# ActiveVisionLab/NeFeS

Hardware: AMD Instinct MI355X
Metric: rays/s (fwd+bwd) at 640x480x(64+128) samples, 8x256 MLP (higher is better)
Workload: dtype f32; 1 GPU; BASELINE configs[1]: 7-Scenes-stairs geometry, 64+128 samples, 8x256 MLP + 16-ch feature head; 640x480, random seed-0 weights, fwd + bwd to the 3x4 pose; parallelism=rows/1

## Files before the change

include/nefes_hip.h:

```cpp
#ifndef NEFES_HIP_H
#define NEFES_HIP_H
#include <stddef.h>
#include <stdint.h>

#ifdef __cplusplus
extern "C" {
#endif

#define NEFES_ABI_VERSION 20
#define NEFES_BLOB_FORMAT 17

#define NEFES_E_BADARG (-1)
#define NEFES_E_UNSUPPORTED (-2)
#define NEFES_E_BADBLOB (-3)

typedef struct NefesNetDesc {
    int32_t width;
    int32_t feat_dim;
    int32_t has_transient;
    int32_t xyz_encoding;
    int32_t fold_final;
} NefesNetDesc;
#define NEFES_XYZ_FREQ10 0
#define NEFES_XYZ_EXTERNAL32 1

typedef struct NefesStreamInfo {
    uint64_t slab_off;
    uint32_t n_slabs;
    uint32_t bias_floats;
    uint64_t bias_off;
    uint32_t scale_off;
    uint32_t scale_count;
} NefesStreamInfo;

typedef struct NefesBlobInfo {
    uint64_t total_bytes;
    NefesStreamInfo stream[13];
} NefesBlobInfo;

#define NEFES_COMP_TRANSIENT 1u
#define NEFES_COMP_STATIC_ONLY 2u
#define NEFES_COMP_SIGMA_ONLY 4u
#define NEFES_COMP_WHITE_BKGD 8u
#define NEFES_COMP_FEAT_WEIGHTS_ONLY 16u

#define NEFES_FIELD_SIGMA 0
#define NEFES_FIELD_STATIC 1
#define NEFES_FIELD_FULL 2

int nefes_version(void);

int nefes_blob_info(const NefesNetDesc* desc, NefesBlobInfo* info);
size_t nefes_stream_slab_bytes(const NefesNetDesc* desc, int stream);
int nefes_pack_weights(const NefesNetDesc* desc, const float* const* tensors, int n_tensors, void* blob,
                       size_t blob_bytes);
int nefes_pack_map(const NefesNetDesc* desc, uint32_t* map, size_t n_entries, int64_t* tensor_elems_out);
int nefes_pack_h3_plan(const NefesNetDesc* desc, int32_t* plan, size_t n_ints, size_t* needed);
int nefes_pack_device(const float* flat, int64_t n_params, const uint32_t* map, int64_t n_entries, const int32_t* plan,
                      int n_jobs, int32_t* scratch, void* blob, void* stream);

int nefes_raygen_fwd(int H, int W, float focal, const float* c2w, int row0, int nrows, float* rays_o, float* rays_d,
                     float* viewdirs, void* stream);
size_t nefes_raygen_bwd_workspace(int n_rays);
int nefes_raygen_bwd(int H, int W, float focal, const float* c2w, int row0, int nrows, const float* g_rays_o,
                     const float* g_rays_d, const float* g_viewdirs, void* workspace, float* g_c2w, void* stream);
int nefes_raygen_k_fwd(int H, int W, const float* intr, const float* c2w, int row0, int nrows, float* rays_o, float* rays_d,
                       float* viewdirs, void* stream);
size_t nefes_raygen_k_bwd_workspace(int n_rays);
int nefes_raygen_k_bwd(int H, int W, const float* intr, const float* c2w, int row0, int nrows, const float* g_rays_o,
                       const float* g_rays_d, const float* g_viewdirs, void* workspace, float* g_c2w, float* g_intr, void* stream);
int nefes_raygen_px_fwd(int n, const float* px, const float* intr, const float* c2w, float* rays_o, float* rays_d, float* viewdirs,
                        void* stream);
size_t nefes_raygen_px_bwd_workspace(int n);
int nefes_raygen_px_bwd(int n, const float* px, const float* intr, const float* c2w, const float* g_rays_o, const float* g_rays_d,
                        const float* g_viewdirs, void* workspace, float* g_c2w, float* g_intr, void* stream);
int nefes_sample_px(int C, int H, int W, const float* map, int n, const float* px, float* out, void* stream);
int nefes_ndc_fwd(int H, int W, float focal, float near, int n, const float* rays_o, const float* rays_d, float* out_o,
                  float* out_d, void* stream);
int nefes_ndc_bwd(int H, int W, float focal, float near, int n, const float* rays_o, const float* rays_d,
                  const float* g_out_o, const float* g_out_d, float* g_rays_o, float* g_rays_d, void* stream);
int nefes_coarse_depths(int N, int Nc, float near, float far, int lindisp, const float* t, const float* t_rand,
                        float* z, void* stream);
int nefes_coarse_depths_rays(int N, int Nc, const float* bounds, int stride, int lindisp, const float* t,
                             const float* t_rand, float* z, void* stream);

size_t nefes_field_mask_bytes(const NefesNetDesc* desc, int64_t M);
int nefes_field_fwd(const NefesNetDesc* desc, const void* packed, int mode, int N, int S, const float* rays_o,
                    const float* rays_d, const float* z, const float* pts, const float* xyz_enc, const float* viewdirs,
                    float* raw_t, uint32_t* masks, void* stream);
int nefes_field_bwd(const NefesNetDesc* desc, const void* packed, int N, int S, const float* rays_o,
                    const float* rays_d, const float* z, const float* pts, const float* viewdirs, const float* raw_t,
                    const float* g_raw_t, const uint32_t* masks, float* g_pts, float* g_xyz_enc, float* g_viewdirs_s,
                    void* stream);
int nefes_ray_grad_reduce(int N, int S, const float* z, const float* g_pts, const float* g_viewdirs_s, float* g_rays_o,
                          float* g_rays_d, float* g_viewdirs, void* stream);

int nefes_composite_fwd(int N, int S, int C, uint32_t flags, float beta_min, const float* raw_t, const float* z,
                        float* rgb, float* feat, float* disp, float* acc, float* depth, float* weights, float* beta,
                        void* stream);
int nefes_composite_bwd(int N, int S, int C, uint32_t flags, const float* raw_t, const float* z, const float* g_rgb,
                        const float* g_feat, const float* g_disp, const float* g_acc, const float* g_depth,
                        const float* g_weights, const float* g_beta, float* g_raw_t, void* stream);

int nefes_sample_pdf_merge(int N, int Nc, int Ni, int layout, const float* z_coarse, const float* weights,
                           const float* u, int u_per_ray, const float* cdf_in, float* z_fine, float* z_samples,
                           int32_t* inds, float* cdf_out, void* stream);
int nefes_coarse_sample(int N, int Nc, int Ni, const float* sigma, const float* z, int z_shared_row, const float* u, int u_per_ray,
                        float* z_fine, float* z_samples, float* weights_out, void* stream);

typedef struct NefesHashGridDesc {
    int32_t n_levels;
    int32_t n_features;
    int32_t log2_hashmap_size;
    int32_t base_resolution;
    float per_level_scale;
    float bound;
} NefesHashGridDesc;
size_t nefes_hashgrid_table_entries(const NefesHashGridDesc* desc);
int nefes_hashgrid_fwd(const NefesHashGridDesc* desc, const float* table, int64_t M, const float* x, float* enc,
                       void* stream);
int nefes_hashgrid_bwd_x(const NefesHashGridDesc* desc, const float* table, int64_t M, const float* x, const float* g_enc,
                         float* g_x, void* stream);
size_t nefes_hashgrid_bwd_table_workspace(const NefesHashGridDesc* desc);
int nefes_hashgrid_bwd_table(const NefesHashGridDesc* desc, int64_t M, const float* x, const float* g_enc, float* g_table,
                             void* workspace, void* stream);

int nefes_field_fwd_x6(const NefesNetDesc* desc, const void* packed, int mode, int N, int S, const float* rays_o,
                       const float* rays_d, const float* z, const float* pts, const float* xyz_enc, const float* viewdirs,
                       float* raw_t, uint32_t* masks, void* stream);

int nefes_field_bwd_static(const NefesNetDesc* desc, const void* packed, int N, int S, const float* rays_o,
                           const float* rays_d, const float* z, const float* pts, const float* viewdirs, const float* raw_t,
                           const float* g_raw_t, const uint32_t* masks, float* g_pts, float* g_viewdirs_s, void* stream);

int nefes_field_bwd_x6(const NefesNetDesc* desc, const void* packed, int N, int S, const float* rays_o, const float* rays_d,
                       const float* z, const float* pts, const float* viewdirs, const float* raw_t, const float* g_raw_t,
                       const uint32_t* masks, float* g_pts, float* g_xyz_enc, float* g_viewdirs_s, void* stream);

int nefes_field_fwd_h3(const NefesNetDesc* desc, const void* packed, int mode, int N, int S, const float* rays_o,
                       const float* rays_d, const float* z, const float* pts, const float* xyz_enc, const float* viewdirs,
                       float* raw_t, uint32_t* masks, void* stream);
int nefes_field_fwd_h3_zrow(const NefesNetDesc* desc, const void* packed, int mode, int N, int S, const float* rays_o,
                            const float* rays_d, const float* z_row, const float* viewdirs, float* raw_t, uint32_t* masks,
                            void* stream);
int nefes_field_bwd_h3(const NefesNetDesc* desc, const void* packed, int N, int S, const float* rays_o, const float* rays_d,
                       const float* z, const float* pts, const float* viewdirs, const float* raw_t, const float* g_raw_t,
                       const uint32_t* masks, float* g_pts, float* g_xyz_enc, float* g_viewdirs_s, void* stream);
int nefes_field_fwd_h3_hashgrid(const NefesNetDesc* desc, const void* packed, const NefesHashGridDesc* grid, const float* table,
                                int mode, int N, int S, const float* rays_o, const float* rays_d, const float* z, int z_is_row,
                                const float* viewdirs, float* raw_t, uint32_t* masks, void* stream);
int nefes_field_bwd_h3_hashgrid(const NefesNetDesc* desc, const void* packed, const NefesHashGridDesc* grid, const float* table,
                                int N, int S, const float* rays_o, const float* rays_d, const float* z, const float* viewdirs,
                                const float* raw_t, const float* g_raw_t, const uint32_t* masks, float* g_pts, float* g_viewdirs_s,
                                void* stream);
int nefes_field_fwd_h3_fh(const NefesNetDesc* desc, const void* packed, int mode, int N, int S, const float* rays_o,
                          const float* rays_d, const float* z, const float* viewdirs, float* raw_t, uint32_t* masks, void* stream);
int nefes_field_bwd_h3_fh(const NefesNetDesc* desc, const void* packed, int N, int S, const float* rays_o, const float* rays_d,
                          const float* z, const float* viewdirs, const float* raw_t, const float* g_raw_t, const float* g_gmap,
                          const uint32_t* masks, float* g_pts, float* g_viewdirs_s, void* stream);
int nefes_feat_head_fwd(int N, int C, int F, const float* gmap, const float* w_t, const float* b, float* feat, void* stream);
int nefes_feat_head_bwd(int N, int C, int F, const float* g_feat, const float* w, const float* b, float* g_gmap, void* stream);
int nefes_field_bwd_static_h3(const NefesNetDesc* desc, const void* packed, int N, int S, const float* rays_o, const float* rays_d,
                              const float* z, const float* pts, const float* viewdirs, const float* raw_t, const float* g_raw_t,
                              const uint32_t* masks, float* g_pts, float* g_viewdirs_s, void* stream);
#define NEFES_H3_REQ_TRAIN 1
#define NEFES_H3_REQ_EXT 2
#define NEFES_H3_REQ_HASHGRID 4
#define NEFES_H3_REQ_FH 8
#define NEFES_H3_REQ_ZROW 16
#define NEFES_H3_REQ_STATIC_BWD 32
int nefes_field_h3_instance(const NefesNetDesc* desc, int backward, int mode, unsigned request_flags, char* name, size_t cap);

typedef struct NefesGenericNetDesc {
    int32_t width;
    int32_t depth;
    int32_t skip;
    int32_t feat_dim;
    int32_t has_transient;
    int32_t xyz_encoding;
} NefesGenericNetDesc;
size_t nefes_generic_blob_bytes(const NefesGenericNetDesc* desc);
int nefes_generic_pack(const NefesGenericNetDesc* desc, const float* const* tensors, int n_tensors, void* blob, size_t blob_bytes);
size_t nefes_generic_mask_bytes(const NefesGenericNetDesc* desc, int64_t M);
int nefes_field_fwd_generic(const NefesGenericNetDesc* desc, const void* packed, int mode, int N, int S, const float* rays_o,
                            const float* rays_d, const float* z, const float* pts, const float* viewdirs, float* raw_t,
                            uint32_t* masks, void* stream);
int nefes_field_bwd_generic(const NefesGenericNetDesc* desc, const void* packed, int mode, int N, int S, const float* rays_o,
                            const float* rays_d, const float* z, const float* pts, const float* viewdirs, const float* raw_t,
                            const float* g_raw_t, const uint32_t* masks, float* g_pts, float* g_viewdirs_s, void* stream);
int nefes_field_fwd_generic_ext(const NefesGenericNetDesc* desc, const void* packed, int mode, int N, int S, const float* xyz_enc,
                                const float* viewdirs, float* raw_t, uint32_t* masks, void* stream);
int nefes_field_bwd_generic_ext(const NefesGenericNetDesc* desc, const void* packed, int mode, int N, int S, const float* viewdirs,
                                const float* raw_t, const float* g_raw_t, const uint32_t* masks, float* g_xyz_enc, float* g_viewdirs_s,
                                void* stream);
int nefes_generic_pack_device(const NefesGenericNetDesc* desc, const float* const* tensors, int n_tensors, void* blob,
                              size_t blob_bytes, void* stream);
size_t nefes_generic_train_rows(const NefesGenericNetDesc* desc);
int nefes_generic_train_row_offset(const NefesGenericNetDesc* desc, int block);
int nefes_field_fwd_train_generic(const NefesGenericNetDesc* desc, const void* packed, int mode, int N, int S, const float* rays_o,
                                  const float* rays_d, const float* z, const float* viewdirs, float* raw_t, float* acts, uint32_t* masks,
                                  void* stream);
int nefes_field_bwd_train_generic(const NefesGenericNetDesc* desc, const void* packed, int mode, int N, int S, const float* rays_o,
                                  const float* rays_d, const float* z, const float* viewdirs, const float* raw_t, const float* g_raw_t,
                                  const uint32_t* masks, float* dacts, float* g_pts, float* g_viewdirs_s, void* stream);
size_t nefes_generic_train_rows_ext(const NefesGenericNetDesc* desc);
int nefes_generic_train_row_offset_ext(const NefesGenericNetDesc* desc, int block);
int nefes_field_fwd_train_generic_ext(const NefesGenericNetDesc* desc, const void* packed, int mode, int N, int S, const float* xyz_enc,
                                      const float* viewdirs, float* raw_t, float* acts, uint32_t* masks, void* stream);
int nefes_field_bwd_train_generic_ext(const NefesGenericNetDesc* desc, const void* packed, int mode, int N, int S,
                                      const float* viewdirs, const float* raw_t, const float* g_raw_t, const uint32_t* masks,
                                      float* dacts, float* g_xyz_enc, float* g_viewdirs_s, void* stream);

size_t nefes_train_rows(const NefesNetDesc* desc);
int nefes_train_row_offset(const NefesNetDesc* desc, int block);
int nefes_field_fwd_train(const NefesNetDesc* desc, const void* packed, int mode, int N, int S, const float* rays_o,
                          const float* rays_d, const float* z, const float* pts, const float* viewdirs, float* raw_t,
                          float* acts, uint32_t* masks, void* stream);
int nefes_field_fwd_train_h3(const NefesNetDesc* desc, const void* packed, int mode, int N, int S, const float* rays_o,
                             const float* rays_d, const float* z, const float* pts, const float* viewdirs, float* raw_t,
                             float* acts, uint32_t* masks, void* stream);
int nefes_field_bwd_train(const NefesNetDesc* desc, const void* packed, int mode, int N, int S, const float* rays_o,
                          const float* rays_d, const float* z, const float* viewdirs, const float* raw_t,
                          const float* g_raw_t, const uint32_t* masks, float* dacts, float* g_pts, float* g_viewdirs_s,
                          void* stream);
int nefes_field_bwd_train_h3(const NefesNetDesc* desc, const void* packed, int mode, int N, int S, const float* rays_o,
                             const float* rays_d, const float* z, const float* viewdirs, const float* raw_t,
                             const float* g_raw_t, const uint32_t* masks, float* dacts, float* g_pts, float* g_viewdirs_s,
                             void* stream);
int nefes_field_fwd_train_h3_ext(const NefesNetDesc* desc, const void* packed, int mode, int N, int S, const float* xyz_enc,
                                 const float* viewdirs, float* raw_t, float* acts, uint32_t* masks, void* stream);
int nefes_field_bwd_train_h3_ext(const NefesNetDesc* desc, const void* packed, int mode, int N, int S, const float* viewdirs,
                                 const float* raw_t, const float* g_raw_t, const uint32_t* masks, float* dacts, float* g_xyz_enc,
                                 float* g_viewdirs_s, void* stream);
int nefes_train_head_grad(const NefesNetDesc* desc, int mode, int N, int S, const float* raw_t, const float* g_raw_t,
                          float* dacts, void* stream);
int nefes_train_dx(int64_t n_tiles, int rows, const float* dacts_in, int g_row0, int n_out, const float* wt, int ldw,
                   int n_in, const float* acts, int dst_row0, int accumulate, int mask, float* dacts_out, void* stream);
int nefes_train_dw(int64_t n_tiles, int rows, const float* dacts, int g_row0, int n_out, const float* acts, int x_row0,
                   int n_in, int x_relu, int splits, float* partial, void* stream);
int nefes_train_dw_bias(int64_t n_tiles, int rows, const float* dacts, int g_row0, int n_out, const float* acts, int x_row0,
                        int n_in, int x_relu, int splits, int64_t split_stride, float* partial, void* stream);

int nefes_conv2d_same(int B, int Cin, int Cout, int H, int W, int ksize, const float* x, const float* mask, const float* w_packed,
                      const float* bias, int relu, float* y, void* stream);
size_t nefes_conv2d_wgrad_workspace(int B, int Cin, int Cout, int H, int W, int ksize);
int nefes_conv2d_wgrad(int B, int Cin, int Cout, int H, int W, int ksize, const float* x, const float* g_y, const float* mask, float* g_w,
                       float* g_bias, void* workspace, void* stream);

int nefes_bicubic_up_fwd(int64_t planes, int h, int w, int OH, int OW, int oy0, int ox0, int CH, int CW, const float* in, float* out,
                         void* stream);
int nefes_bicubic_up_bwd(int64_t planes, int h, int w, int OH, int OW, int oy0, int ox0, int CH, int CW, const float* g_out, float* tmp,
                         float* g_in, void* stream);

int nefes_pose_compose_fwd(int n_poses, const float* r, const float* t, const float* init_c2w, float pose_scale, const float* move,
                           float pose_scale2, float* c2w, void* stream);
int nefes_pose_compose_bwd(int n_poses, const float* r, const float* t, const float* init_c2w, float pose_scale, const float* move,
                           float pose_scale2, const float* g_c2w, float* g_r, float* g_t, void* stream);
int nefes_bn_train_fwd(int B, int C, int64_t P, int per_image, const float* x, const float* weight, const float* bias, double eps,
                       double momentum, float* running_mean, float* running_var, int64_t* num_batches_tracked, float* y, double* save,
                       void* stream);
int nefes_bn_train_bwd(int B, int C, int64_t P, int per_image, const float* x, const float* weight, const double* save, const float* g_y,
                       float* g_x, void* stream);
int nefes_bn_train_bwd_affine(int B, int C, int64_t P, const float* x, const float* weight, const double* save, const float* g_y,
                              float* g_x, float* g_weight, float* g_bias, void* stream);
int nefes_svd_reg_fwd(int n_poses, const float* pose, float* out, double* save, void* stream);
int nefes_svd_reg_bwd(int n_poses, const double* save, const float* g_out, float* g_pose, void* stream);
int nefes_regressed_pose_fwd(int n_poses, const float* pose, int do_svd, float t_scale, float mx, float my, float mz, float* out, double* save,
                             void* stream);
int nefes_regressed_pose_bwd(int n_poses, const double* save, int do_svd, float t_scale, const float* g_out, float* g_pose, void* stream);
size_t nefes_psnr_ssim_workspace(int C, int H, int W);
int nefes_psnr_ssim(int C, int H, int W, const float* x, int64_t x_row_stride, int64_t x_plane_stride, const float* y, int64_t y_row_stride,
                    int64_t y_plane_stride, void* workspace, float* out, void* stream);
size_t nefes_cosine_loss_scratch_doubles(int C);
int nefes_cosine_loss_fwd(int C, int64_t P, const float* a, const float* b, double* scratch, float* loss, void* stream);
int nefes_cosine_loss_bwd(int C, int64_t P, const float* a, const float* b, const double* scratch, const float* g_loss, float* g_a,
                          void* stream);

int nefes_upcos_loss_fwd(int C, int h, int w, int OH, int OW, int crop, const float* x, const float* target, double* scratch, float* loss,
                         void* stream);
int nefes_upcos_loss_bwd(int C, int h, int w, int OH, int OW, int crop, const float* x, const float* target, const double* scratch,
                         const float* g_loss, const int* tx_first, const int* tx_count, const float* tx_wt, const int* ty_first,
                         const int* ty_count, const float* ty_wt, int T, float* tmp, float* g_x, void* stream);
size_t nefes_pixcos_scratch_doubles(int G, int64_t P);
int nefes_pixcos_loss_fwd(int G, int C, int64_t P, const float* a, const float* b, double* scratch, float* loss, void* stream);
int nefes_pixcos_loss_bwd(int G, int C, int64_t P, const float* a, const float* b, const double* scratch, const float* g_loss, float* g_a,
                          void* stream);
size_t nefes_uppixcos_scratch_doubles(int G, int OH, int OW, int crop);
int nefes_uppixcos_loss_fwd(int G, int C, int h, int w, int OH, int OW, int crop, const float* x, const float* target, double* scratch,
                            float* loss, void* stream);
int nefes_uppixcos_loss_bwd(int G, int C, int h, int w, int OH, int OW, int crop, const float* x, const float* target, const double* scratch,
                            const float* g_loss, const int* tx_first, const int* tx_count, const float* tx_wt, const int* ty_first,
                            const int* ty_count, const float* ty_wt, int T, float* tmp, float* g_x, void* stream);
int nefes_cosine_loss_masked_fwd(int G, int Cg, int64_t P, const float* a, const float* b, const uint8_t* mask, double* scratch, float* loss,
                                 void* stream);
int nefes_cosine_loss_masked_bwd(int G, int Cg, int64_t P, const float* a, const float* b, const uint8_t* mask, const double* scratch,
                                 const float* g_loss, float* g_a, void* stream);
int nefes_upcos_loss_masked_fwd(int G, int Cg, int h, int w, int OH, int OW, int crop, const float* x, const float* target,
                                const uint8_t* mask, double* scratch, float* loss, void* stream);
int nefes_upcos_loss_masked_bwd(int G, int Cg, int h, int w, int OH, int OW, int crop, const float* x, const float* target,
                                const uint8_t* mask, const double* scratch, const float* g_loss, const int* tx_first, const int* tx_count,
                                const float* tx_wt, const int* ty_first, const int* ty_count, const float* ty_wt, int T, float* tmp,
                                float* g_x, void* stream);
size_t nefes_pixcos_masked_scratch_doubles(int G, int64_t P);
int nefes_pixcos_loss_masked_fwd(int G, int C, int64_t P, const float* a, const float* b, const uint8_t* mask, double* scratch, float* loss,
                                 void* stream);
int nefes_pixcos_loss_masked_bwd(int G, int C, int64_t P, const float* a, const float* b, const uint8_t* mask, const double* scratch,
                                 const float* g_loss, float* g_a, void* stream);
size_t nefes_uppixcos_masked_scratch_doubles(int G, int OH, int OW, int crop);
int nefes_uppixcos_loss_masked_fwd(int G, int C, int h, int w, int OH, int OW, int crop, const float* x, const float* target,
                                   const uint8_t* mask, double* scratch, float* loss, void* stream);
int nefes_uppixcos_loss_masked_bwd(int G, int C, int h, int w, int OH, int OW, int crop, const float* x, const float* target,
                                   const uint8_t* mask, const double* scratch, const float* g_loss, const int* tx_first,
                                   const int* tx_count, const float* tx_wt, const int* ty_first, const int* ty_count, const float* ty_wt,
                                   int T, float* tmp, float* g_x, void* stream);
int nefes_bicubic_gram(int n_in, int n_out, int o0, int n_win, double* G, void* stream);
int nefes_upcos_prepare(int C, int h, int w, int OH, int OW, int crop, const float* target, const int* tx_first, const int* tx_count,
                        const float* tx_wt, const int* ty_first, const int* ty_count, const float* ty_wt, int T, double* tmp, double* tt,
                        double* dbb, void* stream);
int nefes_upcos_gram_fwd(int C, int h, int w, const float* x, const double* tt, const double* dbb, const double* gram_x, const double* gram_y,
                         int band, double* scratch, double* pmat, float* loss, void* stream);
size_t nefes_upcos_gram_lds_bytes(int h, int w, int band);
int nefes_upcos_gram_bwd(int C, int h, int w, const double* tt, const double* pmat, const double* scratch, const float* g_loss, float* g_x,
                         void* stream);
int nefes_bicubic_gather_table(int n_in, int n_out, int o0, int n_win, int T, int* first, int* count, float* wt, void* stream);

int nefes_fusion_input_fwd(int B, int HW, int C, const float* rgb, const float* feat, const float* affine, const float* mean3,
                           const float* std3, float* x, float* y, void* stream);
int nefes_fusion_input_bwd(int B, int HW, int C, const float* g_x, const float* affine, const float* y, const float* std3, float* g_rgb,
                           float* g_feat, void* stream);
int nefes_adam_step(int n, float* p, const float* g, float* m, float* v, float* step, const double* lr, double beta1, double beta2,
                    double eps, void* stream);

#define NEFES_TRAIN_LOSS_ROWS 16
#define NEFES_LOSS_FEAT_MSE 0
#define NEFES_LOSS_FEAT_L1 1
#define NEFES_LOSS_FEAT_COS 2
#define NEFES_LOSS_HAS_RGB_FINE 1u
#define NEFES_LOSS_HAS_RGB_COARSE 2u
#define NEFES_LOSS_HAS_BETA 4u
#define NEFES_LOSS_HAS_FEAT_FINE 8u
#define NEFES_LOSS_HAS_FEAT_COARSE 16u
#define NEFES_LOSS_HAS_FEAT_FUSION 32u
#define NEFES_LOSS_NERFW 64u
#define NEFES_LOSS_PRESENT_ALL 127u
typedef struct NefesTrainLossDesc {
    int32_t N;
    int32_t C;
    int32_t S;
    int32_t feat_kind;
    uint32_t present;
    float coef;
    float lambda_u;
    int64_t sigma_row_stride;
} NefesTrainLossDesc;
size_t nefes_train_loss_scratch_doubles(int N);
int nefes_train_loss_fwd(const NefesTrainLossDesc* desc, const float* rgb_fine, const float* rgb_coarse, const float* rgb_target,
                         const float* beta, const float* transient_sigmas, const float* feat_fine, const float* feat_coarse,
                         const float* feat_fusion, const float* feat_target, double* scratch, float* terms, float* losses, void* stream);
int nefes_train_loss_bwd(const NefesTrainLossDesc* desc, const float* g_color, const float* g_loss_f, const float* g_loss_fusion,
                         const float* rgb_fine, const float* rgb_coarse, const float* rgb_target, const float* beta,
                         const float* transient_sigmas, const float* feat_fine, const float* feat_coarse, const float* feat_fusion,
                         const float* feat_target, float* g_rgb_fine, float* g_rgb_coarse, float* g_beta, float* g_sigma, float* g_feat_fine,
                         float* g_feat_coarse, float* g_feat_fusion, void* stream);

int nefes_probe_mfma_clock(int random_operands, int ms_target, double* clock_ghz, double* fp16_dense_tflops, void* stream);
int nefes_probe_store_hazard(float* out, int64_t n_float4, int nops, void* stream);
int nefes_probe_pk_mul(unsigned* out, int64_t n, int iters, void* stream);
int nefes_probe_hazard(int test, int k, int blocks, int iters, unsigned* count, void* stream);
int nefes_probe_aggressor(int kind, int iters, int blocks, float* sink, void* stream);

#ifdef __cplusplus
}
#endif
#endif
```

nefes_amd/csrc/field_fwd_h3.hip:

```cpp
#include "field_h3_instances.h"
#ifdef NEFES_TU_W128
#define NEFES_SLAB_KIB 16
#else
#define NEFES_SLAB_KIB 32
#endif
#include <stdio.h>
#include <stdlib.h>
#if defined(NEFES_TU_W128) || !defined(H3_NO_ACC_READ_ASM)
#define NEFES_ASM_READS_ACC
#define NEFES_FENCE_TILES
#endif
#if defined(NEFES_TU_W128)
#define NEFES_ACC_VGPR_FORM
#endif

#ifndef NEFES_FWD_CONSUMER_BIAS
#define NEFES_FWD_CONSUMER_BIAS 1
#endif
#include "field_common.h"
#include "../../include/nefes_hip.h"

#include "field_x6.h"
#include "hashgrid.h"
#if !defined(NEFES_TU_W128) && !defined(H3_NO_ACC_READ_ASM)
#define H3_ACC_READ_ASM
#endif
#include "field_h3.h"
#define NEFES_H3_SLOTS 2

struct FieldFwdH3Args {
    const char* stream;
    const float* bias;
    uint32_t n_slabs, bias_floats, scale_off;
    const float* rays_o;
    const float* rays_d;
    const float* z;
    const float* pts;
    const float* xyz_enc;
    const float* viewdirs;
    float* raw_t;
    uint32_t* masks;
    int N, S, R, C;
    long long M;
    int n_tiles;
    uint32_t s_magic, s_shift;
    float* acts;
    int rows;
    int z_row;
    const float2* hg_table;
    HgGeom hg;
    int gout;
};

template <int NT, int T0, int NX>
__device__ __forceinline__ void train_save_h3(float* tile_base, uint32_t voff, int row0, const f32x16 (&X)[NX], float inv) {
    float* p = tile_base + (size_t)(row0 >> 5) * 4096 + voff;
#pragma unroll
    for (int t = 0; t < NT; ++t)
#pragma unroll
        for (int r = 0; r < 16; ++r) {
#ifndef NEFES_TRAIN_NO_STORES
            __builtin_nontemporal_store(X[T0 + t][r] * inv, &p[t * 4096 + nefes_rho(0, r) * 16]);
#endif
        }
}

template <int MODEF, int ENC, int W = 256, int NTR = 1, bool TRAIN = false, bool FH = false>
__global__ __launch_bounds__(256, W == 128 ? 2 : 1) void field_fwd_h3_kernel(FieldFwdH3Args a) {
    constexpr bool FOLD = MODEF == NEFES_FIELD_FULL_FOLD;
    constexpr int MODE = FOLD ? NEFES_FIELD_FULL : MODEF;
    static_assert(NEFES_SLAB_KIB == (W == 128 ? NEFES_H3_FWD_SLAB_KIB_128 : NEFES_H3_FWD_SLAB_KIB), "ring slab size != the packer's for this width");
    static_assert(!FOLD || (MODE != NEFES_FIELD_SIGMA && !TRAIN), "the fold serves the head products of frozen networks");
    constexpr int NTW = W / 32, NTH = W / 64;
    constexpr int ES = ENC != NEFES_XYZ_FREQ10 ? NEFES_X_STEPS : NEFES_E_STEPS;
    constexpr int MW = 8 * (W / 64) + 4 * (W / 128), WT = (NTW + 1) / 2, WH = (NTH + 1) / 2;
    constexpr int NSEG = MODE == NEFES_FIELD_SIGMA ? NEFES_H3F_SIG + 1
                         : (MODE == NEFES_FIELD_STATIC ? NEFES_H3F_N_STATIC : (FOLD ? NEFES_H3FF_N : NEFES_H3F_N));
    extern __shared__ __attribute__((aligned(16))) char smem[];
    char* ring_base = smem;
    float* bias_lds = (float*)(smem + NEFES_H3_SLOTS * NEFES_SLAB_BYTES);
    float* e_lds = bias_lds + ((a.bias_floats + 63) / 64) * 64 + (threadIdx.x >> 6) * (ES * 64) + (threadIdx.x & 63);
    const int lane = threadIdx.x & 63;
    const int wave = __builtin_amdgcn_readfirstlane(threadIdx.x >> 6);
    const int j = lane & 31, h = lane >> 5;
    for (uint32_t i = threadIdx.x; i < a.bias_floats; i += 256) bias_lds[i] = a.bias[i];
    HgGeom* hg_lds = (HgGeom*)(bias_lds + ((a.bias_floats + 63) / 64) * 64 + 4 * ES * 64);
    if constexpr (ENC == NEFES_XYZ_HASHGRID_FUSED) {
        if (threadIdx.x == 0) *hg_lds = a.hg;
    }
    StagedRing ring;
    ring.init(a.stream, a.n_slabs, ring_base, wave, lane);
    const char* ring_lane = ring_base + lane * 16;
    const char* bias_half = (const char*)bias_lds + 16 * h;
    const int* tab_i = (const int*)(bias_lds + a.scale_off);
    const float* tab_f = bias_lds + a.scale_off;
    auto wexp = [&](int seg) { return tab_i[nefes_h3_tab_exp(nefes_h3f_seg(FOLD, seg))]; };
    auto rowb = [&](int seg) { return tab_f[nefes_h3_tab_bound(nefes_h3f_seg(FOLD, seg))]; };
    auto bmax = [&](int blk) { return tab_f[nefes_h3_tab_bias(NSEG, nefes_h3f_bias(FOLD, blk))]; };
    ring.prime(ring_lane);
    constexpr int B_SIG = 8 * W, B_FINAL = B_SIG + 32, B_DIR = B_FINAL + (FOLD ? 0 : W), B_RGB = B_DIR + W / 2,
                  B_T0 = B_RGB + 32 * NTR, B_T1 = B_T0 + W / 2, B_T2 = B_T1 + W / 2, B_TH = B_T2 + W / 2;
#pragma unroll 1
    for (int tile = blockIdx.x; tile < a.n_tiles; tile += gridDim.x) {
        auto locate = [&](uint32_t& m, uint32_t& ray, uint32_t& smp) {
            const uint32_t m_raw = (uint32_t)tile * 128u + (uint32_t)(wave * 32 + j);
            const bool ok = m_raw < (uint32_t)a.M;
            m = ok ? m_raw : (uint32_t)a.M - 1u;
            ray = a.s_magic ? __umulhi(m, a.s_magic) >> a.s_shift : m;
            smp = m - ray * (uint32_t)a.S;
            return ok;
        };
        uint32_t m, ray, smp;
        locate(m, ray, smp);
        float in_o[3] = {0.f, 0.f, 0.f}, in_d[3] = {0.f, 0.f, 0.f}, in_z = 0.f;
        float E[ES];
        if constexpr (ENC == NEFES_XYZ_EXTERNAL32) {
#pragma unroll
            for (int s = 0; s < ES; ++s) E[s] = a.xyz_enc[(size_t)m * 32 + 2 * s + h];
        } else if (ENC != NEFES_XYZ_HASHGRID_FUSED && a.pts) {
#pragma unroll
            for (int c = 0; c < 3; ++c) in_o[c] = a.pts[(size_t)m * 3 + c];
        } else {
            in_z = a.z[a.z_row ? smp : m];
#pragma unroll
            for (int c = 0; c < 3; ++c) { in_o[c] = a.rays_o[ray * 3 + c]; in_d[c] = a.rays_d[ray * 3 + c]; }
        }
        float mE;
        if constexpr (ENC == NEFES_XYZ_EXTERNAL32) {
            mE = pair_max(array_max(E));
        } else if constexpr (ENC == NEFES_XYZ_HASHGRID_FUSED) {
            float x[3];
#pragma unroll
            for (int c = 0; c < 3; ++c) x[c] = add_rn(in_o[c], mul_rn(in_d[c], in_z));
            hg_encode_slots(E, x, h, *hg_lds, a.hg_table);
            mE = pair_max(array_max(E));
        } else {
            float x[3];
#pragma unroll
            for (int c = 0; c < 3; ++c) x[c] = a.pts ? in_o[c] : add_rn(in_o[c], mul_rn(in_d[c], in_z));
            embed_slots<NEFES_N_FREQ_XYZ>(E, x, h);
            mE = fmaxf(fmaxf(1.f, fabsf(x[0])), fmaxf(fabsf(x[1]), fabsf(x[2])));
        }
#pragma unroll
        for (int s = 0; s < ES; ++s) e_lds[s * 64] = E[s];
        float* act_tile = nullptr;
        const uint32_t act_voff = nefes_train_lane_off(wave, j, h);
        const uint32_t emb_off = (uint32_t)(((wave * 32 + j) >> 4) * 512 + h * 16 + (j & 15));
        if constexpr (TRAIN) {
            act_tile = a.acts + (size_t)tile * a.rows * 128;
            float* pe = act_tile + (size_t)(nefes_train_row(W, 0, NEFES_TB_E) >> 5) * 4096 + emb_off;
#pragma unroll
            for (int s = 0; s < ES; ++s) __builtin_nontemporal_store(E[s], &pe[(s >> 4) * 4096 + 2 * (s & 15) * 16]);
        }
        auto save_trunk = [&](int layer, const f32x16 (&X)[NTW], int es) {
            if constexpr (TRAIN) train_save_h3<NTW, 0>(act_tile, act_voff, nefes_train_row(W, 0, NEFES_TB_L1) + (layer - 1) * W, X, pow2i(-es));
        };
        uint32_t* mask_ptr = (MODE != NEFES_FIELD_SIGMA && a.masks) ? a.masks + ((size_t)((long long)tile * 4 + wave) * MW) * 64 + lane : nullptr;
        auto put_masks = [&](const uint32_t* bits, int n) {
            if (MODE != NEFES_FIELD_SIGMA && mask_ptr) {
                for (int w = 0; w < n; ++w) __builtin_nontemporal_store(bits[w], &mask_ptr[w * 64]);
                mask_ptr += n * 64;
            }
        };
        auto raw_col = [&]() -> float* {
            uint32_t mm, rr, ss;
            if (!locate(mm, rr, ss)) return nullptr;
            return a.raw_t + ((size_t)rr * a.R * a.S + ss);
        };
        auto bias_at = [&](int off_floats, int es) { return BiasInitScaled{bias_half + off_floats * 4, pow2i(es)}; };
        constexpr bool CB = !TRAIN && W == 256 && NEFES_FWD_CONSUMER_BIAS;
        float2 nbias;
        f32x16 A[NTW], B[NTW];
        uint32_t bits[WT];
        auto clear_bits = [&]() {
#pragma unroll
            for (int w = 0; w < WT; ++w) bits[w] = 0u;
        };
        constexpr bool CAP = MODE != NEFES_FIELD_SIGMA;
        auto tau_of = [&](float M, int ew) {
            const int t = pick_exp(M);
            return t < 100 - ew ? t : 100 - ew;
        };
        auto sigma_head = [&](const f32x16 (&X)[NTW], int es_x, int tau_x) {
            f32x16 sg[1];
            float mdummy = 0.f;
            const int es = tau_x + wexp(NEFES_H3F_SIG);
            if constexpr (CB) {
                const char* bp8 = bias_half + 7 * W * 4;
                nbias = ReluBiasSplitH<false, NTW, WT>::prime(bp8);
                mma_run_h3<1, W / 16, 0, true>(ring, ring_lane, ReluBiasSplitH<false, NTW, WT>{X, bits, pow2i(tau_x - es_x), mdummy, bp8, pow2i(es_x), nbias},
                                               bias_at(B_SIG, es), sg);
            } else
            mma_run_h3<1, W / 16, 0, true>(ring, ring_lane, ReluSplitH<false, NTW, WT>{X, bits, pow2i(tau_x - es_x), mdummy},
                                           bias_at(B_SIG, es), sg);
            float* col = raw_col();
            if (col && h == 0) {
                const int ch = (MODE == NEFES_FIELD_SIGMA) ? 0 : 3 + a.C;
                __builtin_nontemporal_store(softplus_ref(sg[0][0] * pow2i(-es)), &col[(size_t)ch * a.S]);
            }
        };
        int es_a, es_b = 0;
        float M;
        {
            const int tau = tau_of(mE, wexp(NEFES_H3F_L1));
            es_a = tau + wexp(NEFES_H3F_L1);
            if constexpr (CB) mma_run_h3<NTW, ES / 8, 0, true>(ring, ring_lane, LdsSplitH{e_lds, pow2i(tau)}, ZeroInit{}, A);
            else mma_run_h3<NTW, ES / 8, 0, true>(ring, ring_lane, LdsSplitH{e_lds, pow2i(tau)}, bias_at(0, es_a), A);
            M = rowb(NEFES_H3F_L1) * mE + bmax(NEFES_H3BB_L1);
            save_trunk(1, A, es_a);
        }
#define NEFES_FWD_EVEN_LAYER(L1_, SEG1_)                                                                                       \
        clear_bits();                                                                                                          \
        {                                                                                                                      \
            const int ew = wexp(SEG1_), tau = tau_of(M, ew);                                                                   \
            const float rb_ = rowb(SEG1_), bm_ = bmax((L1_) - 1);           \
            float mx = 0.f;                                                                                                    \
            if constexpr (CB) {                                                                                                \
                const char* bps = bias_half + ((L1_) - 2) * W * 4;                           \
                nbias = ReluBiasSplitH<CAP, NTW, WT>::prime(bps);                                                              \
                mma_run_h3<NTW, W / 16, 0, true>(ring, ring_lane, ReluBiasSplitH<CAP, NTW, WT>{A, bits, pow2i(tau - es_a), mx, bps, pow2i(es_a), nbias}, \
                                                 ZeroInit{}, B);                                                               \
            } else                                                                                                             \
            mma_run_h3<NTW, W / 16, 0, true>(ring, ring_lane, ReluSplitH<CAP, NTW, WT>{A, bits, pow2i(tau - es_a), mx},        \
                                             bias_at(((L1_) - 1) * W, tau + ew), B);                                           \
            M = rb_ * (pair_max(mx) * pow2i(-es_a)) + bm_;                                                                     \
            es_b = tau + ew;                                                                                                   \
            save_trunk(L1_, B, es_b);                                                                                          \
        }                                                                                                                      \
        put_masks(bits, WT);
        constexpr bool END8 = MODE == NEFES_FIELD_SIGMA || FOLD;
        constexpr int NPAIRS = END8 ? 3 : 4;
#pragma unroll 1
        for (int p = 0; p < NPAIRS; ++p) {
            const int l1 = 2 + 2 * p, l2 = l1 + 1;
            const int seg1 = l1 <= 5 ? l1 - 1 : l1;
            const int seg2 = l2 <= 5 ? l2 - 1 : (l2 <= 8 ? l2 : NEFES_H3F_FINAL);
            NEFES_FWD_EVEN_LAYER(l1, seg1)
            clear_bits();
            {
                const int ew = wexp(seg2);
                const int tau = tau_of(p == 1 ? fmaxf(M, mE) : M, ew);
                if (p == 3) sigma_head(B, es_b, tau_of(M, wexp(NEFES_H3F_SIG)));
                const float rb_ = rowb(seg2), bm_ = bmax(l2 <= 8 ? l2 - 1 : NEFES_H3BB_FINAL);
                const float rbe_ = p == 1 ? rowb(NEFES_H3F_L5E) : 0.f;
                float mx = 0.f;
                if constexpr (CB) {
                    const char* bps = bias_half + (l1 - 1) * W * 4;
                    nbias = ReluBiasSplitH<CAP, NTW, WT>::prime(bps);
                    const ReluBiasSplitH<CAP, NTW, WT> src{B, bits, pow2i(tau - es_b), mx, bps, pow2i(es_b), nbias};
                    mma_run_h3<NTW, W / 16, 0, true>(ring, ring_lane, src, ZeroInit{}, A);
                } else
                mma_run_h3<NTW, W / 16, 0, true>(ring, ring_lane, ReluSplitH<CAP, NTW, WT>{B, bits, pow2i(tau - es_b), mx},
                                                 bias_at(l2 <= 8 ? (l2 - 1) * W : B_FINAL, tau + ew), A);
                if (p == 1) mma_run_h3<NTW, ES / 8, 0, false>(ring, ring_lane, LdsSplitH{e_lds, pow2i(tau)}, ZeroInit{}, A);
                M = rb_ * (pair_max(mx) * pow2i(-es_b)) + (p == 1 ? rbe_ * mE : 0.f) + bm_;
                es_a = tau + ew;
                save_trunk(l2, A, es_a);
            }
            put_masks(bits, WT);
        }
        if constexpr (END8) { NEFES_FWD_EVEN_LAYER(8, NEFES_H3F_L8) }
#undef NEFES_FWD_EVEN_LAYER
        if constexpr (MODE == NEFES_FIELD_SIGMA) sigma_head(B, es_b, tau_of(M, wexp(NEFES_H3F_SIG)));
        if constexpr (MODE != NEFES_FIELD_SIGMA) {
            constexpr bool FULL = MODE == NEFES_FIELD_FULL;
            constexpr int NDT = FULL ? 2 * NTH : NTH;
            float v[3];
            {
                uint32_t mm, rr, ss;
                locate(mm, rr, ss);
#pragma unroll
                for (int c = 0; c < 3; ++c) v[c] = a.viewdirs[(size_t)rr * 3 + c];
            }
            float Dv[16];
            {
                float d14[NEFES_D_STEPS];
                embed_slots<NEFES_N_FREQ_DIR>(d14, v, h);
#pragma unroll
                for (int s = 0; s < 16; ++s) Dv[s] = s < NEFES_D_STEPS ? d14[s] : 0.f;
            }
            if constexpr (TRAIN) {
                float* pd = act_tile + (size_t)(nefes_train_row(W, 0, NEFES_TB_DV) >> 5) * 4096 + emb_off;
#pragma unroll
                for (int s = 0; s < NEFES_D_STEPS; ++s) __builtin_nontemporal_store(Dv[s], &pd[2 * s * 16]);
            }
            f32x16 dt[NDT];
            uint32_t bits2[WH];
            auto clear2 = [&]() {
#pragma unroll
                for (int w = 0; w < WH; ++w) bits2[w] = 0u;
            };
            struct Bias2 {
                BiasInitScaled a, b;
                __device__ __forceinline__ f32x16 operator()(int t) const { return t < NTH ? a(t) : b(t - NTH); }
            };
            int es_dt;
            if constexpr (FOLD) {
                sigma_head(B, es_b, tau_of(M, wexp(NEFES_H3F_SIG)));
                const int ew = wexp(NEFES_H3F_DT_H);
                const float mD = pair_max(array_max(Dv));
                const int tau = tau_of(fmaxf(M, mD), ew);
                const float rbh_ = rowb(NEFES_H3F_DT_H), rbd_ = rowb(NEFES_H3F_DT_D);
                const float bm_ = fmaxf(bmax(NEFES_H3BB_DIR), bmax(NEFES_H3BB_T0));
                float mx = 0.f;
                es_dt = tau + ew;
                clear_bits();
                if constexpr (CB) {
                    const char* bp8 = bias_half + 7 * W * 4;
                    nbias = ReluBiasSplitH<CAP, NTW, WT>::prime(bp8);
                    const ReluBiasSplitH<CAP, NTW, WT> src8{B, bits, pow2i(tau - es_b), mx, bp8, pow2i(es_b), nbias};
                    mma_run_h3<NDT, W / 16, 0, true>(ring, ring_lane, src8, Bias2{bias_at(B_DIR, es_dt), bias_at(B_T0, es_dt)}, dt);
                } else {
                    const ReluSplitH<CAP, NTW, WT> src8{B, bits, pow2i(tau - es_b), mx};
                    mma_run_h3<NDT, W / 16, 0, true>(ring, ring_lane, src8, Bias2{bias_at(B_DIR, es_dt), bias_at(B_T0, es_dt)}, dt);
                }
                mma_run_h3<NDT, 2, 0, false>(ring, ring_lane, ArraySplitH<16>{Dv, pow2i(tau)}, ZeroInit{}, dt);
                M = rbh_ * (pair_max(mx) * pow2i(-es_b)) + rbd_ * mD + bm_;
                put_masks(bits, WT);
            } else {
                const int ew = wexp(NEFES_H3F_DT_H);
                const float mD = pair_max(array_max(Dv));
                const int tau = tau_of(fmaxf(M, mD), ew);
                float mx = 0.f;
                es_dt = tau + ew;
                if constexpr (CB) {
                    const char* bpf = bias_half + B_FINAL * 4;
                    nbias = ReluBiasSplitH<false, 1, 1>::prime(bpf);
                    const IdentBiasSplitH<NTW> srcf{A, pow2i(tau - es_a), mx, bpf, pow2i(es_a), nbias};
                    if constexpr (FULL) mma_run_h3<NDT, W / 16, 0, true>(ring, ring_lane, srcf, Bias2{bias_at(B_DIR, es_dt), bias_at(B_T0, es_dt)}, dt);
                    else mma_run_h3<NDT, W / 16, 0, true>(ring, ring_lane, srcf, bias_at(B_DIR, es_dt), dt);
                } else if constexpr (FULL)
                    mma_run_h3<NDT, W / 16, 0, true>(ring, ring_lane, IdentSplitH<NTW, 0>{A, pow2i(tau - es_a), mx},
                                                     Bias2{bias_at(B_DIR, es_dt), bias_at(B_T0, es_dt)}, dt);
                else
                    mma_run_h3<NDT, W / 16, 0, true>(ring, ring_lane, IdentSplitH<NTW, 0>{A, pow2i(tau - es_a), mx}, bias_at(B_DIR, es_dt), dt);
                mma_run_h3<NDT, 2, 0, false>(ring, ring_lane, ArraySplitH<16>{Dv, pow2i(tau)}, ZeroInit{}, dt);
                M = rowb(NEFES_H3F_DT_H) * (pair_max(mx) * pow2i(-es_a)) + rowb(NEFES_H3F_DT_D) * mD
                    + (FULL ? fmaxf(bmax(NEFES_H3BB_DIR), bmax(NEFES_H3BB_T0)) : bmax(NEFES_H3BB_DIR));
                if constexpr (TRAIN) {
                    train_save_h3<NTH, 0>(act_tile, act_voff, nefes_train_row(W, 0, NEFES_TB_DIR), dt, pow2i(-es_dt));
                    if constexpr (FULL) train_save_h3<NTH, NTH>(act_tile, act_voff, nefes_train_row(W, 0, NEFES_TB_T0), dt, pow2i(-es_dt));
                }
            }
            if constexpr (FH) {
                float* col = raw_col();
                if (col) {
                    int S_g = a.S;
                    asm volatile("" : "+s"(S_g));
                    const float inv = pow2i(-es_dt);
                    float* pg = col + (size_t)(3 + 4 * h) * S_g;
#pragma unroll
                    for (int t = 0; t < NTH; ++t)
#pragma unroll
                        for (int r = 0; r < 16; ++r)
                            __builtin_nontemporal_store(fmaxf(dt[t][r] * inv, 0.f), &pg[(size_t)(32 * t + nefes_rho(0, r)) * S_g]);
                    if (h == 0) __builtin_nontemporal_store(1.f, &col[(size_t)(3 + W / 2) * S_g]);
                }
            }
            {
                f32x16 ar[NTR];
                clear2();
                const int ew = wexp(NEFES_H3F_RGB), tau = tau_of(M, ew), es = tau + ew;
                float mdummy = 0.f;
                mma_run_h3<NTR, W / 32, 0, true>(ring, ring_lane, ReluSplitH<true, NDT, WH>{dt, bits2, pow2i(tau - es_dt), mdummy},
                                                 bias_at(B_RGB, es), ar);
                put_masks(bits2, WH);
                float* col = raw_col();
                if (col) {
                    float* ph = col + (size_t)(4 * h) * a.S;
                    const float inv = pow2i(-es);
                    int S_t = a.S, c3 = FH ? 3 : 3 + a.C;
                    asm volatile("" : "+s"(S_t), "+s"(c3));
                    const int full = c3 >> 5;
#pragma unroll
                    for (int t = 0; t < NTR; ++t) {
                        if (t < full) {
#pragma unroll
                            for (int r = 0; r < 16; ++r)
                                __builtin_nontemporal_store(ar[t][r] * inv, &ph[(size_t)(32 * t + nefes_rho(0, r)) * S_t]);
                        } else if (32 * t < c3) {
#pragma unroll
                            for (int r = 0; r < 16; ++r) {
                                const int cu = 32 * t + nefes_rho(0, r);
                                if (cu + 4 * h < c3) __builtin_nontemporal_store(ar[t][r] * inv, &ph[(size_t)cu * S_t]);
                            }
                        }
                    }
                }
            }
            if constexpr (FULL) {
            f32x16 acc3[NTH], acc2[NTH];
            int es3, es2, es_th;
            clear2();
            {
                const int ew = wexp(NEFES_H3F_T1), tau = tau_of(M, ew);
                float mx = 0.f;
                es3 = tau + ew;
                mma_run_h3<NTH, W / 32, 0, true>(ring, ring_lane, ReluSplitH<true, NDT, WH, NTH>{dt, bits2, pow2i(tau - es_dt), mx},
                                                 bias_at(B_T1, es3), acc3);
                M = rowb(NEFES_H3F_T1) * (pair_max(mx) * pow2i(-es_dt)) + bmax(NEFES_H3BB_T1);
                if constexpr (TRAIN) train_save_h3<NTH, 0>(act_tile, act_voff, nefes_train_row(W, 0, NEFES_TB_T1), acc3, pow2i(-es3));
            }
            put_masks(bits2, WH);
            clear2();
            {
                const int ew = wexp(NEFES_H3F_T2), tau = tau_of(M, ew);
                float mx = 0.f;
                es2 = tau + ew;
                mma_run_h3<NTH, W / 32, 0, true>(ring, ring_lane, ReluSplitH<true, NTH, WH>{acc3, bits2, pow2i(tau - es3), mx},
                                                 bias_at(B_T2, es2), acc2);
                M = rowb(NEFES_H3F_T2) * (pair_max(mx) * pow2i(-es3)) + bmax(NEFES_H3BB_T2);
                if constexpr (TRAIN) train_save_h3<NTH, 0>(act_tile, act_voff, nefes_train_row(W, 0, NEFES_TB_T2), acc2, pow2i(-es2));
            }
            put_masks(bits2, WH);
            f32x16 th[1];
            clear2();
            {
                const int ew = wexp(NEFES_H3F_TH), tau = tau_of(M, ew);
                float mdummy = 0.f;
                es_th = tau + ew;
                mma_run_h3<1, W / 32, 0, true>(ring, ring_lane, ReluSplitH<true, NTH, WH>{acc2, bits2, pow2i(tau - es2), mdummy},
                                               bias_at(B_TH, es_th), th);
            }
            put_masks(bits2, WH);
            float* col = raw_col();
            if (col) {
                float* o = col + (size_t)(3 + a.C + 1) * a.S;
                const float inv = pow2i(-es_th);
                if (h == 0) {
                    __builtin_nontemporal_store(sigmoid_ref(th[0][0] * inv), &o[0]);
                    __builtin_nontemporal_store(sigmoid_ref(th[0][1] * inv), &o[(size_t)a.S]);
                    __builtin_nontemporal_store(sigmoid_ref(th[0][2] * inv), &o[(size_t)2 * a.S]);
                    __builtin_nontemporal_store(softplus_ref(th[0][3] * inv), &o[(size_t)3 * a.S]);
                } else {
                    __builtin_nontemporal_store(softplus_ref(th[0][0] * inv), &o[(size_t)4 * a.S]);
                }
            }
            }
        }
    }
}

static void magic_div(uint32_t d, uint32_t& magic, uint32_t& shift) {
    if (d == 1) { magic = 0; shift = 0; return; }
    uint32_t l = 0;
    while ((1ull << l) < d) ++l;
    const uint64_t p = 31 + l;
    magic = (uint32_t)(((1ull << p) + d - 1) / d);
    shift = (uint32_t)(p - 32);
}

template <int MODE, int ENC, int W = 256, int NTR = 1, bool TRAIN = false, bool FH = false>
static int launch_h3(const FieldFwdH3Args& a, hipStream_t st) {
    constexpr int ES_ = ENC != NEFES_XYZ_FREQ10 ? NEFES_X_STEPS : NEFES_E_STEPS;
    const size_t lds = (size_t)NEFES_H3_SLOTS * NEFES_SLAB_BYTES + ((a.bias_floats + 63) / 64) * 256 + (size_t)4 * ES_ * 64 * 4
                       + (ENC == NEFES_XYZ_HASHGRID_FUSED ? 512 : 0);
    static_assert(sizeof(HgGeom) <= 512, "the level geometry's LDS slot");
    auto k = field_fwd_h3_kernel<MODE, ENC, W, NTR, TRAIN, FH>;
    hipError_t e = hipFuncSetAttribute((const void*)k, hipFuncAttributeMaxDynamicSharedMemorySize, (int)lds);
    if (e != hipSuccess) return (int)e;
    int dev = 0, cus = 256;
    (void)hipGetDevice(&dev);
    (void)hipDeviceGetAttribute(&cus, hipDeviceAttributeMultiprocessorCount, dev);
    const int per_cu = W == 128 ? 2 : 1;
    int grid = a.n_tiles < cus * per_cu ? a.n_tiles : cus * per_cu;
    if (const char* cap = getenv("NEFES_DEBUG_MAX_GRID")) {
        const int c = atoi(cap);
        if (c > 0 && c < grid) grid = c;
    }
    hipLaunchKernelGGL(k, dim3(grid), dim3(256), lds, st, a);
    return (int)hipGetLastError();
}

#ifdef NEFES_TU_W128
constexpr bool kTuW128 = true;
#else
constexpr bool kTuW128 = false;
#endif
#define X(part, MODE, ENC, W, NTR, TRAIN, FH) \
    static_assert(part != NEFES_TU_PART || (W == 128) == kTuW128, "a Wd = 128 row belongs to an object built for Wd = 128, and no other row does");
NEFES_H3_FWD_INSTANCES(X)
#undef X

template <int PART>
static int h3_fwd_launch_rows(const NefesH3FwdKey& k, const FieldFwdH3Args& a, hipStream_t st) {
#define X(part, MODE, ENC, W, NTR, TRAIN, FH)                                                                          \
    if constexpr (part == PART) {                                                                                      \
        if (k == NEFES_H3_FWD_KEY(MODE, ENC, W, NTR, TRAIN, FH))                                                       \
            return launch_h3<NEFES_FIELD_##MODE, NEFES_XYZ_##ENC, W, NTR, TRAIN != 0, FH != 0>(a, st);                 \
    }
    NEFES_H3_FWD_INSTANCES(X)
#undef X
    return NEFES_E_UNSUPPORTED;
}
#define X(part, MODE, ENC, W, NTR, TRAIN, FH) int NEFES_H3_FWD_PART_FN(part)(const NefesH3FwdKey&, const FieldFwdH3Args&, hipStream_t);
NEFES_H3_FWD_INSTANCES(X)
#undef X
int NEFES_H3_FWD_PART_FN(NEFES_TU_PART)(const NefesH3FwdKey& k, const FieldFwdH3Args& a, hipStream_t st) {
    return h3_fwd_launch_rows<NEFES_TU_PART>(k, a, st);
}

#if NEFES_TU_PART == 0
struct H3FwdRow {
    NefesH3FwdKey key;
    const char* name;
    int (*launch)(const NefesH3FwdKey&, const FieldFwdH3Args&, hipStream_t);
};
static const H3FwdRow h3_fwd_rows[] = {
#define X(part, MODE, ENC, W, NTR, TRAIN, FH) \
    {NEFES_H3_FWD_KEY(MODE, ENC, W, NTR, TRAIN, FH), "fwd p" #part " <" #MODE "," #ENC "," #W "," #NTR "," #TRAIN "," #FH ">", NEFES_H3_FWD_PART_FN(part)},
    NEFES_H3_FWD_INSTANCES(X)
#undef X
};

struct H3FwdSel {
    int rc;
    const H3FwdRow* row;
};
static H3FwdSel h3_fwd_select(const NefesNetDesc* desc, int mode, unsigned req) {
    const bool train = req & NEFES_H3_REQ_TRAIN, fh = req & NEFES_H3_REQ_FH, fused_grid = req & NEFES_H3_REQ_HASHGRID;
    const bool ext = desc->xyz_encoding == NEFES_XYZ_EXTERNAL32, fold = desc->fold_final != 0;
    const int cls = nefes_head_class(desc->feat_dim), w = desc->width;
    if (fused_grid ? !ext : (fh && ext)) return {NEFES_E_BADARG, nullptr};
    if ((req & NEFES_H3_REQ_ZROW) && desc->xyz_encoding != NEFES_XYZ_FREQ10) return {NEFES_E_UNSUPPORTED, nullptr};
    if (mode != NEFES_FIELD_FULL && mode != NEFES_FIELD_STATIC && (train || mode != NEFES_FIELD_SIGMA)) return {NEFES_E_UNSUPPORTED, nullptr};
    if (mode == NEFES_FIELD_FULL && !desc->has_transient) return {NEFES_E_BADARG, nullptr};
    bool ok;
    if (train) {
        ok = (req & NEFES_H3_REQ_EXT) ? (w == 256 && ext) : ((w == 256 || w == 128) && desc->xyz_encoding == NEFES_XYZ_FREQ10);
        ok = ok && cls >= 0 && !fold;
    } else {
        ok = (w == 256 || (w == 128 && !ext)) && cls >= 0 && (ext || desc->xyz_encoding == NEFES_XYZ_FREQ10);
        ok = ok && !(mode == NEFES_FIELD_STATIC && ext);
        ok = ok && !(fold && mode != NEFES_FIELD_SIGMA && !(mode == NEFES_FIELD_FULL && w == 256 && !ext && !fh));
        ok = ok && !(fh && (desc->feat_dim != 0 || w != 128 || ext || mode != NEFES_FIELD_FULL));
    }
    if (!ok) return {NEFES_E_UNSUPPORTED, nullptr};
    const NefesH3FwdKey key = {fold && mode == NEFES_FIELD_FULL ? NEFES_FIELD_FULL_FOLD : mode,
                               fused_grid ? NEFES_XYZ_HASHGRID_FUSED : desc->xyz_encoding, w,
                               mode == NEFES_FIELD_SIGMA ? (w == 128 ? 5 : 1) : (cls == 0 ? 1 : 5), train, fh};
    for (const H3FwdRow& r : h3_fwd_rows)
        if (r.key == key) return {0, &r};
    return {NEFES_E_UNSUPPORTED, nullptr};
}

static int h3_fwd_stream(const NefesNetDesc* desc, const NefesH3FwdKey& k, NefesStreamInfo* si) {
    NefesBlobInfo info;
    int rc = nefes_blob_info(desc, &info);
    if (rc) return rc;
    *si = info.stream[k.mode == NEFES_FIELD_SIGMA ? NEFES_STREAM_FWD_SIGMA_H3
                      : (k.mode == NEFES_FIELD_STATIC ? NEFES_STREAM_FWD_STATIC_H3 : NEFES_STREAM_FWD_FULL_H3)];
    return si->n_slabs == 0 ? NEFES_E_UNSUPPORTED : 0;
}

static int h3_fwd_args(const NefesNetDesc* desc, const void* packed, const NefesH3FwdKey& k, int N, int S,
                       const NefesHashGridDesc* grid, FieldFwdH3Args& a) {
    NefesStreamInfo si;
    int rc = h3_fwd_stream(desc, k, &si);
    if (rc) return rc;
    a.stream = (const char*)packed + si.slab_off;
    a.bias = (const float*)((const char*)packed + si.bias_off);
    a.n_slabs = si.n_slabs; a.bias_floats = si.bias_floats; a.scale_off = si.scale_off;
    if (k.enc == NEFES_XYZ_HASHGRID_FUSED) {
        rc = hg_geometry(grid, &a.hg, nullptr);
        if (rc) return rc;
        if (a.hg.n_levels != 16) return NEFES_E_UNSUPPORTED;
    }
    a.gout = k.fh ? k.w / 2 : 0;
    a.N = N; a.S = S; a.C = k.fh ? a.gout + 1 : desc->feat_dim;
    a.R = k.mode == NEFES_FIELD_SIGMA ? 1 : 3 + a.C + (k.mode == NEFES_FIELD_STATIC ? 1 : 6);
    a.M = (long long)N * S;
    if (a.M >= (1ll << 31) - 256) return NEFES_E_UNSUPPORTED;
    a.n_tiles = (int)((a.M + 127) / 128);
    a.rows = k.train ? nefes_train_row(desc->width, desc->feat_dim, NEFES_TB_END) : 0;
    magic_div((uint32_t)S, a.s_magic, a.s_shift);
    return 0;
}

static int h3_fwd_run(const NefesNetDesc* desc, const void* packed, int mode, unsigned req, int N, int S,
                      const NefesHashGridDesc* grid, FieldFwdH3Args& a, void* stream) {
    const H3FwdSel s = h3_fwd_select(desc, mode, req);
    if (s.rc) return s.rc;
    const int rc = h3_fwd_args(desc, packed, s.row->key, N, S, grid, a);
    return rc ? rc : s.row->launch(s.row->key, a, (hipStream_t)stream);
}

int nefes_h3_bwd_instance(const NefesNetDesc* desc, int mode, unsigned req, const char** name);

extern "C" int nefes_field_h3_instance(const NefesNetDesc* desc, int backward, int mode, unsigned request_flags, char* name, size_t cap) {
    if (!desc || !name || cap == 0) return NEFES_E_BADARG;
    name[0] = 0;
    const unsigned kind = request_flags & ~(unsigned)NEFES_H3_REQ_EXT;
    if ((kind & (kind - 1)) || (request_flags >> 6) || ((request_flags & NEFES_H3_REQ_EXT) && kind != NEFES_H3_REQ_TRAIN) ||
        (request_flags & (backward ? NEFES_H3_REQ_ZROW : NEFES_H3_REQ_STATIC_BWD)))
        return NEFES_E_BADARG;
    const char* text = nullptr;
    int rc;
    if (backward) {
        rc = nefes_h3_bwd_instance(desc, mode, request_flags, &text);
    } else {
        const H3FwdSel s = h3_fwd_select(desc, mode, request_flags);
        NefesStreamInfo si;
        rc = s.rc ? s.rc : h3_fwd_stream(desc, s.row->key, &si);
        if (!rc) text = s.row->name;
    }
    if (text) snprintf(name, cap, "%s", text);
    return rc;
}

extern "C" int nefes_field_fwd_train_h3(const NefesNetDesc* desc, const void* packed, int mode, int N, int S, const float* rays_o,
                                        const float* rays_d, const float* z, const float* pts, const float* viewdirs,
                                        float* raw_t, float* acts, uint32_t* masks, void* stream) {
    if (!desc || !packed || !raw_t || !acts || !viewdirs || N <= 0 || S <= 0) return NEFES_E_BADARG;
    if (!pts && !(rays_o && rays_d && z)) return NEFES_E_BADARG;
    FieldFwdH3Args a = {};
    a.rays_o = rays_o; a.rays_d = rays_d; a.z = z; a.pts = pts; a.viewdirs = viewdirs; a.raw_t = raw_t; a.masks = masks; a.acts = acts;
    return h3_fwd_run(desc, packed, mode, NEFES_H3_REQ_TRAIN, N, S, nullptr, a, stream);
}

extern "C" int nefes_field_fwd_train_h3_ext(const NefesNetDesc* desc, const void* packed, int mode, int N, int S, const float* xyz_enc,
                                            const float* viewdirs, float* raw_t, float* acts, uint32_t* masks, void* stream) {
    if (!desc || !packed || !xyz_enc || !raw_t || !acts || !viewdirs || N <= 0 || S <= 0) return NEFES_E_BADARG;
    FieldFwdH3Args a = {};
    a.xyz_enc = xyz_enc; a.viewdirs = viewdirs; a.raw_t = raw_t; a.masks = masks; a.acts = acts;
    return h3_fwd_run(desc, packed, mode, NEFES_H3_REQ_TRAIN | NEFES_H3_REQ_EXT, N, S, nullptr, a, stream);
}

static int field_fwd_h3_impl(const NefesNetDesc* desc, const void* packed, int mode, unsigned req, int N, int S,
                             const NefesHashGridDesc* grid, FieldFwdH3Args& a, void* stream) {
    if (!desc || !packed || !a.raw_t || N <= 0 || S <= 0) return NEFES_E_BADARG;
    const bool ext = desc->xyz_encoding == NEFES_XYZ_EXTERNAL32;
    const bool fused_grid = ext && a.hg_table != nullptr;
    if (fused_grid ? !(a.rays_o && a.rays_d && a.z && grid) : (ext ? !a.xyz_enc : (!a.pts && !(a.rays_o && a.rays_d && a.z)))) return NEFES_E_BADARG;
    if (!a.viewdirs && (mode == NEFES_FIELD_FULL || (mode == NEFES_FIELD_STATIC && !ext))) return NEFES_E_BADARG;
    return h3_fwd_run(desc, packed, mode, req, N, S, grid, a, stream);
}

extern "C" int nefes_field_fwd_h3(const NefesNetDesc* desc, const void* packed, int mode, int N, int S, const float* rays_o,
                                  const float* rays_d, const float* z, const float* pts, const float* xyz_enc,
                                  const float* viewdirs, float* raw_t, uint32_t* masks, void* stream) {
    FieldFwdH3Args a = {};
    a.rays_o = rays_o; a.rays_d = rays_d; a.z = z; a.pts = pts; a.xyz_enc = xyz_enc; a.viewdirs = viewdirs; a.raw_t = raw_t; a.masks = masks;
    return field_fwd_h3_impl(desc, packed, mode, 0, N, S, nullptr, a, stream);
}

extern "C" int nefes_field_fwd_h3_hashgrid(const NefesNetDesc* desc, const void* packed, const NefesHashGridDesc* grid,
                                           const float* table, int mode, int N, int S, const float* rays_o, const float* rays_d,
                                           const float* z, int z_is_row, const float* viewdirs, float* raw_t, uint32_t* masks,
                                           void* stream) {
    if (!desc || desc->xyz_encoding != NEFES_XYZ_EXTERNAL32 || !grid || !table) return NEFES_E_BADARG;
    FieldFwdH3Args a = {};
    a.rays_o = rays_o; a.rays_d = rays_d; a.z = z; a.z_row = z_is_row ? 1 : 0; a.viewdirs = viewdirs; a.raw_t = raw_t; a.masks = masks;
    a.hg_table = (const float2*)table;
    return field_fwd_h3_impl(desc, packed, mode, NEFES_H3_REQ_HASHGRID, N, S, grid, a, stream);
}

extern "C" int nefes_field_fwd_h3_fh(const NefesNetDesc* desc, const void* packed, int mode, int N, int S, const float* rays_o,
                                     const float* rays_d, const float* z, const float* viewdirs, float* raw_t, uint32_t* masks,
                                     void* stream) {
    if (!rays_o || !rays_d || !z) return NEFES_E_BADARG;
    FieldFwdH3Args a = {};
    a.rays_o = rays_o; a.rays_d = rays_d; a.z = z; a.viewdirs = viewdirs; a.raw_t = raw_t; a.masks = masks;
    return field_fwd_h3_impl(desc, packed, mode, NEFES_H3_REQ_FH, N, S, nullptr, a, stream);
}

extern "C" int nefes_field_fwd_h3_zrow(const NefesNetDesc* desc, const void* packed, int mode, int N, int S, const float* rays_o,
                                       const float* rays_d, const float* z_row, const float* viewdirs, float* raw_t, uint32_t* masks,
                                       void* stream) {
    if (!rays_o || !rays_d || !z_row) return NEFES_E_BADARG;
    if (desc && desc->xyz_encoding != NEFES_XYZ_FREQ10) return NEFES_E_UNSUPPORTED;
    FieldFwdH3Args a = {};
    a.rays_o = rays_o; a.rays_d = rays_d; a.z = z_row; a.z_row = 1; a.viewdirs = viewdirs; a.raw_t = raw_t; a.masks = masks;
    return field_fwd_h3_impl(desc, packed, mode, NEFES_H3_REQ_ZROW, N, S, nullptr, a, stream);
}
#endif
```

nefes_amd/csrc/field_h3.h:

```cpp
#pragma once
#ifndef NEFES_H3_WIDE_MIN
#define NEFES_H3_WIDE_MIN 8
#endif
#ifndef NEFES_H3_WIDE_MAX
#define NEFES_H3_WIDE_MAX 64
#endif

typedef _Float16 f16x8 __attribute__((ext_vector_type(8)));

struct Split2 {
    u32x4 h, l;
};
__device__ __forceinline__ f16x8 as_f16x8(u32x4 v) {
    f16x8 r;
    __builtin_memcpy(&r, &v, 16);
    return r;
}
__device__ __forceinline__ f16x8 as_f16x8(f32x4 v) {
    f16x8 r;
    __builtin_memcpy(&r, &v, 16);
    return r;
}

__device__ __forceinline__ float pow2i(int e) {
    e = e < -126 ? -126 : (e > 127 ? 127 : e);
    return __uint_as_float((uint32_t)(e + 127) << 23);
}
__device__ __forceinline__ int pick_exp(float m) {
    const int be = (int)(__float_as_uint(m) >> 23);
    const int ex = NEFES_H3_TARGET_EXP + 127 - be;
    return (be < 20 || be > 250) ? 0 : ex;
}
__device__ __forceinline__ float pair_max(float m) {
    const uint32_t u = __float_as_uint(m);
    const auto r = __builtin_amdgcn_permlane32_swap(u, u, false, false);
    const uint32_t a = r[0], b = r[1];
    return __uint_as_float(a > b ? a : b);
}
__device__ __forceinline__ void max3_acc(float& m, float x0, float x1) {
    asm volatile("v_max3_f32 %0, %0, %1, %2" : "+v"(m) : "v"(x0), "v"(x1));
}
__device__ __forceinline__ void absmax3_acc(float& m, float x0, float x1) {
    asm volatile("v_max3_f32 %0, %0, |%1|, |%2|" : "+v"(m) : "v"(x0), "v"(x1));
}
template <int N>
__device__ __forceinline__ float array_max(const float (&v)[N]) {
    float m = 0.f;
#pragma unroll
    for (int i = 0; i < N; ++i) m = fmaxf(m, fabsf(v[i]));
    return m;
}
__device__ __forceinline__ int cap_exp(int ex, int es_in, int ew) {
    const int room = 100 - es_in - ew;
    return ex < room ? ex : room;
}

__device__ __forceinline__ void split_pair_hi(Split2& o, int p, float x0, float x1, float r) {
    uint32_t h;
    asm volatile(
        "v_fma_mixlo_f16 %0, %1, %3, 0 op_sel_hi:[0,0,0]\n\t"
        "v_fma_mixhi_f16 %0, %2, %3, 0 op_sel_hi:[0,0,0]"
        : "=&v"(h)
        : "v"(x0), "v"(x1), "v"(r));
    o.h[p] = h;
}
template <bool NOP>
__device__ __forceinline__ void split_pair_lo(Split2& o, int p, float x0, float x1, float r) {
    uint32_t l;
    const uint32_t h = o.h[p];
    if (NOP)
        asm volatile(
            "v_fma_mixlo_f16 %0, %1, %3, -%4 op_sel:[0,0,0] op_sel_hi:[0,0,1]\n\t"
            "v_fma_mixhi_f16 %0, %2, %3, -%4 op_sel:[0,0,1] op_sel_hi:[0,0,1]\n\t"
            "s_nop 1"
            : "=&v"(l)
            : "v"(x0), "v"(x1), "v"(r), "v"(h));
    else
        asm volatile(
            "v_fma_mixlo_f16 %0, %1, %3, -%4 op_sel:[0,0,0] op_sel_hi:[0,0,1]\n\t"
            "v_fma_mixhi_f16 %0, %2, %3, -%4 op_sel:[0,0,1] op_sel_hi:[0,0,1]"
            : "=&v"(l)
            : "v"(x0), "v"(x1), "v"(r), "v"(h));
    o.l[p] = l;
}
template <bool NOP>
__device__ __forceinline__ void split_pair_h(Split2& o, int p, float x0, float x1, float r) {
    uint32_t h, l;
    if (NOP)
        asm volatile(
            "v_fma_mixlo_f16 %0, %2, %4, 0 op_sel_hi:[0,0,0]\n\t"
            "v_fma_mixhi_f16 %0, %3, %4, 0 op_sel_hi:[0,0,0]\n\t"
            "v_fma_mixlo_f16 %1, %2, %4, -%0 op_sel:[0,0,0] op_sel_hi:[0,0,1]\n\t"
            "v_fma_mixhi_f16 %1, %3, %4, -%0 op_sel:[0,0,1] op_sel_hi:[0,0,1]\n\t"
            "s_nop 1"
            : "=&v"(h), "=&v"(l)
            : "v"(x0), "v"(x1), "v"(r));
    else
        asm volatile(
            "v_fma_mixlo_f16 %0, %2, %4, 0 op_sel_hi:[0,0,0]\n\t"
            "v_fma_mixhi_f16 %0, %3, %4, 0 op_sel_hi:[0,0,0]\n\t"
            "v_fma_mixlo_f16 %1, %2, %4, -%0 op_sel:[0,0,0] op_sel_hi:[0,0,1]\n\t"
            "v_fma_mixhi_f16 %1, %3, %4, -%0 op_sel:[0,0,1] op_sel_hi:[0,0,1]"
            : "=&v"(h), "=&v"(l)
            : "v"(x0), "v"(x1), "v"(r));
    o.h[p] = h;
    o.l[p] = l;
}

struct PairRegs {
    float x0, x1;
};
__device__ __forceinline__ float acc_read(const float& x) {
#if defined(H3_ACC_READ_ASM)
    float v;
    asm volatile("v_accvgpr_read_b32 %0, %1" : "=v"(v) : "a"(x));
    return v;
#else
    return x;
#endif
}
template <bool CAPTURE, int NX, int NWORDS, int T0 = 0>
struct ReluSplitH {
    const f32x16 (&X)[NX];
    uint32_t (&bits)[NWORDS];
    float r;
    float& m;
    __device__ __forceinline__ void stage_a(PairRegs& s, int q, int p) const {
        s.x0 = acc_read(X[T0 + (q >> 1)][(q & 1) * 8 + 2 * p]);
        s.x1 = acc_read(X[T0 + (q >> 1)][(q & 1) * 8 + 2 * p + 1]);
        if (CAPTURE) {
            mask_shift_in(bits[(8 * q + 2 * p) >> 5], s.x0);
            mask_shift_in(bits[(8 * q + 2 * p + 1) >> 5], s.x1);
        }
    }
    __device__ __forceinline__ void stage_b(PairRegs& s) const {
        s.x0 = relu1<false>(s.x0);
        s.x1 = relu1<false>(s.x1);
        max3_acc(m, s.x0, s.x1);
    }
    template <bool NOP>
    __device__ __forceinline__ void stage_c(Split2& o, int p, const PairRegs& s) const { split_pair_h<NOP>(o, p, s.x0, s.x1, r); }
    __device__ __forceinline__ void stage_c1(Split2& o, int p, const PairRegs& s) const { split_pair_hi(o, p, s.x0, s.x1, r); }
    template <bool NOP>
    __device__ __forceinline__ void stage_c2(Split2& o, int p, const PairRegs& s) const { split_pair_lo<NOP>(o, p, s.x0, s.x1, r); }
};
template <bool CAPTURE, int NX, int NWORDS>
struct ReluBiasSplitH {
    const f32x16 (&X)[NX];
    uint32_t (&bits)[NWORDS];
    float r;
    float& m;
    const char* bp;
    float bs;
    float2& nb;
    static __device__ __forceinline__ int pair_off(int q, int p) {
        const int r0 = (q & 1) * 8 + 2 * p;
        return ((q >> 1) * 32 + 8 * (r0 >> 2) + (r0 & 3)) * 4;
    }
    static __device__ __forceinline__ float2 prime(const char* bp_) { return *(const float2*)(bp_ + pair_off(0, 0)); }
    __device__ __forceinline__ void stage_a(PairRegs& s, int q, int p) const {
        const float2 b = nb;
        const int qn = p == 3 ? q + 1 : q, pn = p == 3 ? 0 : p + 1;
        nb = *(const float2*)(bp + pair_off(qn, pn));
        s.x0 = __builtin_fmaf(b.x, bs, acc_read(X[q >> 1][(q & 1) * 8 + 2 * p]));
        s.x1 = __builtin_fmaf(b.y, bs, acc_read(X[q >> 1][(q & 1) * 8 + 2 * p + 1]));
        if (CAPTURE) {
            mask_shift_in(bits[(8 * q + 2 * p) >> 5], s.x0);
            mask_shift_in(bits[(8 * q + 2 * p + 1) >> 5], s.x1);
        }
    }
    __device__ __forceinline__ void stage_b(PairRegs& s) const {
        s.x0 = relu1<false>(s.x0);
        s.x1 = relu1<false>(s.x1);
        max3_acc(m, s.x0, s.x1);
    }
    template <bool NOP>
    __device__ __forceinline__ void stage_c(Split2& o, int p, const PairRegs& s) const { split_pair_h<NOP>(o, p, s.x0, s.x1, r); }
    __device__ __forceinline__ void stage_c1(Split2& o, int p, const PairRegs& s) const { split_pair_hi(o, p, s.x0, s.x1, r); }
    template <bool NOP>
    __device__ __forceinline__ void stage_c2(Split2& o, int p, const PairRegs& s) const { split_pair_lo<NOP>(o, p, s.x0, s.x1, r); }
};
template <int NX>
struct IdentBiasSplitH {
    const f32x16 (&X)[NX];
    float r;
    float& m;
    const char* bp;
    float bs;
    float2& nb;
    __device__ __forceinline__ void stage_a(PairRegs& s, int q, int p) const {
        const float2 b = nb;
        const int qn = p == 3 ? q + 1 : q, pn = p == 3 ? 0 : p + 1;
        nb = *(const float2*)(bp + ReluBiasSplitH<false, 1, 1>::pair_off(qn, pn));
        s.x0 = __builtin_fmaf(b.x, bs, acc_read(X[q >> 1][(q & 1) * 8 + 2 * p]));
        s.x1 = __builtin_fmaf(b.y, bs, acc_read(X[q >> 1][(q & 1) * 8 + 2 * p + 1]));
    }
    __device__ __forceinline__ void stage_b(PairRegs& s) const { absmax3_acc(m, s.x0, s.x1); }
    template <bool NOP>
    __device__ __forceinline__ void stage_c(Split2& o, int p, const PairRegs& s) const { split_pair_h<NOP>(o, p, s.x0, s.x1, r); }
    __device__ __forceinline__ void stage_c1(Split2& o, int p, const PairRegs& s) const { split_pair_hi(o, p, s.x0, s.x1, r); }
    template <bool NOP>
    __device__ __forceinline__ void stage_c2(Split2& o, int p, const PairRegs& s) const { split_pair_lo<NOP>(o, p, s.x0, s.x1, r); }
};
template <int NX, int NWORDS, int T0>
struct MaskedSplitH {
    const f32x16 (&X)[NX];
    uint32_t (&bits)[NWORDS];
    float r;
    float& m;
    __device__ __forceinline__ void stage_a(PairRegs& s, int q, int p) const {
        s.x0 = mask_pick<false>(bits[(8 * q + 2 * p) >> 5], 8 * q + 2 * p, acc_read(X[T0 + (q >> 1)][(q & 1) * 8 + 2 * p]));
        s.x1 = mask_pick<false>(bits[(8 * q + 2 * p + 1) >> 5], 8 * q + 2 * p + 1, acc_read(X[T0 + (q >> 1)][(q & 1) * 8 + 2 * p + 1]));
    }
    __device__ __forceinline__ void stage_b(PairRegs& s) const {
        absmax3_acc(m, s.x0, s.x1);
    }
    template <bool NOP>
    __device__ __forceinline__ void stage_c(Split2& o, int p, const PairRegs& s) const { split_pair_h<NOP>(o, p, s.x0, s.x1, r); }
    __device__ __forceinline__ void stage_c1(Split2& o, int p, const PairRegs& s) const { split_pair_hi(o, p, s.x0, s.x1, r); }
    template <bool NOP>
    __device__ __forceinline__ void stage_c2(Split2& o, int p, const PairRegs& s) const { split_pair_lo<NOP>(o, p, s.x0, s.x1, r); }
};
template <int NX, int NWORDS, int T0, int NADD>
struct MaskedAddSplitH {
    const f32x16 (&X)[NX];
    uint32_t (&bits)[NWORDS];
    float r;
    float& m;
    const float (&add)[NADD];
    float sa;
    __device__ __forceinline__ void stage_a(PairRegs& s, int q, int p) const {
        const float x0 = __builtin_fmaf(add[8 * q + 2 * p], sa, acc_read(X[T0 + (q >> 1)][(q & 1) * 8 + 2 * p]));
        const float x1 = __builtin_fmaf(add[8 * q + 2 * p + 1], sa, acc_read(X[T0 + (q >> 1)][(q & 1) * 8 + 2 * p + 1]));
        s.x0 = mask_pick<false>(bits[(8 * q + 2 * p) >> 5], 8 * q + 2 * p, x0);
        s.x1 = mask_pick<false>(bits[(8 * q + 2 * p + 1) >> 5], 8 * q + 2 * p + 1, x1);
    }
    __device__ __forceinline__ void stage_b(PairRegs& s) const { absmax3_acc(m, s.x0, s.x1); }
    template <bool NOP>
    __device__ __forceinline__ void stage_c(Split2& o, int p, const PairRegs& s) const { split_pair_h<NOP>(o, p, s.x0, s.x1, r); }
    __device__ __forceinline__ void stage_c1(Split2& o, int p, const PairRegs& s) const { split_pair_hi(o, p, s.x0, s.x1, r); }
    template <bool NOP>
    __device__ __forceinline__ void stage_c2(Split2& o, int p, const PairRegs& s) const { split_pair_lo<NOP>(o, p, s.x0, s.x1, r); }
};
template <int NX, int T0>
struct IdentSplitH {
    const f32x16 (&X)[NX];
    float r;
    float& m;
    __device__ __forceinline__ void stage_a(PairRegs& s, int q, int p) const {
        s.x0 = acc_read(X[T0 + (q >> 1)][(q & 1) * 8 + 2 * p]);
        s.x1 = acc_read(X[T0 + (q >> 1)][(q & 1) * 8 + 2 * p + 1]);
    }
    __device__ __forceinline__ void stage_b(PairRegs& s) const { absmax3_acc(m, s.x0, s.x1); }
    template <bool NOP>
    __device__ __forceinline__ void stage_c(Split2& o, int p, const PairRegs& s) const { split_pair_h<NOP>(o, p, s.x0, s.x1, r); }
    __device__ __forceinline__ void stage_c1(Split2& o, int p, const PairRegs& s) const { split_pair_hi(o, p, s.x0, s.x1, r); }
    template <bool NOP>
    __device__ __forceinline__ void stage_c2(Split2& o, int p, const PairRegs& s) const { split_pair_lo<NOP>(o, p, s.x0, s.x1, r); }
};
template <int N>
struct ArraySplitH {
    const float (&v)[N];
    float r;
    __device__ __forceinline__ void stage_a(PairRegs& s, int q, int p) const { s.x0 = v[8 * q + 2 * p]; s.x1 = v[8 * q + 2 * p + 1]; }
    __device__ __forceinline__ void stage_b(PairRegs&) const {}
    template <bool NOP>
    __device__ __forceinline__ void stage_c(Split2& o, int p, const PairRegs& s) const { split_pair_h<NOP>(o, p, s.x0, s.x1, r); }
    __device__ __forceinline__ void stage_c1(Split2& o, int p, const PairRegs& s) const { split_pair_hi(o, p, s.x0, s.x1, r); }
    template <bool NOP>
    __device__ __forceinline__ void stage_c2(Split2& o, int p, const PairRegs& s) const { split_pair_lo<NOP>(o, p, s.x0, s.x1, r); }
};
struct LdsSplitH {
    const float* base;
    float r;
    __device__ __forceinline__ void stage_a(PairRegs& s, int q, int p) const {
        s.x0 = base[(8 * q + 2 * p) * 64];
        s.x1 = base[(8 * q + 2 * p + 1) * 64];
    }
    __device__ __forceinline__ void stage_b(PairRegs&) const {}
    template <bool NOP>
    __device__ __forceinline__ void stage_c(Split2& o, int p, const PairRegs& s) const { split_pair_h<NOP>(o, p, s.x0, s.x1, r); }
    __device__ __forceinline__ void stage_c1(Split2& o, int p, const PairRegs& s) const { split_pair_hi(o, p, s.x0, s.x1, r); }
    template <bool NOP>
    __device__ __forceinline__ void stage_c2(Split2& o, int p, const PairRegs& s) const { split_pair_lo<NOP>(o, p, s.x0, s.x1, r); }
};

struct BiasInitScaled {
    const char* p;
    float s;
    __device__ __forceinline__ f32x16 operator()(int t) const {
        f32x16 c;
#pragma unroll
        for (int q = 0; q < 4; ++q) {
            const f32x4 b = *(const f32x4*)(p + (t * 32 + 8 * q) * 4);
            c[4 * q + 0] = b[0] * s; c[4 * q + 1] = b[1] * s; c[4 * q + 2] = b[2] * s; c[4 * q + 3] = b[3] * s;
        }
        return c;
    }
};

struct StagedRing {
    const char* src;
    uint32_t n_slabs;
    uint32_t g_next;
    uint32_t c_slot;
    uint32_t cur_off;
    uint32_t my_off;
    char* my_lds;
    f32x4 pf;
    f32x4 stage[NEFES_SLAB_PIECES];

    __device__ __forceinline__ void load_piece(int q) {
        stage[q] = *(const f32x4*)(src + (size_t)g_next * NEFES_SLAB_BYTES + my_off + q * 1024);
    }
    __device__ __forceinline__ void init(const char* stream, uint32_t nslabs, char* ring_base, int wave, int lane) {
        src = stream; n_slabs = nslabs;
        my_off = (uint32_t)(wave * NEFES_SLAB_PIECES * 1024 + lane * 16);
        my_lds = ring_base + my_off;
        g_next = 0; c_slot = 0; cur_off = 0;
#pragma unroll
        for (int q = 0; q < NEFES_SLAB_PIECES; ++q) load_piece(q);
#pragma unroll
        for (int q = 0; q < NEFES_SLAB_PIECES; ++q) *(f32x4*)(my_lds + q * 1024) = stage[q];
        g_next = n_slabs > 1 ? 1 : 0;
#pragma unroll
        for (int q = 0; q < NEFES_SLAB_PIECES; ++q) load_piece(q);
        g_next = (g_next + 1 == n_slabs) ? 0 : g_next + 1;
    }
    __device__ __forceinline__ void store_piece(int q) {
        *(f32x4*)(my_lds + (c_slot ^ 1u) * NEFES_SLAB_BYTES + q * 1024) = stage[q];
    }
    __device__ __forceinline__ void fetch_piece(int q) {
        load_piece(q);
        if (q == NEFES_SLAB_PIECES - 1) g_next = (g_next + 1 == n_slabs) ? 0 : g_next + 1;
    }
    __device__ __forceinline__ void issue_piece(int q) {
        *(f32x4*)(my_lds + (c_slot ^ 1u) * NEFES_SLAB_BYTES + q * 1024) = stage[q];
        load_piece(q);
        if (q == NEFES_SLAB_PIECES - 1) g_next = (g_next + 1 == n_slabs) ? 0 : g_next + 1;
    }
    __device__ __forceinline__ uint32_t acquire() {
        asm volatile("s_waitcnt lgkmcnt(0)" ::: "memory");
        __builtin_amdgcn_s_barrier();
        c_slot ^= 1u;
        return c_slot * NEFES_SLAB_BYTES;
    }
    __device__ __forceinline__ void prime(const char* ring_lane) {
        asm volatile("s_waitcnt lgkmcnt(0)" ::: "memory");
        __builtin_amdgcn_s_barrier();
        cur_off = 0;
        pf = *(const f32x4*)(ring_lane);
    }
    __device__ __forceinline__ void drain() {}
};

__device__ __forceinline__ void mfma_h3_asm(f32x16& c, const f32x4& a, const u32x4& b) {
    asm volatile("v_mfma_f32_32x32x16_f16 %0, %1, %2, %0" : "+a"(c) : "v"(a), "v"(b));
}
__device__ __forceinline__ void mfma_h3_asm_v(f32x16& c, const f32x4& a, const u32x4& b) {
    asm volatile("v_mfma_f32_32x32x16_f16 %0, %1, %2, %0" : "+v"(c) : "v"(a), "v"(b));
}
__device__ __forceinline__ void mfma_h3_asm_c0(f32x16& c, const f32x4& a, const u32x4& b) {
    asm volatile("v_mfma_f32_32x32x16_f16 %0, %1, %2, 0" : "=a"(c) : "v"(a), "v"(b));
}
__device__ __forceinline__ void mfma_h3_asm_v_c0(f32x16& c, const f32x4& a, const u32x4& b) {
    asm volatile("v_mfma_f32_32x32x16_f16 %0, %1, %2, 0" : "=v"(c) : "v"(a), "v"(b));
}
template <class T> struct h3_is_zero_init { static constexpr bool value = false; };
template <> struct h3_is_zero_init<ZeroInit> { static constexpr bool value = true; };
template <int NT, int KS16, int T0, bool FIRST = true, int VT = 0, class SrcFn, class InitFn, int NACC, class Ring>
__device__ __forceinline__ void mma_run_h3_wide(Ring& ring, const char* ring_lane, const SrcFn& src, const InitFn& init,
                                                f32x16 (&acc)[NACC]) {
    static_assert(T0 + NT <= NACC, "accumulator array too small");
    static_assert(T0 + NT - 2 >= VT, "the run's last two tiles must be AGPR tiles (end-of-run wait states)");
    static_assert(NT >= 8 && NT % 2 == 0, "the gap schedule below pairs tiles: an even tile hosts a pair, the odd one a ring piece");
    constexpr int UPS = (NEFES_SLAB_FRAGS / 4) / 2;
    constexpr int NU = KS16 * NT;
    constexpr int NSLAB = (NU + UPS - 1) / UPS;
    Split2 B0, B1;
    auto BQ = [&](int k) -> Split2& { return (k & 1) ? B1 : B0; };
    asm volatile("s_nop 13" ::: "memory");
#ifdef H3_WIDE_ENTRY_FENCE
    __builtin_amdgcn_sched_barrier(0);
    asm volatile("s_nop 7\n\ts_nop 7\n\ts_nop 1" ::: "memory");
    __builtin_amdgcn_sched_barrier(0);
#endif
    {
        PairRegs s0;
#pragma unroll
        for (int pp = 0; pp < 4; ++pp) {
            src.stage_a(s0, 0, pp);
            src.stage_b(s0);
            if (pp == 3) src.template stage_c<true>(B0, pp, s0);
            else src.template stage_c<false>(B0, pp, s0);
        }
    }
    constexpr bool C0 = FIRST && h3_is_zero_init<InitFn>::value
        ;
    if (FIRST && !C0) acc[T0] = init(0);
    const char* p = ring_lane + ring.cur_off;
    f32x4 ha0 = ring.pf, la0 = *(const f32x4*)(p + 1024);
    f32x4 ha1 = *(const f32x4*)(p + 2048), la1 = *(const f32x4*)(p + 3072);
    f32x4 ha2, la2;
    auto HA = [&](int k) -> f32x4& { return k % 3 == 0 ? ha0 : (k % 3 == 1 ? ha1 : ha2); };
    auto LA = [&](int k) -> f32x4& { return k % 3 == 0 ? la0 : (k % 3 == 1 ? la1 : la2); };
    PairRegs ps[4];
#pragma unroll
    for (int sl = 0; sl < NSLAB; ++sl) {
        const int nu = (NU - sl * UPS) < UPS ? (NU - sl * UPS) : UPS;
        const int acq_u = nu >= 2 ? nu - 2 : 0;
        auto piece_unit = [&](int qq) { const int m_ = ((2 * qq + 1) * nu) / UPS; return m_ < acq_u ? m_ : acq_u; };
#pragma unroll
        for (int uu = 0; uu < UPS; ++uu) {
            if (uu < nu) {
                const int u = sl * UPS + uu, q = u / NT, t = u % NT;
                const bool make = q + 1 < KS16;
                const int pp = t / 2;
                const bool host = make && (t % 2 == 0) && pp < 4;
                const bool tail = make && (t % 2 == 1) && pp < 4;
                const char* pn = p + (2 * uu + 4) * 1024;
                Split2& B = BQ(q);
                Split2& Bn = BQ(q + 1);
                f32x4 &h0 = HA(u), &l0 = LA(u), &h2 = HA(u + 2), &l2 = LA(u + 2);
                __builtin_amdgcn_sched_barrier(0);
                const bool vt = T0 + t < VT;
                if (C0 && q == 0) {
                    if (vt) mfma_h3_asm_v_c0(acc[T0 + t], l0, B.h);
                    else mfma_h3_asm_c0(acc[T0 + t], l0, B.h);
                } else {
                    if (FIRST && q == 0) {
                        if (vt) asm volatile("s_nop 1" : "+v"(acc[T0 + t]));
                        else asm volatile("s_nop 1" : "+a"(acc[T0 + t]));
                    }
                    if (vt) mfma_h3_asm_v(acc[T0 + t], l0, B.h);
                    else mfma_h3_asm(acc[T0 + t], l0, B.h);
                }
                __builtin_amdgcn_sched_barrier(0);
                if (host) src.stage_a(ps[pp], q + 1, pp);
                if (tail) src.template stage_c2<false>(Bn, pp, ps[pp]);
                if (!host && uu != acq_u) h2 = *(const f32x4*)(pn);
                __builtin_amdgcn_sched_barrier(0);
                asm volatile("" ::"v"(l0), "v"(B.h));
                if (vt) mfma_h3_asm_v(acc[T0 + t], h0, B.l);
                else mfma_h3_asm(acc[T0 + t], h0, B.l);
                __builtin_amdgcn_sched_barrier(0);
                if (host) src.stage_b(ps[pp]);
                if (host && uu != acq_u) h2 = *(const f32x4*)(pn);
                if (!host) {
#pragma unroll
                    for (int qq = 0; qq < NEFES_SLAB_PIECES; ++qq)
                        if (piece_unit(qq) == uu) ring.store_piece(qq);
                }
                if (FIRST && !C0 && q == 0 && t + 1 < NT) {
                    acc[T0 + t + 1] = init(t + 1);
                }
                __builtin_amdgcn_sched_barrier(0);
                asm volatile("" ::"v"(B.l));
                if (vt) mfma_h3_asm_v(acc[T0 + t], h0, B.h);
                else mfma_h3_asm(acc[T0 + t], h0, B.h);
                __builtin_amdgcn_sched_barrier(0);
                if (host) src.stage_c1(Bn, pp, ps[pp]);
                if (!host) {
#pragma unroll
                    for (int qq = 0; qq < NEFES_SLAB_PIECES; ++qq)
                        if (piece_unit(qq) == uu) ring.fetch_piece(qq);
                }
                if (uu == acq_u) {
#pragma unroll
                    for (int qq = 0; qq < NEFES_SLAB_PIECES; ++qq)
                        if (piece_unit(qq) == uu && host) { ring.store_piece(qq); ring.fetch_piece(qq); }
                    ring.cur_off = ring.acquire();
                    p = ring_lane + ring.cur_off - (size_t)nu * 2048;
                    pn = p + (2 * uu + 4) * 1024;
                    h2 = *(const f32x4*)(pn);
                }
                l2 = *(const f32x4*)(pn + 1024);
                if (uu + 1 == nu) p = ring_lane + ring.cur_off;
                asm volatile("" ::"v"(h0), "v"(B.h));
                __builtin_amdgcn_sched_barrier(0);
            }
        }
    }
    ring.pf = HA(NU);
    asm volatile("s_nop 12\n\ts_nop 4"
                 : "+a"(acc[T0 + NT - 1]), "+a"(acc[T0 + NT - 2])
                 : "v"(HA(NU - 1)), "v"(BQ(KS16 - 1).h), "v"(BQ(KS16 - 1).l));
#pragma unroll
    for (int t = 0; t < VT; ++t)
        if (t >= T0 && t < T0 + NT) asm volatile("" : "+v"(acc[t]));
}

template <int NT, int KS16, int T0, bool FIRST = true, class SrcFn, class InitFn, int NACC, class Ring>
__device__ __forceinline__ void mma_run_h3_small(Ring& ring, const char* ring_lane, const SrcFn& src, const InitFn& init,
                                           f32x16 (&acc)[NACC]) {
    static_assert(T0 + NT <= NACC, "accumulator array too small");
    constexpr int UPS = (NEFES_SLAB_FRAGS / 4) / 2;
    constexpr int NU = KS16 * NT;
    constexpr int NSLAB = (NU + UPS - 1) / UPS;
    Split2 B, Bn;
    {
        PairRegs s0;
#pragma unroll
        for (int pp = 0; pp < 4; ++pp) {
            src.stage_a(s0, 0, pp);
            src.stage_b(s0);
            if (pp == 3) src.template stage_c<true>(B, pp, s0);
            else src.template stage_c<false>(B, pp, s0);
        }
    }
    Bn = B;
    if (FIRST) acc[T0] = init(0);
    const char* p = ring_lane + ring.cur_off;
    f32x4 ah = ring.pf, al = *(const f32x4*)(p + 1024);
#pragma unroll
    for (int sl = 0; sl < NSLAB; ++sl) {
        const int nu = (NU - sl * UPS) < UPS ? (NU - sl * UPS) : UPS;
#pragma unroll
        for (int uu = 0; uu < UPS; ++uu) {
            if (uu < nu) {
                const int u = sl * UPS + uu, q = u / NT, t = u % NT;
                f32x4 nh;
                const bool last = !(uu + 1 < nu);
                if (!last) {
                    nh = *(const f32x4*)(p + (2 * uu + 2) * 1024);
                } else {
#pragma unroll
                    for (int qq = 0; qq < NEFES_SLAB_PIECES; ++qq)
                        if ((qq * nu) / NEFES_SLAB_PIECES >= uu) ring.issue_piece(qq);
                    ring.cur_off = ring.acquire();
                    p = ring_lane + ring.cur_off;
                    nh = *(const f32x4*)(p);
                }
                if (t == 0 && q > 0) B = Bn;
                __builtin_amdgcn_sched_barrier(0);
                const f16x8 Ah = as_f16x8(ah), Al = as_f16x8(al);
                const f16x8 Bh = as_f16x8(B.h), Bl = as_f16x8(B.l);
                f32x16 c = acc[T0 + t];
                c = __builtin_amdgcn_mfma_f32_32x32x16_f16(Al, Bh, c, 0, 0, 0);
                al = *(const f32x4*)(p + (last ? 1 : 2 * uu + 3) * 1024);
                if (FIRST && q == 0 && t + 1 < NT) acc[T0 + t + 1] = init(t + 1);
                if (uu + 1 < nu) {
#pragma unroll
                    for (int qq = 0; qq < NEFES_SLAB_PIECES; ++qq)
                        if ((qq * nu) / NEFES_SLAB_PIECES == uu) {
                            __builtin_amdgcn_sched_barrier(0);
                            ring.issue_piece(qq);
                            __builtin_amdgcn_sched_barrier(0);
                        }
                }
                c = __builtin_amdgcn_mfma_f32_32x32x16_f16(Ah, Bl, c, 0, 0, 0);
                c = __builtin_amdgcn_mfma_f32_32x32x16_f16(Ah, Bh, c, 0, 0, 0);
                acc[T0 + t] = c;
                if (q + 1 < KS16) {
                    constexpr int STRIDE = NT >= 8 ? 2 : 1;
#pragma unroll
                    for (int pp = 0; pp < 4; ++pp)
                        if (NT >= 4 ? (t == pp * STRIDE + STRIDE - 1) : (t == (pp * NT) / 4)) {
                            PairRegs s1;
                            src.stage_a(s1, q + 1, pp);
                            src.stage_b(s1);
                            if (pp == 3) src.template stage_c<true>(Bn, pp, s1);
                            else src.template stage_c<false>(Bn, pp, s1);
#pragma unroll
                            for (int i = 0; i < 2; ++i) {
                                __builtin_amdgcn_sched_group_barrier(0x008, 1, 0);
                                __builtin_amdgcn_sched_group_barrier(0x002, 4, 0);
                            }
                        }
                }
                ah = nh;
            }
        }
    }
    ring.pf = ah;
    mfma_results_fence_tiles<12, NT, T0>(acc);
}

template <int NT, int KS16, int T0, bool FIRST = true, int VT = 0, bool ALLOW_WIDE = true, class SrcFn, class InitFn, int NACC, class Ring>
__device__ __forceinline__ void mma_run_h3(Ring& ring, const char* ring_lane, const SrcFn& src, const InitFn& init,
                                           f32x16 (&acc)[NACC]) {
    if constexpr (ALLOW_WIDE && NT >= NEFES_H3_WIDE_MIN && NT % 2 == 0 && NT <= NEFES_H3_WIDE_MAX) mma_run_h3_wide<NT, KS16, T0, FIRST, VT>(ring, ring_lane, src, init, acc);
    else mma_run_h3_small<NT, KS16, T0, FIRST>(ring, ring_lane, src, init, acc);
}
```

nefes_amd/csrc/field_h3_instances.h:

```cpp
#pragma once

#ifndef NEFES_TU_PART
#define NEFES_TU_PART 0
#endif
#if NEFES_TU_PART >= 2 && NEFES_TU_PART % 2 == 0
#define NEFES_TU_W128
#elif NEFES_TU_PART == 0 || NEFES_TU_PART == 1 || NEFES_TU_PART == 5 || NEFES_TU_PART == 9 || \
    NEFES_TU_PART == 11 || NEFES_TU_PART == 13
#define NEFES_TU_BWD_WIDE
#endif

#define NEFES_XYZ_HASHGRID_FUSED 2
#define NEFES_FIELD_FULL_FOLD 3
#define NEFES_H3B_FOLD 16

struct NefesH3FwdKey { int mode, enc, w, ntr, train, fh; };
struct NefesH3BwdKey { int w, kr16, enc, has_t, train, fh; };
inline bool operator==(const NefesH3FwdKey& a, const NefesH3FwdKey& b) {
    return a.mode == b.mode && a.enc == b.enc && a.w == b.w && a.ntr == b.ntr && a.train == b.train && a.fh == b.fh;
}
inline bool operator==(const NefesH3BwdKey& a, const NefesH3BwdKey& b) {
    return a.w == b.w && a.kr16 == b.kr16 && a.enc == b.enc && a.has_t == b.has_t && a.train == b.train && a.fh == b.fh;
}

#define NEFES_H3_FWD_INSTANCES(X)                                                                                                  \
    X(0, SIGMA, FREQ10, 256, 1, 0, 0)                                                                                              \
    X(0, FULL, FREQ10, 256, 1, 0, 0)                                                                                               \
    X(1, SIGMA, EXTERNAL32, 256, 1, 0, 0)                                                                                          \
    X(1, FULL, EXTERNAL32, 256, 1, 0, 0)                                                                                           \
                                                                                                            \
    X(1, STATIC, FREQ10, 256, 1, 0, 0)                                                                                             \
                                                                                       \
    X(1, SIGMA, HASHGRID_FUSED, 256, 1, 0, 0)                                                                                      \
    X(1, FULL, HASHGRID_FUSED, 256, 1, 0, 0)                                                                                       \
                                                     \
    X(2, SIGMA, FREQ10, 128, 5, 0, 0)                                                                                              \
    X(2, FULL, FREQ10, 128, 5, 0, 0)                                                                                               \
    X(2, STATIC, FREQ10, 128, 5, 0, 0)                                                                                             \
    X(3, STATIC, FREQ10, 256, 1, 1, 0)                                                                                             \
    X(3, FULL, FREQ10, 256, 1, 1, 0)                                                                                               \
                                                                                        \
    X(3, STATIC, EXTERNAL32, 256, 1, 1, 0)                                                                                         \
    X(3, FULL, EXTERNAL32, 256, 1, 1, 0)                                                                                           \
    X(4, STATIC, FREQ10, 128, 5, 1, 0)                                                                                             \
    X(4, FULL, FREQ10, 128, 5, 1, 0)                                                                                               \
                                                                            \
    X(5, FULL, FREQ10, 256, 5, 0, 0)                                                                                               \
    X(5, STATIC, FREQ10, 256, 5, 0, 0)                                                                                             \
    X(6, FULL, FREQ10, 128, 1, 0, 0)                                                                                               \
    X(6, STATIC, FREQ10, 128, 1, 0, 0)                                                                                             \
    X(6, FULL, FREQ10, 128, 1, 0, 1)                                                \
    X(7, STATIC, FREQ10, 256, 5, 1, 0)                                                                                             \
    X(7, FULL, FREQ10, 256, 5, 1, 0)                                                                                               \
    X(8, STATIC, FREQ10, 128, 1, 1, 0)                                                                                             \
    X(8, FULL, FREQ10, 128, 1, 1, 0)                                                                                               \
    X(9, FULL_FOLD, FREQ10, 256, 1, 0, 0)                                                                                          \
    X(11, FULL_FOLD, FREQ10, 256, 5, 0, 0)                                                                                         \
                                                            \
    X(13, FULL, EXTERNAL32, 256, 5, 0, 0)                                                                                          \
    NEFES_H3_FWD_HG_CLASS1(X)                                                                                                      \
    X(15, STATIC, EXTERNAL32, 256, 5, 1, 0)                                                                                        \
    X(15, FULL, EXTERNAL32, 256, 5, 1, 0)

#define NEFES_H3_BWD_INSTANCES(X)                                                                                                  \
    X(0, 256, 2, FREQ10, 1, 0, 0)                                                                                                  \
    X(1, 256, 2, EXTERNAL32, 1, 0, 0)                                                                                              \
    X(1, 256, 2, FREQ10, 0, 0, 0)                                                                                                  \
                                                                                                                         \
    X(1, 256, 2, HASHGRID_FUSED, 1, 0, 0)                                                                                          \
    X(2, 128, 9, FREQ10, 1, 0, 0)                                                                                                  \
    X(2, 128, 9, FREQ10, 0, 0, 0)                                                                                                  \
    X(3, 256, 2, FREQ10, 0, 1, 0)                                                                                                  \
    X(3, 256, 2, FREQ10, 1, 1, 0)                                                                                                  \
    X(3, 256, 2, EXTERNAL32, 0, 1, 0)                                                                     \
    X(3, 256, 2, EXTERNAL32, 1, 1, 0)                                                                                              \
    X(4, 128, 9, FREQ10, 0, 1, 0)                                                                                                  \
    X(4, 128, 9, FREQ10, 1, 1, 0)                                                                                                  \
    X(5, 256, 9, FREQ10, 1, 0, 0)                                                                                                  \
    X(5, 256, 9, FREQ10, 0, 0, 0)                                                                                                  \
    X(6, 128, 2, FREQ10, 1, 0, 0)                                                                                                  \
    X(6, 128, 2, FREQ10, 0, 0, 0)                                                                                                  \
    X(6, 128, 2, FREQ10, 1, 0, 1)                                                                               \
    X(7, 256, 9, FREQ10, 0, 1, 0)                                                                                                  \
    X(7, 256, 9, FREQ10, 1, 1, 0)                                                                                                  \
    X(8, 128, 2, FREQ10, 0, 1, 0)                                                                                                  \
    X(8, 128, 2, FREQ10, 1, 1, 0)                                                                                                  \
    X(9, 256, 2 | NEFES_H3B_FOLD, FREQ10, 1, 0, 0)                                                                                 \
    X(11, 256, 9 | NEFES_H3B_FOLD, FREQ10, 1, 0, 0)                                                                                \
                                                                          \
    X(13, 256, 9, EXTERNAL32, 1, 0, 0)                                                                                             \
    NEFES_H3_BWD_HG_CLASS1(X)                                                                                                      \
    X(15, 256, 9, EXTERNAL32, 0, 1, 0)                                                                                             \
    X(15, 256, 9, EXTERNAL32, 1, 1, 0)

#ifdef NEFES_H3_HG_CLASS1
#define NEFES_H3_FWD_HG_CLASS1(X) X(13, FULL, HASHGRID_FUSED, 256, 5, 0, 0)
#define NEFES_H3_BWD_HG_CLASS1(X) X(13, 256, 9, HASHGRID_FUSED, 1, 0, 0)
#else
#define NEFES_H3_FWD_HG_CLASS1(X)
#define NEFES_H3_BWD_HG_CLASS1(X)
#endif

#define NEFES_H3_PASTE_(a, b) a##b
#define NEFES_H3_PASTE(a, b) NEFES_H3_PASTE_(a, b)
#define NEFES_H3_FWD_PART_FN(part) NEFES_H3_PASTE(nefes_fwd_h3_launch_part, part)
#define NEFES_H3_BWD_PART_FN(part) NEFES_H3_PASTE(nefes_bwd_h3_launch_part, part)

#define NEFES_H3_FWD_KEY(MODE, ENC, W, NTR, TRAIN, FH) NefesH3FwdKey{NEFES_FIELD_##MODE, NEFES_XYZ_##ENC, W, NTR, TRAIN, FH}
#define NEFES_H3_BWD_KEY(W, KR16, ENC, HAS_T, TRAIN, FH) NefesH3BwdKey{W, KR16, NEFES_XYZ_##ENC, HAS_T, TRAIN, FH}
```

nefes_amd/csrc/layout.h:

```cpp
#pragma once
#include <stdint.h>

#if defined(__HIP__)
#define NEFES_HD __host__ __device__ inline __attribute__((always_inline))
#else
#define NEFES_HD inline
#endif

#ifndef NEFES_FWD_SLAB_KIB
#define NEFES_FWD_SLAB_KIB 32
#endif
#ifndef NEFES_BWD_SLAB_KIB
#define NEFES_BWD_SLAB_KIB 32
#endif
#define NEFES_FRAGS_OF_KIB(kib) ((kib) * 4)
#define NEFES_SLAB_BYTES (NEFES_SLAB_KIB * 1024)
#define NEFES_SLAB_FRAGS NEFES_FRAGS_OF_KIB(NEFES_SLAB_KIB)
#define NEFES_SLAB_PIECES (NEFES_SLAB_BYTES / 4096)
#define NEFES_RING_SLOTS (128 / NEFES_FWD_SLAB_KIB)
#define NEFES_BWD_SLOTS (96 / NEFES_BWD_SLAB_KIB)
#define NEFES_N_FREQ_XYZ 10
#define NEFES_N_FREQ_DIR 4
#define NEFES_E_STEPS 32
#define NEFES_D_STEPS 14
#define NEFES_X_STEPS 16

NEFES_HD int nefes_rho(int h, int r) { return (r & 3) + 8 * (r >> 2) + 4 * h; }
NEFES_HD int nefes_row_reg(int i) { return (i & 3) + 4 * (i >> 3); }
NEFES_HD int nefes_row_half(int i) { return (i >> 2) & 1; }
NEFES_HD int nefes_nat_slot(int s, int h) { return 32 * (s >> 4) + nefes_rho(h, s & 15); }
NEFES_HD int nefes_emb_slot(int L, int s, int h) {
    if (s < 3 * L) return 3 + 6 * (s / 3) + 3 * h + (s % 3);
    if (s == 3 * L) return h;
    if (s == 3 * L + 1) return h == 0 ? 2 : -1;
    return -1;
}
NEFES_HD int nefes_head_class(int C) { return C < 0 ? -1 : (3 + C <= 32 ? 0 : (3 + C <= 144 ? 1 : -1)); }
NEFES_HD int nefes_head_ntr(int C) { return 3 + C <= 32 ? 1 : 5; }
NEFES_HD int nefes_head_kr16(int C) { return 3 + C <= 32 ? 2 : 9; }
#define NEFES_HEAD_MAX_C 141
NEFES_HD int nefes_steps_per_slab(int nt, int slab_frags) { return slab_frags / nt; }
NEFES_HD int nefes_segment_slabs(int nt, int ks, int slab_frags) {
    const int sps = slab_frags / nt;
    return (ks + sps - 1) / sps;
}

enum { NEFES_STREAM_FWD_SIGMA = 0, NEFES_STREAM_FWD_STATIC = 1, NEFES_STREAM_FWD_FULL = 2, NEFES_STREAM_BWD_FULL = 3,
       NEFES_STREAM_FWD_SIGMA_X6 = 4, NEFES_STREAM_FWD_FULL_X6 = 5, NEFES_STREAM_BWD_FULL_X6 = 6, NEFES_STREAM_BWD_STATIC = 7,
       NEFES_STREAM_FWD_SIGMA_H3 = 8, NEFES_STREAM_FWD_FULL_H3 = 9, NEFES_STREAM_BWD_FULL_H3 = 10,
       NEFES_STREAM_FWD_STATIC_H3 = 11, NEFES_STREAM_BWD_STATIC_H3 = 12,
       NEFES_N_STREAMS = 13 };
#define NEFES_X6_SLAB_KIB 48
#define NEFES_H3_FWD_SLAB_KIB 32
#define NEFES_H3_FWD_SLAB_KIB_128 16
#define NEFES_H3_BWD_SLAB_KIB 32
#define NEFES_H3_BWD_SLAB_KIB_128 16
#define NEFES_H3_TARGET_EXP 14
NEFES_HD int nefes_stream_slab_kib(int stream, int width) {
    if (stream == NEFES_STREAM_BWD_FULL || stream == NEFES_STREAM_BWD_FULL_X6 || stream == NEFES_STREAM_BWD_STATIC) return NEFES_BWD_SLAB_KIB;
    if (stream == NEFES_STREAM_BWD_FULL_H3 || stream == NEFES_STREAM_BWD_STATIC_H3) return width == 128 ? NEFES_H3_BWD_SLAB_KIB_128 : NEFES_H3_BWD_SLAB_KIB;
    if (stream == NEFES_STREAM_FWD_SIGMA_H3 || stream == NEFES_STREAM_FWD_FULL_H3 || stream == NEFES_STREAM_FWD_STATIC_H3)
        return width == 128 ? NEFES_H3_FWD_SLAB_KIB_128 : NEFES_H3_FWD_SLAB_KIB;
    return stream >= NEFES_STREAM_FWD_SIGMA_X6 ? NEFES_X6_SLAB_KIB : NEFES_FWD_SLAB_KIB;
}
#define NEFES_PACK_KEEP 0xffffffffu
#define NEFES_BLOB_HEADER_BYTES 512

enum { NEFES_H3F_L1 = 0, NEFES_H3F_L2, NEFES_H3F_L3, NEFES_H3F_L4, NEFES_H3F_L5H, NEFES_H3F_L5E, NEFES_H3F_L6, NEFES_H3F_L7,
       NEFES_H3F_L8, NEFES_H3F_SIG, NEFES_H3F_FINAL, NEFES_H3F_DT_H, NEFES_H3F_DT_D, NEFES_H3F_RGB, NEFES_H3F_T1, NEFES_H3F_T2,
       NEFES_H3F_TH, NEFES_H3F_N };
NEFES_HD int nefes_h3_tab_exp(int seg) { return 2 * seg; }
NEFES_HD int nefes_h3_tab_bound(int seg) { return 2 * seg + 1; }
NEFES_HD int nefes_h3_tab_bias(int n_segs, int block) { return 2 * n_segs + block; }
enum { NEFES_H3BB_L1 = 0, NEFES_H3BB_SIG = 8, NEFES_H3BB_FINAL, NEFES_H3BB_DIR, NEFES_H3BB_RGB, NEFES_H3BB_T0, NEFES_H3BB_T1,
       NEFES_H3BB_T2, NEFES_H3BB_TH };
enum { NEFES_H3B_RGB = 0, NEFES_H3B_TH, NEFES_H3B_T2, NEFES_H3B_T1, NEFES_H3B_T0, NEFES_H3B_DIR, NEFES_H3B_FINAL, NEFES_H3B_SIG,
       NEFES_H3B_L8, NEFES_H3B_L7, NEFES_H3B_L6, NEFES_H3B_L5, NEFES_H3B_L4, NEFES_H3B_L3, NEFES_H3B_L2, NEFES_H3B_L1,
       NEFES_H3B_N };
#define NEFES_H3F_N_STATIC (NEFES_H3F_RGB + 1)
#define NEFES_H3B_N_STATIC (NEFES_H3B_N - 4)
NEFES_HD int nefes_h3b_seg(int has_transient, int seg) { return (has_transient || seg == NEFES_H3B_RGB) ? seg : seg - 4; }
enum { NEFES_H3FF_SIG = NEFES_H3F_SIG, NEFES_H3FF_DT_H, NEFES_H3FF_DT_D, NEFES_H3FF_RGB, NEFES_H3FF_T1, NEFES_H3FF_T2, NEFES_H3FF_TH,
       NEFES_H3FF_N };
enum { NEFES_H3FBB_SIG = NEFES_H3BB_SIG, NEFES_H3FBB_DIR, NEFES_H3FBB_RGB, NEFES_H3FBB_T0, NEFES_H3FBB_T1, NEFES_H3FBB_T2, NEFES_H3FBB_TH };
enum { NEFES_H3BF_RGB = 0, NEFES_H3BF_TH, NEFES_H3BF_T2, NEFES_H3BF_T1, NEFES_H3BF_T0, NEFES_H3BF_DIR, NEFES_H3BF_SIG, NEFES_H3BF_L8,
       NEFES_H3BF_L7, NEFES_H3BF_L6, NEFES_H3BF_L5, NEFES_H3BF_L4, NEFES_H3BF_L3, NEFES_H3BF_L2, NEFES_H3BF_L1, NEFES_H3BF_N };
#define NEFES_H3FF_N_STATIC (NEFES_H3FF_RGB + 1)
#define NEFES_H3BF_N_STATIC (NEFES_H3BF_N - 4)
NEFES_HD int nefes_h3f_seg(int fold, int seg) { return (fold && seg > NEFES_H3F_FINAL) ? seg - 1 : seg; }
NEFES_HD int nefes_h3f_bias(int fold, int block) { return (fold && block > NEFES_H3BB_FINAL) ? block - 1 : block; }
NEFES_HD int nefes_h3b_fold_seg(int fold, int seg) { return (fold && seg > NEFES_H3B_FINAL) ? seg - 1 : seg; }
static_assert(NEFES_H3FF_DT_H == NEFES_H3F_DT_H - 1 && NEFES_H3FF_TH == NEFES_H3F_TH - 1 && NEFES_H3FBB_DIR == NEFES_H3BB_DIR - 1 &&
              NEFES_H3FBB_TH == NEFES_H3BB_TH - 1 && NEFES_H3BF_SIG == NEFES_H3B_SIG - 1 && NEFES_H3BF_L1 == NEFES_H3B_L1 - 1,
              "folded ordinals = the unfolded ones with FINAL taken out");

NEFES_HD int nefes_mask_words(int W) { return 8 * (W / 64) + 4 * (W / 128); }

enum { NEFES_TB_E = 0, NEFES_TB_DV = 1, NEFES_TB_L1 = 2 , NEFES_TB_FINAL = 10, NEFES_TB_DIR = 11,
       NEFES_TB_T0 = 12, NEFES_TB_T1 = 13, NEFES_TB_T2 = 14, NEFES_TB_RGB = 15, NEFES_TB_SIG = 16, NEFES_TB_TH = 17,
       NEFES_TB_END = 18 };
NEFES_HD size_t nefes_train_off(int row, int sample) {
    return ((size_t)(row >> 5) * 8 + (size_t)(sample >> 4)) * 512 + (size_t)(row & 31) * 16 + (size_t)(sample & 15);
}
NEFES_HD uint32_t nefes_train_lane_off(int wave, int j, int h) { return (uint32_t)(((wave * 32 + j) >> 4) * 512 + 4 * h * 16 + (j & 15)); }
NEFES_HD int nefes_train_row(int W, int C, int block) {
    const int ntr = nefes_head_ntr(C);
    int r = 0;
    if (block == NEFES_TB_E) return r;
    r += 2 * NEFES_E_STEPS;
    if (block == NEFES_TB_DV) return r;
    r += 32;
    if (block >= NEFES_TB_L1 && block <= NEFES_TB_FINAL) return r + (block - NEFES_TB_L1) * W;
    r += 9 * W;
    if (block >= NEFES_TB_DIR && block <= NEFES_TB_T2) return r + (block - NEFES_TB_DIR) * (W / 2);
    r += 4 * (W / 2);
    if (block == NEFES_TB_RGB) return r;
    r += 32 * ntr;
    if (block == NEFES_TB_SIG) return r;
    r += 32;
    if (block == NEFES_TB_TH) return r;
    return r + 32;
}
```

nefes_amd/lib.py:

```python
import ctypes as C
import os

import torch

_HERE = os.path.dirname(os.path.abspath(__file__))
LIB_PATH = os.environ.get("NEFES_HIP_LIB") or os.path.join(_HERE, "libnefes_hip.so")


class NefesNetDesc(C.Structure):
    _fields_ = [("width", C.c_int32), ("feat_dim", C.c_int32), ("has_transient", C.c_int32), ("xyz_encoding", C.c_int32),
                ("fold_final", C.c_int32)]


class NefesGenericNetDesc(C.Structure):
    _fields_ = [("width", C.c_int32), ("depth", C.c_int32), ("skip", C.c_int32), ("feat_dim", C.c_int32), ("has_transient", C.c_int32),
                ("xyz_encoding", C.c_int32)]


class NefesStreamInfo(C.Structure):
    _fields_ = [("slab_off", C.c_uint64), ("n_slabs", C.c_uint32), ("bias_floats", C.c_uint32), ("bias_off", C.c_uint64),
                ("scale_off", C.c_uint32), ("scale_count", C.c_uint32)]


class NefesBlobInfo(C.Structure):
    _fields_ = [("total_bytes", C.c_uint64), ("stream", NefesStreamInfo * 13)]


class NefesTrainLossDesc(C.Structure):
    _fields_ = [("N", C.c_int32), ("C", C.c_int32), ("S", C.c_int32), ("feat_kind", C.c_int32), ("present", C.c_uint32),
                ("coef", C.c_float), ("lambda_u", C.c_float), ("sigma_row_stride", C.c_int64)]


class NefesHashGridDesc(C.Structure):
    _fields_ = [("n_levels", C.c_int32), ("n_features", C.c_int32), ("log2_hashmap_size", C.c_int32),
                ("base_resolution", C.c_int32), ("per_level_scale", C.c_float), ("bound", C.c_float)]


ABI_VERSION = 20
STREAM_FWD_SIGMA, STREAM_FWD_STATIC, STREAM_FWD_FULL, STREAM_BWD_FULL, STREAM_FWD_SIGMA_X6, STREAM_FWD_FULL_X6, STREAM_BWD_FULL_X6, STREAM_BWD_STATIC = 0, 1, 2, 3, 4, 5, 6, 7
STREAM_FWD_SIGMA_H3, STREAM_FWD_FULL_H3, STREAM_BWD_FULL_H3, STREAM_FWD_STATIC_H3, STREAM_BWD_STATIC_H3 = 8, 9, 10, 11, 12
FIELD_SIGMA, FIELD_STATIC, FIELD_FULL = 0, 1, 2
XYZ_FREQ10, XYZ_EXTERNAL32 = 0, 1
H3_REQ_TRAIN, H3_REQ_EXT, H3_REQ_HASHGRID, H3_REQ_FH, H3_REQ_ZROW, H3_REQ_STATIC_BWD = 1, 2, 4, 8, 16, 32
(TB_E, TB_DV, TB_L1, TB_FINAL, TB_DIR, TB_T0, TB_T1, TB_T2, TB_RGB, TB_SIG, TB_TH, TB_END) = (0, 1, 2, 10, 11, 12, 13, 14, 15, 16,
                                                                                              17, 18)
COMP_TRANSIENT, COMP_STATIC_ONLY, COMP_SIGMA_ONLY, COMP_WHITE_BKGD, COMP_FEAT_WEIGHTS_ONLY = 1, 2, 4, 8, 16

TRAIN_LOSS_ROWS = 16
LOSS_FEAT_MSE, LOSS_FEAT_L1, LOSS_FEAT_COS = 0, 1, 2
(LOSS_HAS_RGB_FINE, LOSS_HAS_RGB_COARSE, LOSS_HAS_BETA, LOSS_HAS_FEAT_FINE, LOSS_HAS_FEAT_COARSE, LOSS_HAS_FEAT_FUSION,
 LOSS_NERFW) = 1, 2, 4, 8, 16, 32, 64

_p, _i, _f, _u32, _sz = C.c_void_p, C.c_int, C.c_float, C.c_uint32, C.c_size_t
_desc = C.POINTER(NefesNetDesc)
_gdesc = C.POINTER(NefesGenericNetDesc)

SIGNATURES = {
    "nefes_version": (_i, []),
    "nefes_blob_info": (_i, [_desc, C.POINTER(NefesBlobInfo)]),
    "nefes_stream_slab_bytes": (_sz, [_desc, _i]),
    "nefes_fusion_input_fwd": (_i, [_i, _i, _i, _p, _p, _p, C.POINTER(_f), C.POINTER(_f), _p, _p, _p]),
    "nefes_fusion_input_bwd": (_i, [_i, _i, _i, _p, _p, _p, C.POINTER(_f), _p, _p, _p]),
    "nefes_upcos_loss_fwd": (_i, [_i, _i, _i, _i, _i, _i, _p, _p, _p, _p, _p]),
    "nefes_upcos_loss_bwd": (_i, [_i, _i, _i, _i, _i, _i, _p, _p, _p, _p, _p, _p, _p, _p, _p, _p, _i, _p, _p, _p]),
    "nefes_bicubic_gather_table": (_i, [_i, _i, _i, _i, _i, _p, _p, _p, _p]),
    "nefes_bicubic_gram": (_i, [_i, _i, _i, _i, _p, _p]),
    "nefes_bn_train_fwd": (_i, [_i, _i, C.c_int64, _i, _p, _p, _p, C.c_double, C.c_double, _p, _p, _p, _p, _p, _p]),
    "nefes_bn_train_bwd": (_i, [_i, _i, C.c_int64, _i, _p, _p, _p, _p, _p, _p]),
    "nefes_bn_train_bwd_affine": (_i, [_i, _i, C.c_int64, _p, _p, _p, _p, _p, _p, _p, _p]),
    "nefes_svd_reg_fwd": (_i, [_i, _p, _p, _p, _p]),
    "nefes_svd_reg_bwd": (_i, [_i, _p, _p, _p, _p]),
    "nefes_regressed_pose_fwd": (_i, [_i, _p, _i, _f, _f, _f, _f, _p, _p, _p]),
    "nefes_regressed_pose_bwd": (_i, [_i, _p, _i, _f, _p, _p, _p]),
    "nefes_upcos_prepare": (_i, [_i, _i, _i, _i, _i, _i, _p, _p, _p, _p, _p, _p, _p, _i, _p, _p, _p, _p]),
    "nefes_upcos_gram_fwd": (_i, [_i, _i, _i, _p, _p, _p, _p, _p, _i, _p, _p, _p, _p]),
    "nefes_upcos_gram_bwd": (_i, [_i, _i, _i, _p, _p, _p, _p, _p, _p]),
    "nefes_upcos_gram_lds_bytes": (_sz, [_i, _i, _i]),
    "nefes_adam_step": (_i, [_i, _p, _p, _p, _p, _p, _p, C.c_double, C.c_double, C.c_double, _p]),
    "nefes_pack_weights": (_i, [_desc, C.POINTER(_p), _i, _p, _sz]),
    "nefes_pack_map": (_i, [_desc, _p, _sz, _p]),
    "nefes_pack_h3_plan": (_i, [_desc, _p, _sz, C.POINTER(_sz)]),
    "nefes_pack_device": (_i, [_p, C.c_int64, _p, C.c_int64, _p, _i, _p, _p, _p]),
    "nefes_raygen_fwd": (_i, [_i, _i, _f, _p, _i, _i, _p, _p, _p, _p]),
    "nefes_raygen_bwd_workspace": (_sz, [_i]),
    "nefes_raygen_bwd": (_i, [_i, _i, _f, _p, _i, _i, _p, _p, _p, _p, _p, _p]),
    "nefes_raygen_k_fwd": (_i, [_i, _i, _p, _p, _i, _i, _p, _p, _p, _p]),
    "nefes_raygen_k_bwd_workspace": (_sz, [_i]),
    "nefes_raygen_k_bwd": (_i, [_i, _i, _p, _p, _i, _i, _p, _p, _p, _p, _p, _p, _p]),
    "nefes_raygen_px_fwd": (_i, [_i, _p, _p, _p, _p, _p, _p, _p]),
    "nefes_raygen_px_bwd_workspace": (_sz, [_i]),
    "nefes_raygen_px_bwd": (_i, [_i, _p, _p, _p, _p, _p, _p, _p, _p, _p, _p]),
    "nefes_sample_px": (_i, [_i, _i, _i, _p, _i, _p, _p, _p]),
    "nefes_ndc_fwd": (_i, [_i, _i, _f, _f, _i, _p, _p, _p, _p, _p]),
    "nefes_ndc_bwd": (_i, [_i, _i, _f, _f, _i, _p, _p, _p, _p, _p, _p, _p]),
    "nefes_coarse_depths": (_i, [_i, _i, _f, _f, _i, _p, _p, _p, _p]),
    "nefes_coarse_depths_rays": (_i, [_i, _i, _p, _i, _i, _p, _p, _p, _p]),
    "nefes_field_mask_bytes": (_sz, [_desc, C.c_int64]),
    "nefes_field_fwd": (_i, [_desc, _p, _i, _i, _i, _p, _p, _p, _p, _p, _p, _p, _p, _p]),
    "nefes_field_bwd": (_i, [_desc, _p, _i, _i, _p, _p, _p, _p, _p, _p, _p, _p, _p, _p, _p, _p]),
    "nefes_ray_grad_reduce": (_i, [_i, _i, _p, _p, _p, _p, _p, _p, _p]),
    "nefes_composite_fwd": (_i, [_i, _i, _i, _u32, _f, _p, _p, _p, _p, _p, _p, _p, _p, _p, _p]),
    "nefes_composite_bwd": (_i, [_i, _i, _i, _u32, _p, _p, _p, _p, _p, _p, _p, _p, _p, _p, _p]),
    "nefes_hashgrid_table_entries": (_sz, [C.POINTER(NefesHashGridDesc)]),
    "nefes_hashgrid_fwd": (_i, [C.POINTER(NefesHashGridDesc), _p, C.c_int64, _p, _p, _p]),
    "nefes_hashgrid_bwd_x": (_i, [C.POINTER(NefesHashGridDesc), _p, C.c_int64, _p, _p, _p, _p]),
    "nefes_hashgrid_bwd_table_workspace": (_sz, [C.POINTER(NefesHashGridDesc)]),
    "nefes_hashgrid_bwd_table": (_i, [C.POINTER(NefesHashGridDesc), C.c_int64, _p, _p, _p, _p, _p]),
    "nefes_field_bwd_static": (_i, [_desc, _p, _i, _i, _p, _p, _p, _p, _p, _p, _p, _p, _p, _p, _p]),
    "nefes_field_bwd_x6": (_i, [_desc, _p, _i, _i, _p, _p, _p, _p, _p, _p, _p, _p, _p, _p, _p, _p]),
    "nefes_field_fwd_x6": (_i, [_desc, _p, _i, _i, _i, _p, _p, _p, _p, _p, _p, _p, _p, _p]),
    "nefes_field_bwd_h3": (_i, [_desc, _p, _i, _i, _p, _p, _p, _p, _p, _p, _p, _p, _p, _p, _p, _p]),
    "nefes_field_bwd_static_h3": (_i, [_desc, _p, _i, _i, _p, _p, _p, _p, _p, _p, _p, _p, _p, _p, _p]),
    "nefes_field_h3_instance": (_i, [_desc, _i, _i, C.c_uint, C.c_char_p, _sz]),
    "nefes_feat_head_fwd": (_i, [_i, _i, _i, _p, _p, _p, _p, _p]),
    "nefes_feat_head_bwd": (_i, [_i, _i, _i, _p, _p, _p, _p, _p]),
    "nefes_field_fwd_h3_fh": (_i, [_desc, _p, _i, _i, _i, _p, _p, _p, _p, _p, _p, _p]),
    "nefes_field_bwd_h3_fh": (_i, [_desc, _p, _i, _i, _p, _p, _p, _p, _p, _p, _p, _p, _p, _p, _p]),
    "nefes_field_fwd_h3_hashgrid": (_i, [_desc, _p, C.POINTER(NefesHashGridDesc), _p, _i, _i, _i, _p, _p, _p, _i, _p, _p, _p, _p]),
    "nefes_field_bwd_h3_hashgrid": (_i, [_desc, _p, C.POINTER(NefesHashGridDesc), _p, _i, _i, _p, _p, _p, _p, _p, _p, _p, _p, _p, _p]),
    "nefes_field_fwd_h3": (_i, [_desc, _p, _i, _i, _i, _p, _p, _p, _p, _p, _p, _p, _p, _p]),
    "nefes_field_fwd_h3_zrow": (_i, [_desc, _p, _i, _i, _i, _p, _p, _p, _p, _p, _p, _p]),
    "nefes_coarse_sample": (_i, [_i, _i, _i, _p, _p, _i, _p, _i, _p, _p, _p, _p]),
    "nefes_conv2d_same": (_i, [_i, _i, _i, _i, _i, _i, _p, _p, _p, _p, _i, _p, _p]),
    "nefes_conv2d_wgrad_workspace": (_sz, [_i, _i, _i, _i, _i, _i]),
    "nefes_conv2d_wgrad": (_i, [_i, _i, _i, _i, _i, _i, _p, _p, _p, _p, _p, _p, _p]),
    "nefes_probe_mfma_clock": (_i, [_i, _i, C.POINTER(C.c_double), C.POINTER(C.c_double), _p]),
    "nefes_probe_store_hazard": (_i, [_p, C.c_int64, _i, _p]),
    "nefes_probe_pk_mul": (_i, [_p, C.c_int64, _i, _p]),
    "nefes_probe_hazard": (_i, [_i, _i, _i, _i, _p, _p]),
    "nefes_probe_aggressor": (_i, [_i, _i, _i, _p, _p]),
    "nefes_generic_blob_bytes": (_sz, [_gdesc]),
    "nefes_generic_pack": (_i, [_gdesc, C.POINTER(_p), _i, _p, _sz]),
    "nefes_generic_mask_bytes": (_sz, [_gdesc, C.c_int64]),
    "nefes_field_fwd_generic": (_i, [_gdesc, _p, _i, _i, _i, _p, _p, _p, _p, _p, _p, _p, _p]),
    "nefes_field_bwd_generic": (_i, [_gdesc, _p, _i, _i, _i, _p, _p, _p, _p, _p, _p, _p, _p, _p, _p, _p]),
    "nefes_field_fwd_generic_ext": (_i, [_gdesc, _p, _i, _i, _i, _p, _p, _p, _p, _p]),
    "nefes_field_bwd_generic_ext": (_i, [_gdesc, _p, _i, _i, _i, _p, _p, _p, _p, _p, _p, _p]),
    "nefes_generic_pack_device": (_i, [_gdesc, C.POINTER(_p), _i, _p, _sz, _p]),
    "nefes_generic_train_rows": (_sz, [_gdesc]),
    "nefes_generic_train_row_offset": (_i, [_gdesc, _i]),
    "nefes_field_fwd_train_generic": (_i, [_gdesc, _p, _i, _i, _i, _p, _p, _p, _p, _p, _p, _p, _p]),
    "nefes_field_bwd_train_generic": (_i, [_gdesc, _p, _i, _i, _i, _p, _p, _p, _p, _p, _p, _p, _p, _p, _p, _p]),
    "nefes_generic_train_rows_ext": (_sz, [_gdesc]),
    "nefes_generic_train_row_offset_ext": (_i, [_gdesc, _i]),
    "nefes_field_fwd_train_generic_ext": (_i, [_gdesc, _p, _i, _i, _i, _p, _p, _p, _p, _p, _p]),
    "nefes_field_bwd_train_generic_ext": (_i, [_gdesc, _p, _i, _i, _i, _p, _p, _p, _p, _p, _p, _p, _p]),
    "nefes_train_rows": (_sz, [_desc]),
    "nefes_train_row_offset": (_i, [_desc, _i]),
    "nefes_field_fwd_train": (_i, [_desc, _p, _i, _i, _i, _p, _p, _p, _p, _p, _p, _p, _p, _p]),
    "nefes_field_fwd_train_h3": (_i, [_desc, _p, _i, _i, _i, _p, _p, _p, _p, _p, _p, _p, _p, _p]),
    "nefes_field_bwd_train": (_i, [_desc, _p, _i, _i, _i, _p, _p, _p, _p, _p, _p, _p, _p, _p, _p, _p]),
    "nefes_field_bwd_train_h3": (_i, [_desc, _p, _i, _i, _i, _p, _p, _p, _p, _p, _p, _p, _p, _p, _p, _p]),
    "nefes_field_fwd_train_h3_ext": (_i, [_desc, _p, _i, _i, _i, _p, _p, _p, _p, _p, _p]),
    "nefes_field_bwd_train_h3_ext": (_i, [_desc, _p, _i, _i, _i, _p, _p, _p, _p, _p, _p, _p, _p]),
    "nefes_train_head_grad": (_i, [_desc, _i, _i, _i, _p, _p, _p, _p]),
    "nefes_train_dx": (_i, [C.c_int64, _i, _p, _i, _i, _p, _i, _i, _p, _i, _i, _i, _p, _p]),
    "nefes_train_dw": (_i, [C.c_int64, _i, _p, _i, _i, _p, _i, _i, _i, _i, _p, _p]),
    "nefes_train_dw_bias": (_i, [C.c_int64, _i, _p, _i, _i, _p, _i, _i, _i, _i, C.c_int64, _p, _p]),
    "nefes_bicubic_up_fwd": (_i, [C.c_int64, _i, _i, _i, _i, _i, _i, _i, _i, _p, _p, _p]),
    "nefes_bicubic_up_bwd": (_i, [C.c_int64, _i, _i, _i, _i, _i, _i, _i, _i, _p, _p, _p, _p]),
    "nefes_pose_compose_fwd": (_i, [_i, _p, _p, _p, C.c_float, C.POINTER(C.c_float), C.c_float, _p, _p]),
    "nefes_pose_compose_bwd": (_i, [_i, _p, _p, _p, C.c_float, C.POINTER(C.c_float), C.c_float, _p, _p, _p, _p]),
    "nefes_psnr_ssim_workspace": (_sz, [_i, _i, _i]),
    "nefes_psnr_ssim": (_i, [_i, _i, _i, _p, C.c_int64, C.c_int64, _p, C.c_int64, C.c_int64, _p, _p, _p]),
    "nefes_cosine_loss_scratch_doubles": (_sz, [_i]),
    "nefes_cosine_loss_fwd": (_i, [_i, C.c_int64, _p, _p, _p, _p, _p]),
    "nefes_cosine_loss_bwd": (_i, [_i, C.c_int64, _p, _p, _p, _p, _p, _p]),
    "nefes_pixcos_scratch_doubles": (_sz, [_i, C.c_int64]),
    "nefes_pixcos_loss_fwd": (_i, [_i, _i, C.c_int64, _p, _p, _p, _p, _p]),
    "nefes_pixcos_loss_bwd": (_i, [_i, _i, C.c_int64, _p, _p, _p, _p, _p, _p]),
    "nefes_uppixcos_scratch_doubles": (_sz, [_i, _i, _i, _i]),
    "nefes_uppixcos_loss_fwd": (_i, [_i, _i, _i, _i, _i, _i, _i, _p, _p, _p, _p, _p]),
    "nefes_uppixcos_loss_bwd": (_i, [_i, _i, _i, _i, _i, _i, _i, _p, _p, _p, _p, _p, _p, _p, _p, _p, _p, _i, _p, _p, _p]),
    "nefes_cosine_loss_masked_fwd": (_i, [_i, _i, C.c_int64, _p, _p, _p, _p, _p, _p]),
    "nefes_cosine_loss_masked_bwd": (_i, [_i, _i, C.c_int64, _p, _p, _p, _p, _p, _p, _p]),
    "nefes_upcos_loss_masked_fwd": (_i, [_i, _i, _i, _i, _i, _i, _i, _p, _p, _p, _p, _p, _p]),
    "nefes_upcos_loss_masked_bwd": (_i, [_i, _i, _i, _i, _i, _i, _i, _p, _p, _p, _p, _p, _p, _p, _p, _p, _p, _p, _i, _p, _p, _p]),
    "nefes_pixcos_masked_scratch_doubles": (_sz, [_i, C.c_int64]),
    "nefes_pixcos_loss_masked_fwd": (_i, [_i, _i, C.c_int64, _p, _p, _p, _p, _p, _p]),
    "nefes_pixcos_loss_masked_bwd": (_i, [_i, _i, C.c_int64, _p, _p, _p, _p, _p, _p, _p]),
    "nefes_uppixcos_masked_scratch_doubles": (_sz, [_i, _i, _i, _i]),
    "nefes_uppixcos_loss_masked_fwd": (_i, [_i, _i, _i, _i, _i, _i, _i, _p, _p, _p, _p, _p, _p]),
    "nefes_uppixcos_loss_masked_bwd": (_i, [_i, _i, _i, _i, _i, _i, _i, _p, _p, _p, _p, _p, _p, _p, _p, _p, _p, _p, _i, _p, _p, _p]),
    "nefes_train_loss_scratch_doubles": (_sz, [_i]),
    "nefes_train_loss_fwd": (_i, [C.POINTER(NefesTrainLossDesc)] + [_p] * 13),
    "nefes_train_loss_bwd": (_i, [C.POINTER(NefesTrainLossDesc)] + [_p] * 20),
    "nefes_sample_pdf_merge": (_i, [_i, _i, _i, _i, _p, _p, _p, _i, _p, _p, _p, _p, _p, _p]),
}

_lib = None


def load():
    global _lib
    if _lib is not None:
        return _lib
    if not os.path.exists(LIB_PATH):
        raise RuntimeError(
            f"{LIB_PATH} not found: build it with `python -c 'import __graft_entry__ as g; g.build()'` "
            "or `make -C nefes_amd/csrc`. nefes_amd has no CPU or PyTorch fallback for the hot path.")
    lib = C.CDLL(LIB_PATH)
    for name, (res, args) in SIGNATURES.items():
        fn = getattr(lib, name)
        fn.restype = res
        fn.argtypes = args
    if lib.nefes_version() != ABI_VERSION:
        raise RuntimeError("libnefes_hip.so ABI version mismatch")
    _lib = lib
    return lib


COMPILED_SET = ("fp16 two-part instances (default): widths 128 / 256 x feature heads of 0..29 or 30..141 channels with the frequency "
                "embedding, width 256 x 0..29 or 30..141 channels with an external 32-feature embedding (hash grid); bf16x6 and fp32-MFMA instances "
                "(NEFES_SPLIT=x6 / f32): width 256 x 16 channels and width 128 x 128 channels only")
GENERIC_SET = ("generic fp32-MFMA kernels (frequency embedding: frozen weights, or train mode with NEFES_GENERIC_TRAIN=1; an external "
               "32-feature embedding (hash grid): frozen weights only, the table may train -- or train mode with "
               "NEFES_GENERIC_TRAIN_EXT=1): any width that is "
               "a multiple of 32 from 32 to 512, depth 1..8 with skips=[4] (or none when depth <= 4), feature heads of 1..141 channels")
COMPILED_SET += ".  Other shapes (NeRFH_NFF.packed_generic): " + GENERIC_SET


def check(rc, what):
    if rc != 0:
        kind = {-1: "bad argument", -2: "unsupported configuration", -3: "bad weight blob"}.get(rc, f"hipError {rc}")
        raise RuntimeError(f"{what} failed: {kind}" + (f".  Compiled: {COMPILED_SET}" if rc == -2 else ""))
```

nefes_amd/ops.py:

```python
import collections
import ctypes as C
from typing import Optional

import os

import torch

from . import lib as L


def _stream():
    return C.c_void_p(torch.cuda.current_stream().cuda_stream)


TIMERS = None


class _timed:

    def __init__(self, name):
        self.name = name

    def __enter__(self):
        if TIMERS is not None and self.name is not None:
# ... 141 lines not shown
    return g, gk


class RayGenK(torch.autograd.Function):

    @staticmethod
    def forward(ctx, c2w, intr, H, W, row0, nrows):
        o, d, v = raygen_k_fwd(H, W, intr, c2w, row0, nrows)
        ctx.save_for_backward(c2w, intr)
        ctx.geom = (H, W, row0, nrows)
        return o, d, v

    @staticmethod
    def backward(ctx, g_o, g_d, g_v):
        c2w, intr = ctx.saved_tensors
        H, W, row0, nrows = ctx.geom
        g, gk = raygen_k_bwd(H, W, intr, c2w, row0, nrows, g_o, g_d, g_v, want_intr=ctx.needs_input_grad[1])
        if not (tuple(c2w.shape) == (3, 4) and c2w.dtype == torch.float32):
            out = torch.zeros_like(c2w)
            out[:3, :4] = g
            g = out
        return g, gk, None, None, None, None


def as_pixels(x, device):
    dev = torch.device(device)
    if torch.is_tensor(x):
        ok_shape = x.dim() == 2 and x.shape[1] == 2 and x.shape[0] > 0
        here = x.device.type == dev.type and (dev.index is None or x.device.index == dev.index)
        if here and x.dtype == torch.float32 and ok_shape and x.is_contiguous():
            return x
        integer = not (x.dtype.is_floating_point or x.dtype.is_complex or x.dtype == torch.bool)
        if ok_shape and integer:
            return x.detach().to(dev, torch.float32).contiguous()
        if x.device.type != "cpu":
            raise ValueError(f"nefes_amd: pixels on a device must be a contiguous float32 (or an integer) [K, 2] tensor of (x, y) on {dev}; got "
                             f"{x.dtype} {tuple(x.shape)} on {x.device}")
    import numpy as np
    a = np.asarray(x.detach().numpy() if torch.is_tensor(x) else x, dtype=np.float64)
    if a.ndim != 2 or a.shape[1] != 2 or a.shape[0] == 0:
        raise ValueError(f"nefes_amd: pixels must be [K, 2] rows of (x, y) = (column, row); got shape {a.shape}")
    if not np.isfinite(a).all():
        k = int(np.argwhere(~np.isfinite(a))[0][0])
        raise ValueError(f"nefes_amd: pixel {k} = ({float(a[k, 0])!r}, {float(a[k, 1])!r}) is not finite")
    return torch.tensor(np.ascontiguousarray(a), dtype=torch.float32, device=dev)


def _px(px):
    if px.dim() != 2 or px.shape[1] != 2 or px.shape[0] == 0:
        raise RuntimeError(f"nefes_amd: `px` must be [K, 2] rows of (x, y); got {tuple(px.shape)}")
    return _chk(px.detach(), "px")


def raygen_px_fwd(px, intr, c2w):
    c2w = _f32(c2w[:3, :4])
    n = px.shape[0]
    o = torch.empty(n, 3, device=c2w.device)
    d = torch.empty_like(o)
    v = torch.empty_like(o)
    L.check(L.load().nefes_raygen_px_fwd(n, _px(px), _intr(intr), _chk(c2w, "c2w"), _chk(o, "o"), _chk(d, "d"), _chk(v, "v"), _stream()),
            "nefes_raygen_px_fwd")
    return o, d, v


def raygen_px_bwd(px, intr, c2w, g_o, g_d, g_v, want_intr=True):
    lib = L.load()
    c2w = _f32(c2w[:3, :4])
    n = px.shape[0]
    ws = torch.empty(lib.nefes_raygen_px_bwd_workspace(n), dtype=torch.uint8, device=c2w.device)
    g = torch.empty(3, 4, device=c2w.device)
    gk = torch.empty(4, device=c2w.device) if want_intr else None
    fix = lambda t: None if t is None else _f32(t)
    g_o, g_d, g_v = fix(g_o), fix(g_d), fix(g_v)
    L.check(lib.nefes_raygen_px_bwd(n, _px(px), _intr(intr), _chk(c2w, "c2w"), _chk(g_o, "g_o"), _chk(g_d, "g_d"), _chk(g_v, "g_v"),
                                    _chk(ws, "ws", torch.uint8), _chk(g, "g_c2w"), _chk(gk, "g_intr"), _stream()), "nefes_raygen_px_bwd")
    return g, gk


class RayGenPx(torch.autograd.Function):

    @staticmethod
    def forward(ctx, c2w, intr, px):
        o, d, v = raygen_px_fwd(px, intr, c2w)
        ctx.save_for_backward(c2w, intr, px)
        return o, d, v

    @staticmethod
    def backward(ctx, g_o, g_d, g_v):
        c2w, intr, px = ctx.saved_tensors
        g, gk = raygen_px_bwd(px, intr, c2w, g_o, g_d, g_v, want_intr=ctx.needs_input_grad[1])
        if not (tuple(c2w.shape) == (3, 4) and c2w.dtype == torch.float32):
            out = torch.zeros_like(c2w)
            out[:3, :4] = g
            g = out
        return g, gk, None


def sample_pixels(map, px, out=None):
    if map.dim() != 3:
        raise RuntimeError(f"nefes_amd: sample_pixels: `map` must be [C, H, W]; got {tuple(map.shape)}")
    Cc, H, W = (int(v) for v in map.shape)
    n = px.shape[0]
    if out is None:
        out = torch.empty(Cc, n, device=map.device)
    elif tuple(out.shape) != (Cc, n):
        raise RuntimeError(f"nefes_amd: sample_pixels: `out` must be [{Cc}, {n}]; got {tuple(out.shape)}")
    L.check(L.load().nefes_sample_px(Cc, H, W, _chk(map.detach(), "map"), n, _px(px), _chk(out, "out"), _stream()), "nefes_sample_px")
    return out


class NdcRays(torch.autograd.Function):

    @staticmethod
    def forward(ctx, rays_o, rays_d, H, W, focal, near):
        o, d = _f32(rays_o).reshape(-1, 3), _f32(rays_d).reshape(-1, 3)
        oo, od = torch.empty_like(o), torch.empty_like(d)
        L.check(L.load().nefes_ndc_fwd(H, W, float(focal), float(near), o.shape[0], _chk(o, "o"), _chk(d, "d"),
                                       _chk(oo, "oo"), _chk(od, "od"), _stream()), "nefes_ndc_fwd")
        ctx.save_for_backward(o, d)
        ctx.geom = (H, W, focal, near, rays_o.shape)
        return oo.reshape(rays_o.shape), od.reshape(rays_d.shape)

    @staticmethod
    def backward(ctx, g_oo, g_od):
        o, d = ctx.saved_tensors
        H, W, focal, near, shape = ctx.geom
        go, gd = torch.empty_like(o), torch.empty_like(d)
        g_oo = None if g_oo is None else _f32(g_oo).reshape(-1, 3)
        g_od = None if g_od is None else _f32(g_od).reshape(-1, 3)
        L.check(L.load().nefes_ndc_bwd(H, W, float(focal), float(near), o.shape[0], _chk(o, "o"), _chk(d, "d"),
                                       _chk(g_oo, "g_oo"), _chk(g_od, "g_od"), _chk(go, "go"), _chk(gd, "gd"), _stream()),
                "nefes_ndc_bwd")
        return go.reshape(shape), gd.reshape(shape), None, None, None, None


_LINSPACE = {}


def _linspace01(n, device):
    key = (int(n), str(device))
    t = _LINSPACE.get(key)
    if t is None:
        t = _LINSPACE[key] = torch.linspace(0., 1., steps=int(n), device=device)
    return t


def coarse_depths(N, Nc, near, far, lindisp=False, t_rand=None, device="cuda", bounds=None):
    t = _linspace01(Nc, device)
    z = torch.empty(N, Nc, device=device)
    t_rand = None if t_rand is None else _f32(t_rand)
    if bounds is not None:
        if not (bounds.is_cuda and bounds.dtype == torch.float32 and bounds.dim() == 2 and bounds.shape[0] == N
                and bounds.shape[1] >= 2 and bounds.stride(1) == 1):
            raise RuntimeError("nefes_amd: `bounds` must be a float32 CUDA tensor [N, >=2] with unit column stride")
        L.check(L.load().nefes_coarse_depths_rays(N, Nc, C.c_void_p(bounds.data_ptr()), int(bounds.stride(0)),
                                                  int(bool(lindisp)), _chk(t, "t"), _chk(t_rand, "t_rand"), _chk(z, "z"),
                                                  _stream()), "nefes_coarse_depths_rays")
        return z
    L.check(L.load().nefes_coarse_depths(N, Nc, float(near), float(far), int(bool(lindisp)), _chk(t, "t"),
                                         _chk(t_rand, "t_rand"), _chk(z, "z"), _stream()), "nefes_coarse_depths")
    return z


_ZROW = {}
_ZROW_MAX = 64


def coarse_depth_row(Nc, near, far, lindisp=False, device="cuda"):
    key = (int(Nc), float(near), float(far), bool(lindisp), str(device))
    z = _ZROW.get(key)
    if z is not None:
        _ZROW[key] = _ZROW.pop(key)
        return z
    z = coarse_depths(1, Nc, near, far, lindisp, None, device=device).reshape(-1)
    if not torch.cuda.is_current_stream_capturing():
        _ZROW[key] = z
        while len(_ZROW) > _ZROW_MAX:
            _ZROW.pop(next(iter(_ZROW)))
    return z


def fused_coarse_pass_ok(pk, Nc, Ni, N=0, grid=None):
    enc_ok = pk.xyz_encoding == L.XYZ_FREQ10 if grid is None else hashgrid_fused_ok(pk, grid)
    return (FUSED_COARSE and h3_serves(pk) and enc_ok and Nc in (64, 128, 256)
            and Ni > 0 and Nc + Ni <= 512 and N * Nc < H3_MAX_SAMPLES)


def field_sigma_row(pk, rays_o, rays_d, z_row, grid=None):
    rays_o, rays_d = _f32(rays_o), _f32(rays_d)
    return _field_fwd(pk, L.FIELD_SIGMA, rays_o.shape[0], z_row.numel(), rays_o=rays_o, rays_d=rays_d, z=z_row, grid=grid)[0]


def coarse_sample(sigma, z, Ni, u=None, want_samples=True, want_weights=False):
    sigma, z = _f32(sigma), _f32(z)
    N, Nc = sigma.shape[0], sigma.shape[-1]
    dev = sigma.device
    if u is None:
        u = _linspace01(Ni, dev)
    u = _f32(u)
    z_fine = torch.empty(N, Nc + Ni, device=dev)
    z_samples = torch.empty(N, Ni, device=dev) if want_samples else None
    weights = torch.empty(N, Nc, device=dev) if want_weights else None
    with _timed("coarse_sample"):
        L.check(L.load().nefes_coarse_sample(N, Nc, Ni, _chk(sigma, "sigma"), _chk(z, "z"), 1 if z.dim() == 1 else 0, _chk(u, "u"),
                                             1 if u.dim() == 2 else 0, _chk(z_fine, "z_fine"), _chk(z_samples, "z_samples"),
                                             _chk(weights, "weights"), _stream()), "nefes_coarse_sample")
    _tap("z_fine", z_fine)
    _tap("z_samples", z_samples)
    return (z_fine, z_samples, weights) if want_weights else (z_fine, z_samples)


class PackedField:

    LAYERS_COARSE = [f"xyz_encoding_{i}.0" for i in range(1, 9)] + ["xyz_encoding_final", "dir_encoding.0",
                                                                    "static_sigma.0", "static_rgb.0"]
    LAYERS_FINE = LAYERS_COARSE + ["transient_encoding.0", "transient_encoding.2", "transient_encoding.4",
                                   "transient_sigma.0", "transient_rgb.0", "transient_beta.0"]

    def __init__(self, state_dict, width, feat_dim, has_transient, device, xyz_encoding=0, fold_final=False):
        lib = L.load()
        self.desc = L.NefesNetDesc(int(width), int(feat_dim), 1 if has_transient else 0, int(xyz_encoding), 1 if fold_final else 0)
        self.fold = bool(fold_final)
        self.xyz_encoding = int(xyz_encoding)
        self.width, self.feat_dim, self.has_transient = int(width), int(feat_dim), bool(has_transient)
        info = L.NefesBlobInfo()
        L.check(lib.nefes_blob_info(self.desc, info), "nefes_blob_info")
        names = self.LAYERS_FINE if has_transient else self.LAYERS_COARSE
        host = []
        for n in names:
            host.append(state_dict[n + ".weight"].detach().to("cpu", torch.float32).contiguous())
            host.append(state_dict[n + ".bias"].detach().to("cpu", torch.float32).contiguous())
        ptrs = (C.c_void_p * len(host))(*[t.data_ptr() for t in host])
        blob = torch.zeros(info.total_bytes, dtype=torch.uint8)
        L.check(lib.nefes_pack_weights(self.desc, ptrs, len(host), C.c_void_p(blob.data_ptr()), blob.numel()),
                "nefes_pack_weights")
        self.blob = blob.to(device)
        self.info = info
        self.generation = 0
        self.h3_valid = True
        self._map = None

    def repack(self, params):
        lib = L.load()
        if self.fold:
            raise RuntimeError("nefes_amd: a folded pack (fold_final) holds products of parameters and is not re-packed on the device; "
                               "trainable networks take NeRFH_NFF.packed()")
        if self._map is None:
            n = self.info.total_bytes // 2
            host_map = torch.zeros(n, dtype=torch.int32)
            elems = (C.c_int64 * 36)()
            L.check(lib.nefes_pack_map(self.desc, C.c_void_p(host_map.data_ptr()), n, C.cast(elems, C.c_void_p)), "nefes_pack_map")
            self._map = host_map.to(self.blob.device)
            self._elems = list(elems)[:36 if self.has_transient else 24]
            need = C.c_size_t(0)
            L.check(lib.nefes_pack_h3_plan(self.desc, None, 0, C.byref(need)), "nefes_pack_h3_plan")
            plan = torch.zeros(int(need.value), dtype=torch.int32)
            L.check(lib.nefes_pack_h3_plan(self.desc, C.c_void_p(plan.data_ptr()), plan.numel(), None), "nefes_pack_h3_plan")
            self._plan_jobs = int(plan[0])
            self._plan = plan.to(self.blob.device)
            self._plan_scratch = torch.zeros(32, dtype=torch.int32, device=self.blob.device)
        if [int(p.numel()) for p in params] != self._elems:
            raise RuntimeError("nefes_amd: parameter shapes do not match the packed network description")
        flat = torch.cat([p.detach().reshape(-1) for p in params]).to(torch.float32)
        h3 = REPACK_H3 and self._plan_jobs > 0
        L.check(lib.nefes_pack_device(flat.data_ptr(), flat.numel(), self._map.data_ptr(), self._map.numel(),
                                      self._plan.data_ptr() if h3 else None, self._plan_jobs if h3 else 0,
                                      self._plan_scratch.data_ptr() if h3 else None, self.blob.data_ptr(), _stream()),
                "nefes_pack_device")
        self.generation += 1
        if not h3:
            self.h3_valid = False

    def h3_byte_ranges(self):
        out = []
        for k in (L.STREAM_FWD_SIGMA_H3, L.STREAM_FWD_FULL_H3, L.STREAM_BWD_FULL_H3, L.STREAM_FWD_STATIC_H3, L.STREAM_BWD_STATIC_H3):
            si = self.info.stream[k]
            if si.n_slabs:
                slab = int(L.load().nefes_stream_slab_bytes(self.desc, k))
                out.append((int(si.slab_off), int(si.slab_off + si.n_slabs * slab)))
                out.append((int(si.bias_off + 4 * si.scale_off), int(si.bias_off + 4 * si.bias_floats)))
        return out

    def check_generation(self, gen):
        if gen != self.generation:
            raise RuntimeError("nefes_amd: the network weights were modified (re-packed) between this forward pass and its "
                               "backward pass")

    def mask_bytes(self, M):
        return L.load().nefes_field_mask_bytes(self.desc, M)

    def train_rows(self):
        lib = L.load()
        return int(lib.nefes_train_rows(self.desc)), [int(lib.nefes_train_row_offset(self.desc, b)) for b in range(L.TB_END + 1)]

    def n_raw(self, mode):
        return 1 if mode == L.FIELD_SIGMA else (3 + self.feat_dim + (1 if mode == L.FIELD_STATIC else 6))


SPLIT = os.environ.get("NEFES_SPLIT", "h3")
REPACK_H3 = os.environ.get("NEFES_REPACK_H3", "1") != "0"
USE_X6 = os.environ.get("NEFES_X6", "1") != "0"
FUSED_COARSE = os.environ.get("NEFES_FUSED_COARSE", "1") != "0"
FOLD_FINAL = os.environ.get("NEFES_FOLD_FINAL", "1") != "0"
FACTORED_HEAD = os.environ.get("NEFES_FACTORED_HEAD", "1") != "0"
FIELD_GENERIC = os.environ.get("NEFES_FIELD_GENERIC", "0") == "1"
FUSED_HASHGRID = os.environ.get("NEFES_FUSED_HASHGRID", "1") != "0"

FUSION_TRAIN = os.environ.get("NEFES_HIP_FUSION_TRAIN", "0") == "1"


HEAD_MAX_C = 141
COMPILED_SET = L.COMPILED_SET
H3_MAX_SAMPLES = (1 << 31) - 256
MODE_NAMES = ("sigma", "static", "full")


def head_class(C):
    return -1 if C < 0 else (0 if 3 + C <= 32 else (1 if 3 + C <= 144 else -1))


def canonical_shape(pk):
    return (pk.width == 256 and pk.feat_dim == 16) or (pk.width == 128 and pk.feat_dim == 128 and pk.xyz_encoding == L.XYZ_FREQ10)


def h3_shape(pk):
    cls = head_class(pk.feat_dim)
    if pk.width not in (128, 256) or cls < 0:
        return False
    return True if pk.xyz_encoding == L.XYZ_FREQ10 else pk.width == 256


def _h3(pk):
    if SPLIT not in ("h3", "x6", "f32"):
        raise ValueError("nefes_amd.ops.SPLIT must be 'h3', 'x6' or 'f32'")
    return SPLIT == "h3" and pk.h3_valid


def h3_serves(pk):
    return _h3(pk) and h3_shape(pk)


def static_h3(pk):
    return h3_serves(pk) and pk.xyz_encoding == L.XYZ_FREQ10


def _has_instance(pk):
    return canonical_shape(pk) or h3_serves(pk)


def x6_supported(pk, mode):
    if mode == L.FIELD_STATIC:
        return static_h3(pk)
    return _has_instance(pk) and (mode == L.FIELD_SIGMA or (mode == L.FIELD_FULL and pk.has_transient))


def require_instance(pk, what):
    if _has_instance(pk):
        return
    raise RuntimeError(f"nefes_amd: no kernel instance serves {what} for W={pk.width}, f_dim={pk.feat_dim}, "
                       f"xyz_encoding={pk.xyz_encoding} with NEFES_SPLIT={SPLIT}"
                       f"{'' if pk.h3_valid else ' (fp16 streams stale: NEFES_REPACK_H3=0)'}.  Compiled: {COMPILED_SET}")


def fold_shape(width, feat_dim, xyz_encoding=L.XYZ_FREQ10):
    return width == 256 and head_class(feat_dim) >= 0 and xyz_encoding == L.XYZ_FREQ10


def fold_serves(width, feat_dim, xyz_encoding):
    return FOLD_FINAL and SPLIT == "h3" and USE_X6 and not FIELD_GENERIC and fold_shape(width, feat_dim, xyz_encoding)


def factored_head_serves(width, feat_dim):
    return FACTORED_HEAD and SPLIT == "h3" and not FIELD_GENERIC and width == 128 and 3 + feat_dim > 3 + width // 2 + 1


def is_generic(pk):
    return bool(getattr(pk, "generic", False))


def hashgrid_fused_ok(pk, grid):
    return (FUSED_HASHGRID and isinstance(grid, HashGrid) and h3_serves(pk) and pk.xyz_encoding == L.XYZ_EXTERNAL32
            and head_class(pk.feat_dim) == 0 and grid.desc.n_levels == 16 and grid.desc.n_features == 2)


Route = collections.namedtuple("Route", "entry key label g_enc")


def field_route(pk, mode, backward=False, kind="rays", M=0, override=None):
    name = MODE_NAMES[mode]
    d = "bwd" if backward else "fwd"
    switched = USE_X6 and SPLIT != "f32"
    route = lambda entry, key, g_enc=False: Route(entry, key, entry, g_enc)
    gen_ext = is_generic(pk) and pk.xyz_encoding == L.XYZ_EXTERNAL32
    if is_generic(pk) and (kind == "enc") != gen_ext:
        raise RuntimeError(f"nefes_amd: the generic field kernels of W={pk.width}, D={pk.depth}, f_dim={pk.feat_dim} were packed for "
                           f"{'a supplied 32-feature encoding' if gen_ext else 'the frequency embedding'} (xyz_encoding={pk.xyz_encoding}) "
                           f"and cannot take input of kind '{kind}'")
    if kind in ("hashgrid", "zrow"):
        if M >= H3_MAX_SAMPLES:
            raise RuntimeError("nefes_amd: too many samples for one launch of the fp16 two-part kernels (32-bit sample index)")
        if kind == "zrow":
            return route("nefes_field_fwd_h3_zrow", "field_fwd[sigma,h3]")
        if backward:
            return route("nefes_field_bwd_h3_hashgrid", "field_bwd[h3,hashgrid]")
        if mode == L.FIELD_STATIC:
            raise NotImplementedError("nefes_amd: the hash-grid field kernels evaluate the sigma-only or the full head")
        return route("nefes_field_fwd_h3_hashgrid", f"field_fwd[{name},h3,hashgrid]")
    if is_generic(pk):
        if gen_ext:
            return route(f"nefes_field_{d}_generic_ext", f"field_{d}[{name},generic,ext]", backward)
        return route(f"nefes_field_{d}_generic", f"field_{d}[{name},generic]")
    fold = getattr(pk, "fold", False)
    if not backward:
        if override is None:
            split = switched and x6_supported(pk, mode) and (kind != "points" or pk.xyz_encoding == L.XYZ_FREQ10)
        else:
            split = override == "split"
        if split:
            h3 = h3_serves(pk) and M < H3_MAX_SAMPLES
            if h3 or mode != L.FIELD_STATIC:
                if not h3 and not canonical_shape(pk):
                    raise RuntimeError(f"nefes_amd: {M} samples in one launch exceed the fp16 two-part kernels' 32-bit sample index and "
                                       f"W={pk.width}, f_dim={pk.feat_dim} has no other instance; render fewer rays per launch")
                if fold and not (h3 and mode == L.FIELD_FULL):
                    raise RuntimeError("nefes_amd: a folded pack serves the full pass on the fp16 two-part kernels only")
                return route("nefes_field_fwd_h3" if h3 else "nefes_field_fwd_x6",
                             f"field_fwd[{name},{'h3' if h3 else 'x6'}{',fold' if fold else ''}]")
        if not canonical_shape(pk):
            raise RuntimeError(f"nefes_amd: the {name} forward of W={pk.width}, f_dim={pk.feat_dim} was routed to "
                               f"the fp32-MFMA instances (NEFES_SPLIT={SPLIT}; or a frozen network's static head with test_time=False), "
                               f"which exist for the canonical shapes only.  Compiled: {COMPILED_SET}")
        return route("nefes_field_fwd", f"field_fwd[{name}]")
    if mode == L.FIELD_STATIC:
        if switched and static_h3(pk) and M < H3_MAX_SAMPLES:
            return route("nefes_field_bwd_static_h3", "field_bwd[static,h3]")
        if not canonical_shape(pk):
            raise RuntimeError(f"nefes_amd: the static-head backward of W={pk.width}, f_dim={pk.feat_dim} was routed to the fp32-MFMA "
                               f"instances (NEFES_SPLIT={SPLIT}), which exist for the canonical shapes only.  Compiled: {COMPILED_SET}")
        return route("nefes_field_bwd_static", "field_bwd[static]")
    ext = pk.xyz_encoding == L.XYZ_EXTERNAL32
    if switched and x6_supported(pk, L.FIELD_FULL):
        h3 = _h3(pk)
        if fold and not h3:
            raise RuntimeError("nefes_amd: a folded pack serves the fp16 two-part kernels only")
        return route("nefes_field_bwd_h3" if h3 else "nefes_field_bwd_x6",
                     ("field_bwd[h3,fold]" if fold else "field_bwd[h3]") if h3 else "field_bwd[x6]", ext)
    return route("nefes_field_bwd", "field_bwd", ext)


def _blob(pk):
    return _chk(pk.blob, "blob", torch.uint8)


def _alloc_masks(pk, M, dev, want):
    return torch.empty(pk.mask_bytes(M) // 4, dtype=torch.int32, device=dev) if want else None


def _tap_masks(pk, masks, N, S, mode):
    if masks is not None and is_generic(pk):
        _tap("masks_generic", (masks, N, S, pk, mode))
    elif masks is not None:
        _tap("masks", (masks, N, S, pk.width, mode))


def _input_kind(z, pts, xyz_enc, grid):
    if grid is not None:
        return "hashgrid"
    if z is not None and z.dim() == 1:
        return "zrow"
    return "points" if pts is not None else ("enc" if xyz_enc is not None else "rays")


def _field_fwd(pk, mode, N, S, rays_o=None, rays_d=None, z=None, pts=None, xyz_enc=None, viewdirs=None, want_masks=False, grid=None,
               override=None):
    rt = field_route(pk, mode, False, _input_kind(z, pts, xyz_enc, grid), N * S, override)
    dev = pk.blob.device
    raw_t = torch.empty(N, pk.n_raw(mode), S, device=dev)
    masks = _alloc_masks(pk, N * S, dev, want_masks)
    o, d, zz, v = _chk(rays_o, "rays_o"), _chk(rays_d, "rays_d"), _chk(z, "z"), _chk(viewdirs, "viewdirs")
    if rt.entry == "nefes_field_fwd_generic":
        args = (mode, N, S, o, d, zz, _chk(pts, "pts"), v)
    elif rt.entry == "nefes_field_fwd_generic_ext":
        args = (mode, N, S, _chk(xyz_enc, "xyz_enc"), v)
    elif rt.entry == "nefes_field_fwd_h3_hashgrid":
        args = (grid.desc, _chk(grid.table, "table"), mode, N, S, o, d, zz, 1 if z.dim() == 1 else 0, v)
    elif rt.entry == "nefes_field_fwd_h3_zrow":
        args = (mode, N, S, o, d, zz, v)
    else:
        args = (mode, N, S, o, d, zz, _chk(pts, "pts"), _chk(xyz_enc, "xyz_enc"), v)
    with _timed(rt.key):
        L.check(getattr(L.load(), rt.entry)(pk.desc, _blob(pk), *args, _chk(raw_t, "raw_t"), _chk(masks, "masks", torch.int32), _stream()),
                rt.label)
    _tap_masks(pk, masks, N, S, mode)
    return raw_t, masks


def _field_bwd(pk, mode, N, S, raw_t, g_raw_t, masks, rays_o=None, rays_d=None, z=None, pts=None, viewdirs=None, grid=None, enc=False):
    rt = field_route(pk, mode, True, _input_kind(z, pts, True if enc else None, grid), N * S)
    dev = pk.blob.device
    g_in, g_vs = torch.empty(N * S, 32 if rt.g_enc else 3, device=dev), torch.empty(N * S, 3, device=dev)
    o, d, zz, v = _chk(rays_o, "rays_o"), _chk(rays_d, "rays_d"), _chk(z, "z"), _chk(viewdirs, "viewdirs")
    out = (_chk(raw_t, "raw_t"), _chk(g_raw_t, "g_raw_t"), _chk(masks, "masks", torch.int32))
    if rt.entry == "nefes_field_bwd_generic":
        args = (mode, N, S, o, d, zz, _chk(pts, "pts"), v, *out, _chk(g_in, "g_pts"))
    elif rt.entry == "nefes_field_bwd_generic_ext":
        args = (mode, N, S, v, *out, _chk(g_in, "g_enc"))
    elif rt.entry == "nefes_field_bwd_h3_hashgrid":
        args = (grid.desc, _chk(grid.table, "table"), N, S, o, d, zz, v, *out, _chk(g_in, "g_pts"))
    elif rt.entry.startswith("nefes_field_bwd_static"):
        args = (N, S, o, d, zz, _chk(pts, "pts"), v, *out, _chk(g_in, "g_pts"))
    else:
        args = (N, S, o, d, zz, _chk(pts, "pts"), v, *out, None if rt.g_enc else _chk(g_in, "g_pts"), _chk(g_in, "g_enc") if rt.g_enc else None)
    with _timed(rt.key):
        L.check(getattr(L.load(), rt.entry)(pk.desc, _blob(pk), *args, _chk(g_vs, "g_vs"), _stream()), rt.label)
    return g_in, g_vs


def field_fwd(pk, mode, N, S, rays_o=None, rays_d=None, z=None, pts=None, viewdirs=None, want_masks=False, xyz_enc=None):
    return _field_fwd(pk, mode, N, S, rays_o, rays_d, z, pts, xyz_enc, viewdirs, want_masks, override="f32")


def field_fwd_x6(pk, mode, N, S, rays_o=None, rays_d=None, z=None, viewdirs=None, want_masks=False, xyz_enc=None, pts=None):
    return _field_fwd(pk, mode, N, S, rays_o, rays_d, z, pts, xyz_enc, viewdirs, want_masks, override="split")


def field_bwd(pk, N, S, raw_t, g_raw_t, masks, rays_o=None, rays_d=None, z=None, pts=None, viewdirs=None, mode=L.FIELD_FULL):
    return _field_bwd(pk, mode, N, S, raw_t, g_raw_t, masks, rays_o, rays_d, z, pts, viewdirs)


def field_fwd_generic(pk, mode, N, S, rays_o=None, rays_d=None, z=None, pts=None, viewdirs=None, want_masks=False):
    return _field_fwd(pk, mode, N, S, rays_o, rays_d, z, pts, None, viewdirs, want_masks)


def field_bwd_generic(pk, mode, N, S, raw_t, g_raw_t, masks, rays_o=None, rays_d=None, z=None, pts=None, viewdirs=None):
    return _field_bwd(pk, mode, N, S, raw_t, g_raw_t, masks, rays_o, rays_d, z, pts, viewdirs)


def ray_grad_reduce(N, S, z, g_pts, g_vs):
    dev = g_pts.device
    g_o, g_d, g_v = (torch.empty(N, 3, device=dev) for _ in range(3))
    with _timed("ray_grad_reduce"):
      L.check(L.load().nefes_ray_grad_reduce(N, S, _chk(z, "z"), _chk(g_pts, "g_pts"), _chk(g_vs, "g_vs"), _chk(g_o, "g_o"),
                                           _chk(g_d, "g_d"), _chk(g_v, "g_v"), _stream()), "nefes_ray_grad_reduce")
    return g_o, g_d, g_v


_NO_SIGMA_BWD = ("nefes_amd: the sigma-only field pass has no backward (the reference evaluates it without gradients at test time: "
                 "nerfh_nff.py:192-202)")


class FieldFromRays(torch.autograd.Function):

    @staticmethod
    def forward(ctx, rays_o, rays_d, viewdirs, z, pk, mode):
        rays_o, rays_d, viewdirs, z = _f32(rays_o), _f32(rays_d), _f32(viewdirs), _f32(z)
        N, S = z.shape
        need = mode in (L.FIELD_FULL, L.FIELD_STATIC) and any(ctx.needs_input_grad[:3])
        raw_t, masks = _field_fwd(pk, mode, N, S, rays_o=rays_o, rays_d=rays_d, z=z, viewdirs=viewdirs, want_masks=need)
        ctx.pk, ctx.mode, ctx.have, ctx.pk_gen = pk, mode, need, pk.generation
        if need:
            ctx.save_for_backward(rays_o, rays_d, viewdirs, z, raw_t, masks)
        return raw_t

    @staticmethod
    def backward(ctx, g_raw_t):
        if not ctx.have:
            raise NotImplementedError(_NO_SIGMA_BWD)
        rays_o, rays_d, viewdirs, z, raw_t, masks = ctx.saved_tensors
        N, S = z.shape
        ctx.pk.check_generation(ctx.pk_gen)
        g_pts, g_vs = _field_bwd(ctx.pk, ctx.mode, N, S, raw_t, _f32(g_raw_t), masks, rays_o=rays_o, rays_d=rays_d, z=z, viewdirs=viewdirs)
        g_o, g_d, g_v = ray_grad_reduce(N, S, z, g_pts, g_vs)
        return g_o, g_d, g_v, None, None, None


class FeatHead(torch.autograd.Function):

    @staticmethod
    def forward(ctx, gmap, w, w_t, b):
        gmap = _f32(gmap)
        N, F1 = gmap.shape
        C = w.shape[0]
        feat = torch.empty(N, C, device=gmap.device)
        with _timed("feat_head_fwd"):
            L.check(L.load().nefes_feat_head_fwd(N, C, F1 - 1, _chk(gmap, "gmap"), _chk(w_t, "w_t"), _chk(b, "b"), _chk(feat, "feat"), _stream()),
                    "nefes_feat_head_fwd")
        ctx.save_for_backward(w, b)
        ctx.F1 = F1
        return feat

    @staticmethod
    def backward(ctx, g_feat):
        w, b = ctx.saved_tensors
        g_feat = _f32(g_feat)
        N, C = g_feat.shape
        g_gmap = torch.empty(N, ctx.F1, device=g_feat.device)
        with _timed("feat_head_bwd"):
            L.check(L.load().nefes_feat_head_bwd(N, C, ctx.F1 - 1, _chk(g_feat, "g_feat"), _chk(w, "w"), _chk(b, "b"), _chk(g_gmap, "g_gmap"),
                                                 _stream()), "nefes_feat_head_bwd")
        return g_gmap, None, None, None


def _fh_fwd(pk, rays_o, rays_d, viewdirs, z, want_masks):
    N, S = z.shape
    raw_t = torch.empty(N, 3 + pk.width // 2 + 1 + 6, S, device=z.device)
    masks = _alloc_masks(pk, N * S, z.device, want_masks)
    with _timed("field_fwd[full,h3,fh]"):
        L.check(L.load().nefes_field_fwd_h3_fh(pk.desc, _blob(pk), L.FIELD_FULL, N, S, _chk(rays_o, "rays_o"), _chk(rays_d, "rays_d"),
                                               _chk(z, "z"), _chk(viewdirs, "viewdirs"), _chk(raw_t, "raw_t"),
                                               _chk(masks, "masks", torch.int32), _stream()), "nefes_field_fwd_h3_fh")
    _tap_masks(pk, masks, N, S, L.FIELD_FULL)
    return raw_t, masks


def _fh_bwd(pk, rays_o, rays_d, viewdirs, z, raw_t, g_raw_t, g_gmap, masks):
    N, S = z.shape
    g_pts, g_vs = torch.empty(N * S, 3, device=z.device), torch.empty(N * S, 3, device=z.device)
    with _timed("field_bwd[h3,fh]"):
        L.check(L.load().nefes_field_bwd_h3_fh(pk.desc, _blob(pk), N, S, _chk(rays_o, "rays_o"), _chk(rays_d, "rays_d"), _chk(z, "z"),
                                               _chk(viewdirs, "viewdirs"), _chk(raw_t, "raw_t"), _chk(g_raw_t, "g_raw_t"),
                                               _chk(g_gmap, "g_gmap"), _chk(masks, "masks", torch.int32), _chk(g_pts, "g_pts"),
                                               _chk(g_vs, "g_vs"), _stream()), "nefes_field_bwd_h3_fh")
    return ray_grad_reduce(N, S, z, g_pts, g_vs)


class FieldFromRaysFH(torch.autograd.Function):

    @staticmethod
    def forward(ctx, rays_o, rays_d, viewdirs, z, pk):
        rays_o, rays_d, viewdirs, z = _f32(rays_o), _f32(rays_d), _f32(viewdirs), _f32(z)
        if z.shape[0] * z.shape[1] >= H3_MAX_SAMPLES:
            raise RuntimeError("nefes_amd: too many samples for one launch of the fp16 two-part kernels (32-bit sample index)")
        need = any(ctx.needs_input_grad[:3])
        raw_t, masks = _fh_fwd(pk, rays_o, rays_d, viewdirs, z, need)
        ctx.pk, ctx.have, ctx.pk_gen = pk, need, pk.generation
        if need:
            ctx.save_for_backward(rays_o, rays_d, viewdirs, z, raw_t, masks)
        return raw_t

    @staticmethod
    def backward(ctx, g_raw_t):
        if not ctx.have:
            return None, None, None, None, None
        rays_o, rays_d, viewdirs, z, raw_t, masks = ctx.saved_tensors
        ctx.pk.check_generation(ctx.pk_gen)
        return _fh_bwd(ctx.pk, rays_o, rays_d, viewdirs, z, raw_t, _f32(g_raw_t), None, masks) + (None, None)


class RenderFineFH(torch.autograd.Function):

    @staticmethod
    def forward(ctx, rays_o, rays_d, viewdirs, z, pk, w_f, w_f_t, b_f, flags, beta_min, emit_gmap=False):
        rays_o, rays_d, viewdirs, z = _f32(rays_o), _f32(rays_d), _f32(viewdirs), _f32(z)
        N, S = z.shape
        need = any(ctx.needs_input_grad[:3])
        Cg = pk.width // 2
        raw_t, masks = _fh_fwd(pk, rays_o, rays_d, viewdirs, z, need)
        rgb, gmap, disp, acc, _, _, _ = composite_fwd(raw_t, z, Cg + 1, flags, beta_min)
        if emit_gmap:
            feat = gmap
        else:
            C = w_f.shape[0]
            feat = torch.empty(N, C, device=z.device)
            with _timed("feat_head_fwd"):
                L.check(L.load().nefes_feat_head_fwd(N, C, Cg, _chk(gmap, "gmap"), _chk(w_f_t, "w_t"), _chk(b_f, "b"), _chk(feat, "feat"), _stream()),
                        "nefes_feat_head_fwd")
        ctx.set_materialize_grads(False)
        ctx.pk, ctx.have, ctx.pk_gen, ctx.cfg, ctx.emit_gmap = pk, need, pk.generation, (Cg, int(flags)), bool(emit_gmap)
        if need:
            ctx.save_for_backward(rays_o, rays_d, viewdirs, z, raw_t, masks, w_f, b_f)
        return rgb, feat, disp, acc

    @staticmethod
    def backward(ctx, g_rgb, g_feat, g_disp, g_acc):
        if not ctx.have:
            return (None,) * 11
        rays_o, rays_d, viewdirs, z, raw_t, masks, w_f, b_f = ctx.saved_tensors
        N, S = z.shape
        pk = ctx.pk
        pk.check_generation(ctx.pk_gen)
        Cg, flags = ctx.cfg
        fix = lambda g: None if (g is None or g.numel() == 0) else _f32(g)
        g_rgb, g_feat, g_disp, g_acc = fix(g_rgb), fix(g_feat), fix(g_disp), fix(g_acc)
        g_gmap = None
        if g_feat is not None and ctx.emit_gmap:
            g_gmap = g_feat
        elif g_feat is not None:
            g_gmap = torch.empty(N, Cg + 1, device=z.device)
            with _timed("feat_head_bwd"):
                L.check(L.load().nefes_feat_head_bwd(N, w_f.shape[0], Cg, _chk(g_feat, "g_feat"), _chk(w_f, "w"), _chk(b_f, "b"),
                                                     _chk(g_gmap, "g_gmap"), _stream()), "nefes_feat_head_bwd")
        else:
            g_gmap = torch.zeros(N, Cg + 1, device=z.device)
        g_raw_t = torch.empty_like(raw_t)
        with _timed("composite_bwd"):
            L.check(L.load().nefes_composite_bwd(N, S, Cg + 1, flags | L.COMP_FEAT_WEIGHTS_ONLY, _chk(raw_t, "raw_t"), _chk(z, "z"),
                                                 _chk(g_rgb, "g_rgb"), None, _chk(g_disp, "g_disp"), _chk(g_acc, "g_acc"), None, None, None,
                                                 _chk(g_raw_t, "g_raw_t"), _stream()), "nefes_composite_bwd")
        return _fh_bwd(pk, rays_o, rays_d, viewdirs, z, raw_t, g_raw_t, g_gmap, masks) + (None,) * 8


class FieldFromPoints(torch.autograd.Function):

    @staticmethod
    def forward(ctx, pts, viewdirs, pk, mode):
        pts = _f32(pts)
        N, S = pts.shape[0], pts.shape[1]
        if viewdirs is None:
            viewdirs = torch.zeros(N, 3, device=pts.device)
        viewdirs = _f32(viewdirs)
        need = mode in (L.FIELD_FULL, L.FIELD_STATIC) and any(ctx.needs_input_grad[:2])
        raw_t, masks = _field_fwd(pk, mode, N, S, pts=pts.reshape(-1, 3), viewdirs=viewdirs, want_masks=need)
        ctx.pk, ctx.mode, ctx.have, ctx.pk_gen = pk, mode, need, pk.generation
        if need:
            ctx.save_for_backward(pts, viewdirs, raw_t, masks)
        return raw_t

    @staticmethod
    def backward(ctx, g_raw_t):
        if not ctx.have:
            raise NotImplementedError(_NO_SIGMA_BWD)
        pts, viewdirs, raw_t, masks = ctx.saved_tensors
        N, S = pts.shape[0], pts.shape[1]
        ctx.pk.check_generation(ctx.pk_gen)
        g_pts, g_vs = _field_bwd(ctx.pk, ctx.mode, N, S, raw_t, _f32(g_raw_t), masks, pts=pts.reshape(-1, 3), viewdirs=viewdirs)
        zeros = torch.zeros(N, S, device=pts.device)
        _, _, g_v = ray_grad_reduce(N, S, zeros, g_pts, g_vs)
        return g_pts.reshape(N, S, 3), g_v, None, None


GENERIC_TRAIN = os.environ.get("NEFES_GENERIC_TRAIN", "0") == "1"
GENERIC_TRAIN_EXT = os.environ.get("NEFES_GENERIC_TRAIN_EXT", "0") == "1"
GENERIC_SET = L.GENERIC_SET


def generic_shape_ok(width, depth, skips, feat_dim):
    skips = [s for s in skips if 0 <= s < depth]
    return (width % 32 == 0 and 32 <= width <= 512 and 1 <= depth <= 8 and skips in ([], [4])
            and 0 < feat_dim <= HEAD_MAX_C)


class PackedGeneric:

    generic = True
    h3_valid = False

    @staticmethod
    def layer_names(depth, has_transient):
        names = [f"xyz_encoding_{i}.0" for i in range(1, depth + 1)] + ["xyz_encoding_final", "dir_encoding.0", "static_sigma.0", "static_rgb.0"]
        if has_transient:
            names += PackedField.LAYERS_FINE[len(PackedField.LAYERS_COARSE):]
        return names

    def __init__(self, state_dict, width, depth, skip, feat_dim, has_transient, device, xyz_encoding=L.XYZ_FREQ10):
        lib = L.load()
        self.desc = L.NefesGenericNetDesc(int(width), int(depth), int(skip), int(feat_dim), 1 if has_transient else 0, int(xyz_encoding))
        self.xyz_encoding = int(xyz_encoding)
        self.width, self.depth, self.skip = int(width), int(depth), int(skip)
        self.feat_dim, self.has_transient = int(feat_dim), bool(has_transient)
        n = int(lib.nefes_generic_blob_bytes(self.desc))
        if n == 0:
            raise RuntimeError(f"nefes_amd: no field kernel serves W={width}, D={depth}, skip={skip}, f_dim={feat_dim}, "
                               f"xyz_encoding={xyz_encoding}.  "
                               f"Compiled: {COMPILED_SET}")
        host = []
        for name in self.layer_names(self.depth, self.has_transient):
            host.append(state_dict[name + ".weight"].detach().to("cpu", torch.float32).contiguous())
            host.append(state_dict[name + ".bias"].detach().to("cpu", torch.float32).contiguous())
        ptrs = (C.c_void_p * len(host))(*[t.data_ptr() for t in host])
        blob = torch.zeros(n, dtype=torch.uint8)
        L.check(lib.nefes_generic_pack(self.desc, ptrs, len(host), C.c_void_p(blob.data_ptr()), blob.numel()), "nefes_generic_pack")
        self.blob = blob.to(device)
        self.generation = 0
        self.tile = 64 if self.width <= 256 else 32

    def repack(self, state_dict):
        dev = self.blob.device
        t = []
        for name in self.layer_names(self.depth, self.has_transient):
            t.append(state_dict[name + ".weight"].detach().to(dev, torch.float32).contiguous())
            t.append(state_dict[name + ".bias"].detach().to(dev, torch.float32).contiguous())
        ptrs = (C.c_void_p * len(t))(*[x.data_ptr() for x in t])
        L.check(L.load().nefes_generic_pack_device(self.desc, ptrs, len(t), C.c_void_p(self.blob.data_ptr()), self.blob.numel(), _stream()),
                "nefes_generic_pack_device")
        self.generation += 1
        del t

    def check_generation(self, gen):
        if gen != self.generation:
            raise RuntimeError("nefes_amd: the network weights were re-packed between this forward pass and its backward pass")

    def mask_bytes(self, M):
# ... 968 lines not shown
```

Measured before the change: 774,400 rays/s.

## Compute sigma head as fp32 dot fused into layer-8 activation staging

Adds DOT variants of the forward h3 kernel that compute the sigma output as an fp32 dot product with the sigma weights. The dot is accumulated while the layer-8 activations are being staged into the next MFMA, instead of running a separate sigma-head MFMA pass. The ring skips the sigma weight slab, and the weights are loaded into LDS from the fp32 sigma stream. The twin instance is chosen at dispatch by default, with an environment switch to turn it off. The cost is extra VALU FMAs and LDS reads in the staging path and many new kernel instantiations.

```diff
diff --git a/include/nefes_hip.h b/include/nefes_hip.h
--- a/include/nefes_hip.h
+++ b/include/nefes_hip.h
@@ -170,6 +170,8 @@
 #define NEFES_H3_REQ_ZROW 16
 #define NEFES_H3_REQ_STATIC_BWD 32
 int nefes_field_h3_instance(const NefesNetDesc* desc, int backward, int mode, unsigned request_flags, char* name, size_t cap);
+int nefes_sigma_dot(int on);
+int nefes_field_fwd_h3_runs(const NefesNetDesc* desc, int mode, unsigned request_flags, char* name, size_t cap);
 
 typedef struct NefesGenericNetDesc {
     int32_t width;
diff --git a/nefes_amd/csrc/field_fwd_h3.hip b/nefes_amd/csrc/field_fwd_h3.hip
--- a/nefes_amd/csrc/field_fwd_h3.hip
+++ b/nefes_amd/csrc/field_fwd_h3.hip
@@ -49,6 +49,7 @@
     int z_row;
     const float2* hg_table;
     HgGeom hg;
+    const float* sig_w;
     int gout;
 };
 
@@ -67,8 +68,10 @@
 
 template <int MODEF, int ENC, int W = 256, int NTR = 1, bool TRAIN = false, bool FH = false>
 __global__ __launch_bounds__(256, W == 128 ? 2 : 1) void field_fwd_h3_kernel(FieldFwdH3Args a) {
-    constexpr bool FOLD = MODEF == NEFES_FIELD_FULL_FOLD;
-    constexpr int MODE = FOLD ? NEFES_FIELD_FULL : MODEF;
+    constexpr bool DOT = (MODEF & NEFES_FIELD_DOT) != 0;
+    constexpr bool FOLD = (MODEF & ~NEFES_FIELD_DOT) == NEFES_FIELD_FULL_FOLD;
+    constexpr int MODE = FOLD ? NEFES_FIELD_FULL : (MODEF & ~NEFES_FIELD_DOT);
+    static_assert(!DOT || (W == 256 && !TRAIN && !FH && NEFES_FWD_CONSUMER_BIAS), "the dot product rides on the consumer-side bias functor of the Wd = 256 inference instances");
     static_assert(NEFES_SLAB_KIB == (W == 128 ? NEFES_H3_FWD_SLAB_KIB_128 : NEFES_H3_FWD_SLAB_KIB), "ring slab size != the packer's for this width");
     static_assert(!FOLD || (MODE != NEFES_FIELD_SIGMA && !TRAIN), "the fold serves the head products of frozen networks");
     constexpr int NTW = W / 32, NTH = W / 64;
@@ -88,7 +91,13 @@
     if constexpr (ENC == NEFES_XYZ_HASHGRID_FUSED) {
         if (threadIdx.x == 0) *hg_lds = a.hg;
     }
-    StagedRing ring;
+    float* sigw_lds = bias_lds + ((a.bias_floats + 63) / 64) * 64 + 4 * ES * 64 + (ENC == NEFES_XYZ_HASHGRID_FUSED ? 128 : 0);
+    if constexpr (DOT) {
+        for (int k = threadIdx.x; k < W; k += 256) sigw_lds[k] = a.sig_w[nefes_sig_w_index(k)];
+    }
+    constexpr int UPS_ = (NEFES_SLAB_FRAGS / 4) / 2;
+    constexpr int SIG_SLAB = 2 * ((NTW * (ES / 8) + UPS_ - 1) / UPS_) + 7 * ((NTW * (W / 16) + UPS_ - 1) / UPS_);
+    StagedRingT<DOT ? SIG_SLAB : -1> ring;
     ring.init(a.stream, a.n_slabs, ring_base, wave, lane);
     const char* ring_lane = ring_base + lane * 16;
     const char* bias_half = (const char*)bias_lds + 16 * h;
@@ -199,6 +208,19 @@
                 __builtin_nontemporal_store(softplus_ref(sg[0][0] * pow2i(-es)), &col[(size_t)ch * a.S]);
             }
         };
+        float sacc[4] = {0.f, 0.f, 0.f, 0.f};
+        float2 sw;
+        auto sigma_store = [&](int es_x) {
+            const float t = ReluBiasDotSplitH<false, NTW, WT>::sum(sacc);
+            const int e1 = (-es_x) / 2, e2 = -es_x - e1;
+            const float pre = t * pow2i(e1) * pow2i(e2) + bias_lds[B_SIG];
+            float* col = raw_col();
+            if (col && h == 0) {
+                const int ch = (MODE == NEFES_FIELD_SIGMA) ? 0 : 3 + a.C;
+                __builtin_nontemporal_store(softplus_ref(pre), &col[(size_t)ch * a.S]);
+            }
+        };
+        const char* sigw_half = (const char*)sigw_lds + 16 * h;
         int es_a, es_b = 0;
         float M;
         {
@@ -240,15 +262,26 @@
             {
                 const int ew = wexp(seg2);
                 const int tau = tau_of(p == 1 ? fmaxf(M, mE) : M, ew);
-                if (p == 3) sigma_head(B, es_b, tau_of(M, wexp(NEFES_H3F_SIG)));
+                if constexpr (!DOT) {
+                    if (p == 3) sigma_head(B, es_b, tau_of(M, wexp(NEFES_H3F_SIG)));
+                }
                 const float rb_ = rowb(seg2), bm_ = bmax(l2 <= 8 ? l2 - 1 : NEFES_H3BB_FINAL);
                 const float rbe_ = p == 1 ? rowb(NEFES_H3F_L5E) : 0.f;
                 float mx = 0.f;
                 if constexpr (CB) {
                     const char* bps = bias_half + (l1 - 1) * W * 4;
                     nbias = ReluBiasSplitH<CAP, NTW, WT>::prime(bps);
+                    if (DOT && p == 3) {
+                        if constexpr (DOT) {
+#pragma unroll
+                            for (int i = 0; i < 4; ++i) sacc[i] = 0.f;
+                            const ReluBiasDotSplitH<CAP, NTW, WT> src{{B, bits, pow2i(tau - es_b), mx, bps, pow2i(es_b), nbias}, sigw_half, sw, sacc};
+                            mma_run_h3<NTW, W / 16, 0, true>(ring, ring_lane, src, ZeroInit{}, A);
+                        }
+                    } else {
                     const ReluBiasSplitH<CAP, NTW, WT> src{B, bits, pow2i(tau - es_b), mx, bps, pow2i(es_b), nbias};
                     mma_run_h3<NTW, W / 16, 0, true>(ring, ring_lane, src, ZeroInit{}, A);
+                    }
                 } else
                 mma_run_h3<NTW, W / 16, 0, true>(ring, ring_lane, ReluSplitH<CAP, NTW, WT>{B, bits, pow2i(tau - es_b), mx},
                                                  bias_at(l2 <= 8 ? (l2 - 1) * W : B_FINAL, tau + ew), A);
@@ -261,7 +294,20 @@
         }
         if constexpr (END8) { NEFES_FWD_EVEN_LAYER(8, NEFES_H3F_L8) }
 #undef NEFES_FWD_EVEN_LAYER
-        if constexpr (MODE == NEFES_FIELD_SIGMA) sigma_head(B, es_b, tau_of(M, wexp(NEFES_H3F_SIG)));
+        if constexpr (DOT && !END8) sigma_store(es_b);
+        if constexpr (MODE == NEFES_FIELD_SIGMA) {
+            if constexpr (DOT) {
+                float mdummy = 0.f;
+                const char* bp8 = bias_half + 7 * W * 4;
+                nbias = ReluBiasSplitH<false, NTW, WT>::prime(bp8);
+#pragma unroll
+                for (int i = 0; i < 4; ++i) sacc[i] = 0.f;
+                const ReluBiasDotSplitH<false, NTW, WT> src{{B, bits, 1.f, mdummy, bp8, pow2i(es_b), nbias}, sigw_half, sw, sacc};
+                src.template dot_pass<W / 16>();
+                sigma_store(es_b);
+            } else
+                sigma_head(B, es_b, tau_of(M, wexp(NEFES_H3F_SIG)));
+        }
         if constexpr (MODE != NEFES_FIELD_SIGMA) {
             constexpr bool FULL = MODE == NEFES_FIELD_FULL;
             constexpr int NDT = FULL ? 2 * NTH : NTH;
@@ -296,7 +342,7 @@
             };
             int es_dt;
             if constexpr (FOLD) {
-                sigma_head(B, es_b, tau_of(M, wexp(NEFES_H3F_SIG)));
+                if constexpr (!DOT) sigma_head(B, es_b, tau_of(M, wexp(NEFES_H3F_SIG)));
                 const int ew = wexp(NEFES_H3F_DT_H);
                 const float mD = pair_max(array_max(Dv));
                 const int tau = tau_of(fmaxf(M, mD), ew);
@@ -308,8 +354,16 @@
                 if constexpr (CB) {
                     const char* bp8 = bias_half + 7 * W * 4;
                     nbias = ReluBiasSplitH<CAP, NTW, WT>::prime(bp8);
+                    if constexpr (DOT) {
+#pragma unroll
+                        for (int i = 0; i < 4; ++i) sacc[i] = 0.f;
+                        const ReluBiasDotSplitH<CAP, NTW, WT> src8{{B, bits, pow2i(tau - es_b), mx, bp8, pow2i(es_b), nbias}, sigw_half, sw, sacc};
+                        mma_run_h3<NDT, W / 16, 0, true>(ring, ring_lane, src8, Bias2{bias_at(B_DIR, es_dt), bias_at(B_T0, es_dt)}, dt);
+                        sigma_store(es_b);
+                    } else {
                     const ReluBiasSplitH<CAP, NTW, WT> src8{B, bits, pow2i(tau - es_b), mx, bp8, pow2i(es_b), nbias};
                     mma_run_h3<NDT, W / 16, 0, true>(ring, ring_lane, src8, Bias2{bias_at(B_DIR, es_dt), bias_at(B_T0, es_dt)}, dt);
+                    }
                 } else {
                     const ReluSplitH<CAP, NTW, WT> src8{B, bits, pow2i(tau - es_b), mx};
                     mma_run_h3<NDT, W / 16, 0, true>(ring, ring_lane, src8, Bias2{bias_at(B_DIR, es_dt), bias_at(B_T0, es_dt)}, dt);
@@ -454,7 +508,7 @@
 static int launch_h3(const FieldFwdH3Args& a, hipStream_t st) {
     constexpr int ES_ = ENC != NEFES_XYZ_FREQ10 ? NEFES_X_STEPS : NEFES_E_STEPS;
     const size_t lds = (size_t)NEFES_H3_SLOTS * NEFES_SLAB_BYTES + ((a.bias_floats + 63) / 64) * 256 + (size_t)4 * ES_ * 64 * 4
-                       + (ENC == NEFES_XYZ_HASHGRID_FUSED ? 512 : 0);
+                       + (ENC == NEFES_XYZ_HASHGRID_FUSED ? 512 : 0) + ((MODE & NEFES_FIELD_DOT) ? W * 4 : 0);
     static_assert(sizeof(HgGeom) <= 512, "the level geometry's LDS slot");
     auto k = field_fwd_h3_kernel<MODE, ENC, W, NTR, TRAIN, FH>;
     hipError_t e = hipFuncSetAttribute((const void*)k, hipFuncAttributeMaxDynamicSharedMemorySize, (int)lds);
@@ -479,7 +533,7 @@
 #endif
 #define X(part, MODE, ENC, W, NTR, TRAIN, FH) \
     static_assert(part != NEFES_TU_PART || (W == 128) == kTuW128, "a Wd = 128 row belongs to an object built for Wd = 128, and no other row does");
-NEFES_H3_FWD_INSTANCES(X)
+NEFES_H3_FWD_ALL_INSTANCES(X)
 #undef X
 
 template <int PART>
@@ -489,12 +543,12 @@
         if (k == NEFES_H3_FWD_KEY(MODE, ENC, W, NTR, TRAIN, FH))                                                       \
             return launch_h3<NEFES_FIELD_##MODE, NEFES_XYZ_##ENC, W, NTR, TRAIN != 0, FH != 0>(a, st);                 \
     }
-    NEFES_H3_FWD_INSTANCES(X)
+    NEFES_H3_FWD_ALL_INSTANCES(X)
 #undef X
     return NEFES_E_UNSUPPORTED;
 }
 #define X(part, MODE, ENC, W, NTR, TRAIN, FH) int NEFES_H3_FWD_PART_FN(part)(const NefesH3FwdKey&, const FieldFwdH3Args&, hipStream_t);
-NEFES_H3_FWD_INSTANCES(X)
+NEFES_H3_FWD_ALL_INSTANCES(X)
 #undef X
 int NEFES_H3_FWD_PART_FN(NEFES_TU_PART)(const NefesH3FwdKey& k, const FieldFwdH3Args& a, hipStream_t st) {
     return h3_fwd_launch_rows<NEFES_TU_PART>(k, a, st);
@@ -509,7 +563,7 @@
 static const H3FwdRow h3_fwd_rows[] = {
 #define X(part, MODE, ENC, W, NTR, TRAIN, FH) \
     {NEFES_H3_FWD_KEY(MODE, ENC, W, NTR, TRAIN, FH), "fwd p" #part " <" #MODE "," #ENC "," #W "," #NTR "," #TRAIN "," #FH ">", NEFES_H3_FWD_PART_FN(part)},
-    NEFES_H3_FWD_INSTANCES(X)
+    NEFES_H3_FWD_ALL_INSTANCES(X)
 #undef X
 };
 
@@ -544,13 +598,40 @@
     return {NEFES_E_UNSUPPORTED, nullptr};
 }
 
+static int g_sigma_dot = 1;
+extern "C" int nefes_sigma_dot(int on) {
+    if (on >= 0) g_sigma_dot = on != 0;
+    return g_sigma_dot;
+}
+static const H3FwdRow* h3_fwd_twin(const H3FwdRow* row) {
+    if (!g_sigma_dot || (row->key.mode & NEFES_FIELD_DOT)) return row;
+    NefesH3FwdKey key = row->key;
+    key.mode |= NEFES_FIELD_DOT;
+    for (const H3FwdRow& r : h3_fwd_rows)
+        if (r.key == key) return &r;
+    return row;
+}
+
 static int h3_fwd_stream(const NefesNetDesc* desc, const NefesH3FwdKey& k, NefesStreamInfo* si) {
     NefesBlobInfo info;
     int rc = nefes_blob_info(desc, &info);
     if (rc) return rc;
-    *si = info.stream[k.mode == NEFES_FIELD_SIGMA ? NEFES_STREAM_FWD_SIGMA_H3
-                      : (k.mode == NEFES_FIELD_STATIC ? NEFES_STREAM_FWD_STATIC_H3 : NEFES_STREAM_FWD_FULL_H3)];
+    const int mode = k.mode & ~NEFES_FIELD_DOT;
+    *si = info.stream[mode == NEFES_FIELD_SIGMA ? NEFES_STREAM_FWD_SIGMA_H3
+                      : (mode == NEFES_FIELD_STATIC ? NEFES_STREAM_FWD_STATIC_H3 : NEFES_STREAM_FWD_FULL_H3)];
     return si->n_slabs == 0 ? NEFES_E_UNSUPPORTED : 0;
+}
+static int h3_fwd_sig_w(const NefesNetDesc* desc, const void* packed, const NefesH3FwdKey& k, const float** sig_w) {
+    static_assert(256 / 2 <= NEFES_FRAGS_OF_KIB(NEFES_FWD_SLAB_KIB), "static_sigma's fp32 segment is one slab");
+    NefesBlobInfo info;
+    const int rc = nefes_blob_info(desc, &info);
+    if (rc) return rc;
+    const NefesStreamInfo& f32 = info.stream[NEFES_STREAM_FWD_SIGMA];
+    const NefesStreamInfo& h3 = info.stream[NEFES_STREAM_FWD_SIGMA_H3];
+    const uint32_t l1 = k.enc == NEFES_XYZ_FREQ10 ? 2 : 1;
+    if (k.w != 256 || f32.n_slabs == 0 || h3.n_slabs != 2 * l1 + 7 * 8 + 1) return NEFES_E_UNSUPPORTED;
+    *sig_w = (const float*)((const char*)packed + f32.slab_off + (size_t)(f32.n_slabs - 1) * NEFES_FWD_SLAB_KIB * 1024);
+    return 0;
 }
 
 static int h3_fwd_args(const NefesNetDesc* desc, const void* packed, const NefesH3FwdKey& k, int N, int S,
@@ -561,6 +642,11 @@
     a.stream = (const char*)packed + si.slab_off;
     a.bias = (const float*)((const char*)packed + si.bias_off);
     a.n_slabs = si.n_slabs; a.bias_floats = si.bias_floats; a.scale_off = si.scale_off;
+    if (k.mode & NEFES_FIELD_DOT) {
+        rc = h3_fwd_sig_w(desc, packed, k, &a.sig_w);
+        if (rc) return rc;
+    }
+    const int mode = k.mode & ~NEFES_FIELD_DOT;
     if (k.enc == NEFES_XYZ_HASHGRID_FUSED) {
         rc = hg_geometry(grid, &a.hg, nullptr);
         if (rc) return rc;
@@ -568,7 +654,7 @@
     }
     a.gout = k.fh ? k.w / 2 : 0;
     a.N = N; a.S = S; a.C = k.fh ? a.gout + 1 : desc->feat_dim;
-    a.R = k.mode == NEFES_FIELD_SIGMA ? 1 : 3 + a.C + (k.mode == NEFES_FIELD_STATIC ? 1 : 6);
+    a.R = mode == NEFES_FIELD_SIGMA ? 1 : 3 + a.C + (mode == NEFES_FIELD_STATIC ? 1 : 6);
     a.M = (long long)N * S;
     if (a.M >= (1ll << 31) - 256) return NEFES_E_UNSUPPORTED;
     a.n_tiles = (int)((a.M + 127) / 128);
@@ -581,8 +667,9 @@
                       const NefesHashGridDesc* grid, FieldFwdH3Args& a, void* stream) {
     const H3FwdSel s = h3_fwd_select(desc, mode, req);
     if (s.rc) return s.rc;
-    const int rc = h3_fwd_args(desc, packed, s.row->key, N, S, grid, a);
-    return rc ? rc : s.row->launch(s.row->key, a, (hipStream_t)stream);
+    const H3FwdRow* row = h3_fwd_twin(s.row);
+    const int rc = h3_fwd_args(desc, packed, row->key, N, S, grid, a);
+    return rc ? rc : row->launch(row->key, a, (hipStream_t)stream);
 }
 
 int nefes_h3_bwd_instance(const NefesNetDesc* desc, int mode, unsigned req, const char** name);
@@ -608,6 +695,14 @@
     return rc;
 }
 
+extern "C" int nefes_field_fwd_h3_runs(const NefesNetDesc* desc, int mode, unsigned request_flags, char* name, size_t cap) {
+    const int rc = nefes_field_h3_instance(desc, 0, mode, request_flags, name, cap);
+    if (rc) return rc;
+    const H3FwdRow* row = h3_fwd_twin(h3_fwd_select(desc, mode, request_flags).row);
+    snprintf(name, cap, "%s", row->name);
+    return 0;
+}
+
 extern "C" int nefes_field_fwd_train_h3(const NefesNetDesc* desc, const void* packed, int mode, int N, int S, const float* rays_o,
                                         const float* rays_d, const float* z, const float* pts, const float* viewdirs,
                                         float* raw_t, float* acts, uint32_t* masks, void* stream) {
diff --git a/nefes_amd/csrc/field_h3.h b/nefes_amd/csrc/field_h3.h
--- a/nefes_amd/csrc/field_h3.h
+++ b/nefes_amd/csrc/field_h3.h
@@ -180,6 +180,51 @@
     template <bool NOP>
     __device__ __forceinline__ void stage_c2(Split2& o, int p, const PairRegs& s) const { split_pair_lo<NOP>(o, p, s.x0, s.x1, r); }
 };
+template <bool CAPTURE, int NX, int NWORDS>
+struct ReluBiasDotSplitH {
+    ReluBiasSplitH<CAPTURE, NX, NWORDS> b;
+    const char* wp;
+    float2& w;
+    float (&acc)[4];
+    __device__ __forceinline__ void stage_a(PairRegs& s, int q, int p) const {
+        b.stage_a(s, q, p);
+        w = *(const float2*)(wp + ReluBiasSplitH<CAPTURE, NX, NWORDS>::pair_off(q, p));
+    }
+    __device__ __forceinline__ void stage_b(PairRegs& s) const { b.stage_b(s); }
+    __device__ __forceinline__ void dot(int p, const PairRegs& s) const {
+        acc[p] = __builtin_fmaf(w.x, s.x0, acc[p]);
+        acc[p] = __builtin_fmaf(w.y, s.x1, acc[p]);
+    }
+    template <bool NOP>
+    __device__ __forceinline__ void stage_c(Split2& o, int p, const PairRegs& s) const {
+        dot(p, s);
+        b.template stage_c<NOP>(o, p, s);
+    }
+    __device__ __forceinline__ void stage_c1(Split2& o, int p, const PairRegs& s) const { b.stage_c1(o, p, s); }
+    template <bool NOP>
+    __device__ __forceinline__ void stage_c2(Split2& o, int p, const PairRegs& s) const { b.template stage_c2<NOP>(o, p, s); }
+    template <int KS16>
+    __device__ __forceinline__ void dot_pass() const {
+#pragma unroll
+        for (int q = 0; q < KS16; ++q)
+#pragma unroll
+            for (int p = 0; p < 4; ++p) {
+                PairRegs s;
+                stage_a(s, q, p);
+                s.x0 = relu1<false>(s.x0);
+                s.x1 = relu1<false>(s.x1);
+                dot(p, s);
+            }
+    }
+    static __device__ __forceinline__ float sum(const float (&a)[4]) {
+        const float t = (a[0] + a[1]) + (a[2] + a[3]);
+        const uint32_t u = __float_as_uint(t);
+        const auto r = __builtin_amdgcn_permlane32_swap(u, u, false, false);
+        return __uint_as_float(r[0]) + __uint_as_float(r[1]);
+    }
+};
+template <class T> struct h3_has_dot { static constexpr bool value = false; };
+template <bool CAPTURE, int NX, int NWORDS> struct h3_has_dot<ReluBiasDotSplitH<CAPTURE, NX, NWORDS>> { static constexpr bool value = true; };
 template <int NX>
 struct IdentBiasSplitH {
     const f32x16 (&X)[NX];
@@ -299,7 +344,8 @@
     }
 };
 
-struct StagedRing {
+template <int SKIP>
+struct StagedRingT {
     const char* src;
     uint32_t n_slabs;
     uint32_t g_next;
@@ -310,6 +356,15 @@
     f32x4 pf;
     f32x4 stage[NEFES_SLAB_PIECES];
 
+    __device__ __forceinline__ void advance() {
+        if constexpr (SKIP < 0) {
+            g_next = (g_next + 1 == n_slabs) ? 0 : g_next + 1;
+        } else {
+            uint32_t g = g_next + 1;
+            if (g == (uint32_t)SKIP) ++g;
+            g_next = g >= n_slabs ? 0 : g;
+        }
+    }
     __device__ __forceinline__ void load_piece(int q) {
         stage[q] = *(const f32x4*)(src + (size_t)g_next * NEFES_SLAB_BYTES + my_off + q * 1024);
     }
@@ -325,19 +380,19 @@
         g_next = n_slabs > 1 ? 1 : 0;
 #pragma unroll
         for (int q = 0; q < NEFES_SLAB_PIECES; ++q) load_piece(q);
-        g_next = (g_next + 1 == n_slabs) ? 0 : g_next + 1;
+        advance();
     }
     __device__ __forceinline__ void store_piece(int q) {
         *(f32x4*)(my_lds + (c_slot ^ 1u) * NEFES_SLAB_BYTES + q * 1024) = stage[q];
     }
     __device__ __forceinline__ void fetch_piece(int q) {
         load_piece(q);
-        if (q == NEFES_SLAB_PIECES - 1) g_next = (g_next + 1 == n_slabs) ? 0 : g_next + 1;
+        if (q == NEFES_SLAB_PIECES - 1) advance();
     }
     __device__ __forceinline__ void issue_piece(int q) {
         *(f32x4*)(my_lds + (c_slot ^ 1u) * NEFES_SLAB_BYTES + q * 1024) = stage[q];
         load_piece(q);
-        if (q == NEFES_SLAB_PIECES - 1) g_next = (g_next + 1 == n_slabs) ? 0 : g_next + 1;
+        if (q == NEFES_SLAB_PIECES - 1) advance();
     }
     __device__ __forceinline__ uint32_t acquire() {
         asm volatile("s_waitcnt lgkmcnt(0)" ::: "memory");
@@ -353,6 +408,7 @@
     }
     __device__ __forceinline__ void drain() {}
 };
+typedef StagedRingT<-1> StagedRing;
 
 __device__ __forceinline__ void mfma_h3_asm(f32x16& c, const f32x4& a, const u32x4& b) {
     asm volatile("v_mfma_f32_32x32x16_f16 %0, %1, %2, %0" : "+a"(c) : "v"(a), "v"(b));
@@ -445,6 +501,9 @@
                 else mfma_h3_asm(acc[T0 + t], h0, B.l);
                 __builtin_amdgcn_sched_barrier(0);
                 if (host) src.stage_b(ps[pp]);
+                if constexpr (h3_has_dot<SrcFn>::value) {
+                    if (tail) src.dot(pp, ps[pp]);
+                }
                 if (host && uu != acq_u) h2 = *(const f32x4*)(pn);
                 if (!host) {
 #pragma unroll
diff --git a/nefes_amd/csrc/field_h3_instances.h b/nefes_amd/csrc/field_h3_instances.h
--- a/nefes_amd/csrc/field_h3_instances.h
+++ b/nefes_amd/csrc/field_h3_instances.h
@@ -13,6 +13,11 @@
 #define NEFES_XYZ_HASHGRID_FUSED 2
 #define NEFES_FIELD_FULL_FOLD 3
 #define NEFES_H3B_FOLD 16
+#define NEFES_FIELD_DOT 4
+#define NEFES_FIELD_SIGMA_DOT (NEFES_FIELD_SIGMA | NEFES_FIELD_DOT)
+#define NEFES_FIELD_STATIC_DOT (NEFES_FIELD_STATIC | NEFES_FIELD_DOT)
+#define NEFES_FIELD_FULL_DOT (NEFES_FIELD_FULL | NEFES_FIELD_DOT)
+#define NEFES_FIELD_FULL_FOLD_DOT (NEFES_FIELD_FULL_FOLD | NEFES_FIELD_DOT)
 
 struct NefesH3FwdKey { int mode, enc, w, ntr, train, fh; };
 struct NefesH3BwdKey { int w, kr16, enc, has_t, train, fh; };
@@ -62,6 +67,21 @@
     X(15, STATIC, EXTERNAL32, 256, 5, 1, 0)                                                                                        \
     X(15, FULL, EXTERNAL32, 256, 5, 1, 0)
 
+#define NEFES_H3_FWD_DOT_INSTANCES(X)                                                                                              \
+    X(17, SIGMA_DOT, FREQ10, 256, 1, 0, 0)                                                                                         \
+    X(17, FULL_DOT, FREQ10, 256, 1, 0, 0)                                                                                          \
+    X(19, SIGMA_DOT, EXTERNAL32, 256, 1, 0, 0)                                                                                     \
+    X(19, FULL_DOT, EXTERNAL32, 256, 1, 0, 0)                                                                                      \
+    X(19, STATIC_DOT, FREQ10, 256, 1, 0, 0)                                                                                        \
+    X(21, SIGMA_DOT, HASHGRID_FUSED, 256, 1, 0, 0)                                                                                 \
+    X(21, FULL_DOT, HASHGRID_FUSED, 256, 1, 0, 0)                                                                                  \
+    X(23, FULL_DOT, FREQ10, 256, 5, 0, 0)                                                                                          \
+    X(23, STATIC_DOT, FREQ10, 256, 5, 0, 0)                                                                                        \
+    X(25, FULL_FOLD_DOT, FREQ10, 256, 1, 0, 0)                                                                                     \
+    X(27, FULL_FOLD_DOT, FREQ10, 256, 5, 0, 0)                                                                                     \
+    X(29, FULL_DOT, EXTERNAL32, 256, 5, 0, 0)
+#define NEFES_H3_FWD_ALL_INSTANCES(X) NEFES_H3_FWD_INSTANCES(X) NEFES_H3_FWD_DOT_INSTANCES(X)
+
 #define NEFES_H3_BWD_INSTANCES(X)                                                                                                  \
     X(0, 256, 2, FREQ10, 1, 0, 0)                                                                                                  \
     X(1, 256, 2, EXTERNAL32, 1, 0, 0)                                                                                              \
diff --git a/nefes_amd/csrc/layout.h b/nefes_amd/csrc/layout.h
--- a/nefes_amd/csrc/layout.h
+++ b/nefes_amd/csrc/layout.h
@@ -39,6 +39,10 @@
 NEFES_HD int nefes_head_ntr(int C) { return 3 + C <= 32 ? 1 : 5; }
 NEFES_HD int nefes_head_kr16(int C) { return 3 + C <= 32 ? 2 : 9; }
 #define NEFES_HEAD_MAX_C 141
+NEFES_HD int nefes_sig_w_index(int k) {
+    const int row = k & 31, s = 16 * (k >> 5) + nefes_row_reg(row);
+    return (s >> 2) * 256 + (s & 3) + 128 * nefes_row_half(row);
+}
 NEFES_HD int nefes_steps_per_slab(int nt, int slab_frags) { return slab_frags / nt; }
 NEFES_HD int nefes_segment_slabs(int nt, int ks, int slab_frags) {
     const int sps = slab_frags / nt;
diff --git a/nefes_amd/lib.py b/nefes_amd/lib.py
--- a/nefes_amd/lib.py
+++ b/nefes_amd/lib.py
@@ -112,6 +112,8 @@
     "nefes_field_bwd_h3": (_i, [_desc, _p, _i, _i, _p, _p, _p, _p, _p, _p, _p, _p, _p, _p, _p, _p]),
     "nefes_field_bwd_static_h3": (_i, [_desc, _p, _i, _i, _p, _p, _p, _p, _p, _p, _p, _p, _p, _p, _p]),
     "nefes_field_h3_instance": (_i, [_desc, _i, _i, C.c_uint, C.c_char_p, _sz]),
+    "nefes_sigma_dot": (_i, [_i]),
+    "nefes_field_fwd_h3_runs": (_i, [_desc, _i, C.c_uint, C.c_char_p, _sz]),
     "nefes_feat_head_fwd": (_i, [_i, _i, _i, _p, _p, _p, _p, _p]),
     "nefes_feat_head_bwd": (_i, [_i, _i, _i, _p, _p, _p, _p, _p]),
     "nefes_field_fwd_h3_fh": (_i, [_desc, _p, _i, _i, _i, _p, _p, _p, _p, _p, _p, _p]),
diff --git a/nefes_amd/ops.py b/nefes_amd/ops.py
--- a/nefes_amd/ops.py
+++ b/nefes_amd/ops.py
@@ -467,6 +467,7 @@
 USE_X6 = os.environ.get("NEFES_X6", "1") != "0"
 FUSED_COARSE = os.environ.get("NEFES_FUSED_COARSE", "1") != "0"
 FOLD_FINAL = os.environ.get("NEFES_FOLD_FINAL", "1") != "0"
+SIGMA_DOT = os.environ.get("NEFES_SIGMA_DOT", "1") != "0"
 FACTORED_HEAD = os.environ.get("NEFES_FACTORED_HEAD", "1") != "0"
 FIELD_GENERIC = os.environ.get("NEFES_FIELD_GENERIC", "0") == "1"
 FUSED_HASHGRID = os.environ.get("NEFES_FUSED_HASHGRID", "1") != "0"
@@ -636,6 +637,15 @@
     return "points" if pts is not None else ("enc" if xyz_enc is not None else "rays")
 
 
+_SIGMA_DOT_SENT = True
+
+
+def _send_sigma_dot():
+    global _SIGMA_DOT_SENT
+    if bool(SIGMA_DOT) != _SIGMA_DOT_SENT:
+        _SIGMA_DOT_SENT = bool(L.load().nefes_sigma_dot(1 if SIGMA_DOT else 0))
+
+
 def _field_fwd(pk, mode, N, S, rays_o=None, rays_d=None, z=None, pts=None, xyz_enc=None, viewdirs=None, want_masks=False, grid=None,
                override=None):
     rt = field_route(pk, mode, False, _input_kind(z, pts, xyz_enc, grid), N * S, override)
@@ -653,6 +663,7 @@
         args = (mode, N, S, o, d, zz, v)
     else:
         args = (mode, N, S, o, d, zz, _chk(pts, "pts"), _chk(xyz_enc, "xyz_enc"), v)
+    _send_sigma_dot()
     with _timed(rt.key):
         L.check(getattr(L.load(), rt.entry)(pk.desc, _blob(pk), *args, _chk(raw_t, "raw_t"), _chk(masks, "masks", torch.int32), _stream()),
                 rt.label)
```

Result: no change. 781,700 rays/s, median of 6 (+0.9%).
